# frankcholula/sapr

Hardware: AMD Instinct MI355X
Metric: frames/sec MFCC+Viterbi (16kHz, 13-MFCC, 8-state HMM) (higher is better)
Workload: dtype f32 (MFCC) + f64 (trellis); 1 GPU; configs[1]+[2]: 16 kHz 1 s utterances -> 13 MFCC (25 ms/10 ms, n_fft 512, 40 mels) -> Viterbi vs 11 word models x 8 emitting states (decoder.py API), features materialised in HBM; utterances_per_gpu=100000, frames_per_utterance=101, word_models=11, states=10, parallelism=utterance-shard x1, decoder=pruned

## Files before the change

### include/sapr_hip.h

```cpp
#ifndef SAPR_HIP_H
#define SAPR_HIP_H

#include <stddef.h>
#include <stdint.h>

#ifdef __cplusplus
extern "C" {
#endif

#define SAPR_ABI_VERSION 2

#define SAPR_TOPO_DENSE 0
#define SAPR_TOPO_BIDIAG 1

#define SAPR_TIE_LOW 0
#define SAPR_TIE_HIGH 1

#define SAPR_SUM_PAIRWISE 0
#define SAPR_SUM_TVIEW 1
#define SAPR_SUM_SEQ 2

#define SAPR_PACK_FAST_DIV 1
#define SAPR_PACK_BOUND_OK 2
#define SAPR_ESTEP_STAGED 256
#define SAPR_PACK_GEMM_OK 4
#define SAPR_PACK_BIDIAG 8

#define SAPR_PACK_EXACT_ONLY 16

#define SAPR_ERR_ARG (-1)
#define SAPR_ERR_UNSUPPORTED (-2)
#define SAPR_ERR_WORKSPACE (-3)

int sapr_abi_version(void);
const char *sapr_last_error(void);
int sapr_device_info(int dev, int *cu_count, int *wave_size, char *arch, size_t arch_len);
int sapr_selftest_lse(const double *d, int64_t n, double *out, void *stream);

int sapr_viterbi_workspace_bytes(int64_t n_utts, int32_t W, int32_t S, int32_t max_T,
                                 int32_t topology, size_t *bytes);

int sapr_diag_pack_bytes(int32_t W, int32_t S, int32_t D, size_t *bytes);
int sapr_diag_pack(const double *means, const double *vars, const double *gconst,
                   const double *log_start, const double *log_trans, int32_t W, int32_t S, int32_t D,
                   void *pack, size_t pack_bytes, int32_t *pack_flags , void *stream);

int sapr_viterbi_diag_scores(const float *feats, const int64_t *offsets, const int32_t *order,
                             int64_t n_utts, int32_t D, int32_t max_T, const void *pack,
                             int32_t W, int32_t S, int32_t topology, int32_t tie, int32_t sum_order,
                             int32_t fast_div, void *workspace, size_t workspace_bytes,
                             double *scores, int32_t *last_state, void *stream);

int sapr_viterbi_backtrace(const int64_t *offsets, const int32_t *order, int64_t n_utts,
                           int32_t max_T, int32_t W, int32_t S, int32_t topology,
                           const void *workspace, size_t workspace_bytes,
                           const double *scores, const int32_t *last_state,
                           const int32_t *word_sel,
                           int32_t *best_word, double *best_score,
                           int32_t *path , void *stream);

int sapr_viterbi_pruned_workspace_bytes(int64_t n_utts, int32_t W, int32_t S, int32_t max_T, size_t *bytes);
int sapr_viterbi_decode_pruned(const float *feats, const int64_t *offsets, const int32_t *order, int64_t n_utts,
                               int32_t D, int32_t max_T, const void *pack, int32_t W, int32_t S, int32_t tie,
                               int32_t sum_order, int32_t pack_flags, void *workspace, size_t workspace_bytes,
                               int32_t *best_word, double *best_score, int32_t *path ,
                               void *stream);
int sapr_viterbi_pruned_views(int64_t n_utts, int32_t W, int32_t max_T, void *workspace, double **approx_score,
                              double **approx_eps, double **exact_score, int32_t **cand_slot,
                              int32_t **cand_count);

int sapr_fb_workspace_bytes(int64_t n_utts, int64_t n_tiles, int32_t S, int32_t D, int32_t max_T,
                            size_t *bytes);
int sapr_stats_width(int32_t S, int32_t D, int32_t *width);
int sapr_forward_diag(const float *feats, const int64_t *offsets, const int32_t *slot_utt,
                      const int32_t *tile_model, int64_t n_tiles, int32_t D, const void *pack,
                      int32_t W, int32_t S, int32_t topology, int32_t fast_div, double *loglik,
                      void *stream);
int sapr_estep_diag(const float *feats, const int64_t *offsets, const int32_t *slot_utt,
                    const int32_t *tile_model, const int32_t *model_tile_off, int64_t n_utts,
                    int64_t n_tiles, int32_t D, int32_t max_T, const void *pack, int32_t W, int32_t S,
                    int32_t topology, int32_t fast_div, void *workspace, size_t workspace_bytes,
                    double *loglik, double *stats, void *stream);

int sapr_colsum_f32(const float *x, int64_t n_rows, int32_t D, const float *center , float *out,
                    void *stream);

int sapr_custom_estep(const float *feats, const int64_t *offsets, const int32_t *utt_model, int64_t n_utts,
                      int32_t D, int32_t S, int32_t W, const double *means, const double *inv,
                      const double *cterm, const double *A, const double *logA, int64_t lane_slots, double *E,
                      double *alpha, double *beta, double *gamma, double *xi_dense ,
                      double *utt_out, void *stream);
int sapr_custom_stage_features(const float *feats, const int64_t *offsets, int64_t n_utts, int32_t D, int32_t max_T,
                               int64_t lane_slots, float *feat_t, double *frame_sums , void *stream);
int sapr_custom_estep_staged(const float *feats, const int64_t *offsets, const int32_t *utt_model, int64_t n_utts,
                             int32_t D, int32_t S, int32_t W, const double *means, const double *inv,
                             const double *cterm, const double *A, const double *logA, int64_t lane_slots, double *E,
                             double *alpha, double *beta, double *gamma, double *xi ,
                             double *utt_out, const float *feat_t ,
                             const double *frame_sums , void *stream);
int sapr_custom_piece(int32_t op, const float *x, int32_t T, int32_t D, int32_t S, const double *means,
                      const double *inv, const double *cterm, const double *A, const double *logA, double *E,
                      double *alpha, double *beta, double *gamma, double *xi, double *scalar, void *stream);
int sapr_custom_emission_exact(const float *feats, const int64_t *offsets, int64_t n_utts, int32_t W, int32_t D,
                               int32_t S, int32_t n_rows, int32_t max_T ,
                               const double *means, const double *inv, const double *cterm, double *E, void *stream);
int sapr_custom_decode(const float *feats, const int64_t *offsets, int64_t n_utts, int32_t W, int32_t D,
                       int32_t S, int32_t num_states, int32_t Tq, const double *means, const double *inv,
                       const double *cterm, const double *A, const double *logA, double *e_rows, double *scores,
                       int32_t *paths, int32_t *best_word, double *best_score, int32_t *best_path, void *stream);
int sapr_custom_update_b_workspace_bytes(int64_t n_utts, int32_t W, int32_t D, int32_t S, size_t *bytes);
int sapr_custom_update_b(const float *feats, const int64_t *offsets, const int32_t *utt_model, int64_t n_utts,
                         int32_t W, int32_t D, int32_t S, const double *gamma, int64_t lane_slots,
                         double *means_out, double *occ_out, double *covs_out, void *workspace,
                         size_t workspace_bytes, void *stream);
int sapr_custom_update_b_sums(const float *feats, const int64_t *offsets, const int32_t *utt_model, int64_t n_utts,
                              int32_t W, int32_t D, int32_t S, const double *gamma, int64_t lane_slots,
                              double *sum_x_out, double *occ_out, void *workspace, size_t workspace_bytes,
                              void *stream);
int sapr_custom_update_b_scatter(const float *feats, const int64_t *offsets, const int32_t *utt_model,
                                 int64_t n_utts, int32_t W, int32_t D, int32_t S, const double *gamma,
                                 int64_t lane_slots, const double *means, double *scatter_out, void *workspace,
                                 size_t workspace_bytes, void *stream);
int sapr_custom_update_b_moments(const float *feats, const int64_t *offsets, int64_t n_utts, int32_t D, int32_t S,
                                 const double *gamma, int64_t lane_slots, const double *center, double *out,
                                 void *workspace, size_t workspace_bytes, void *stream);
int sapr_custom_normalise(double *x, const double *occ, int64_t n_states, int32_t per, void *stream);
int sapr_custom_fold_rows(const double *part, int64_t n_rows, int64_t K, double *out, void *stream);
int sapr_custom_global_workspace_bytes(int64_t n_utts, int64_t total_frames, int32_t D, size_t *bytes);
int sapr_custom_global_sum(const float *feats, const int64_t *offsets, int64_t n_utts, int32_t D,
                           double *sum_out, void *workspace, size_t workspace_bytes, void *stream);
int sapr_custom_global_cov(const float *feats, int64_t total_frames, int32_t D, const double *mean,
                           double *cov_out, void *workspace, size_t workspace_bytes, void *stream);

int sapr_mfcc_plan_create(double sr, int32_t n_fft, int32_t win_length, int32_t hop,
                          int32_t n_mels, int32_t n_mfcc, double fmin, double fmax ,
                          double top_db, double preemph , int32_t deltas,
                          int32_t max_frames, void **plan_out);
int sapr_mfcc_plan_destroy(void *plan);
int sapr_mfcc_plan_info(const void *plan, int32_t *d_out, int32_t *max_frames, int64_t *lds_bytes,
                        int32_t *mel_ksteps);
int sapr_mfcc_workspace_bytes(const void *plan, int64_t total_frames, int64_t n_utts, size_t *bytes);
int sapr_mfcc_batch(const void *plan, const float *pcm, const int64_t *sample_offsets,
                    const int64_t *frame_offsets, int64_t n_utts, int64_t total_frames, float *out,
                    int32_t grid_blocks , void *workspace ,
                    size_t workspace_bytes, void *stream);

int sapr_resample_poly(const float *x, const int64_t *in_offsets, const int64_t *out_offsets, int64_t n_utts,
                       int64_t max_out, int32_t up, int32_t down, const float *taps, int32_t n_taps,
                       int32_t n_pre_remove, float *y, void *stream);

int sapr_pcm16_to_f32(const int16_t *pcm16, int64_t n_samples, float *out, void *stream);

int sapr_mfcc_batch_stamped(const void *plan, const float *pcm, const int64_t *sample_offsets,
                            const int64_t *frame_offsets, int64_t n_utts, float *out,
                            int32_t grid_blocks, uint64_t *stamps, void *stream);

#ifdef __cplusplus
}
#endif
#endif
```

### sapr_amd/_lib.py

```python
from __future__ import annotations

import ctypes as C
import os

HERE = os.path.dirname(os.path.abspath(__file__))
LIB_PATH = os.environ.get("SAPR_LIB") or os.path.join(HERE, "libsapr_hip.so")

c_void_p, c_int, c_int32, c_int64, c_size_t, c_double, c_float = (
    C.c_void_p, C.c_int, C.c_int32, C.c_int64, C.c_size_t, C.c_double, C.c_float)

SIGNATURES = {
    "sapr_abi_version": (c_int, []),
    "sapr_last_error": (C.c_char_p, []),
    "sapr_device_info": (c_int, [c_int, C.POINTER(c_int), C.POINTER(c_int), C.c_char_p, c_size_t]),
    "sapr_selftest_lse": (c_int, [c_void_p, c_int64, c_void_p, c_void_p]),
    "sapr_viterbi_workspace_bytes": (c_int, [c_int64, c_int32, c_int32, c_int32, c_int32,
                                             C.POINTER(c_size_t)]),
    "sapr_diag_pack_bytes": (c_int, [c_int32, c_int32, c_int32, C.POINTER(c_size_t)]),
    "sapr_diag_pack": (c_int, [c_void_p, c_void_p, c_void_p, c_void_p, c_void_p, c_int32, c_int32, c_int32,
                               c_void_p, c_size_t, C.POINTER(c_int32), c_void_p]),
    "sapr_viterbi_diag_scores": (c_int, [c_void_p, c_void_p, c_void_p, c_int64, c_int32, c_int32,
                                         c_void_p, c_int32, c_int32, c_int32, c_int32, c_int32, c_int32,
                                         c_void_p, c_size_t, c_void_p, c_void_p, c_void_p]),
    "sapr_viterbi_backtrace": (c_int, [c_void_p, c_void_p, c_int64, c_int32, c_int32, c_int32, c_int32,
                                       c_void_p, c_size_t, c_void_p, c_void_p, c_void_p,
                                       c_void_p, c_void_p, c_void_p, c_void_p]),
    "sapr_viterbi_pruned_workspace_bytes": (c_int, [c_int64, c_int32, c_int32, c_int32, C.POINTER(c_size_t)]),
    "sapr_viterbi_decode_pruned": (c_int, [c_void_p, c_void_p, c_void_p, c_int64, c_int32, c_int32, c_void_p,
                                           c_int32, c_int32, c_int32, c_int32, c_int32, c_void_p, c_size_t,
                                           c_void_p, c_void_p, c_void_p, c_void_p]),
    "sapr_viterbi_pruned_views": (c_int, [c_int64, c_int32, c_int32, c_void_p] + [C.POINTER(c_void_p)] * 5),
    "sapr_fb_workspace_bytes": (c_int, [c_int64, c_int64, c_int32, c_int32, c_int32, C.POINTER(c_size_t)]),
    "sapr_stats_width": (c_int, [c_int32, c_int32, C.POINTER(c_int32)]),
    "sapr_forward_diag": (c_int, [c_void_p, c_void_p, c_void_p, c_void_p, c_int64, c_int32, c_void_p,
                                  c_int32, c_int32, c_int32, c_int32, c_void_p, c_void_p]),
    "sapr_estep_diag": (c_int, [c_void_p, c_void_p, c_void_p, c_void_p, c_void_p, c_int64, c_int64, c_int32,
                                c_int32, c_void_p, c_int32, c_int32, c_int32, c_int32, c_void_p, c_size_t,
                                c_void_p, c_void_p, c_void_p]),
    "sapr_colsum_f32": (c_int, [c_void_p, c_int64, c_int32, c_void_p, c_void_p, c_void_p]),
    "sapr_custom_estep": (c_int, [c_void_p, c_void_p, c_void_p, c_int64, c_int32, c_int32, c_int32] + [c_void_p] * 5
                          + [c_int64] + [c_void_p] * 6 + [c_void_p]),
    "sapr_custom_stage_features": (c_int, [c_void_p, c_void_p, c_int64, c_int32, c_int32, c_int64, c_void_p, c_void_p,
                                           c_void_p]),
    "sapr_custom_estep_staged": (c_int, [c_void_p, c_void_p, c_void_p, c_int64, c_int32, c_int32, c_int32] + [c_void_p] * 5
                                 + [c_int64] + [c_void_p] * 6 + [c_void_p, c_void_p, c_void_p]),
    "sapr_custom_piece": (c_int, [c_int32, c_void_p, c_int32, c_int32, c_int32] + [c_void_p] * 11 + [c_void_p]),
    "sapr_custom_emission_exact": (c_int, [c_void_p, c_void_p, c_int64, c_int32, c_int32, c_int32, c_int32, c_int32]
                                   + [c_void_p] * 4 + [c_void_p]),
    "sapr_custom_decode": (c_int, [c_void_p, c_void_p, c_int64, c_int32, c_int32, c_int32, c_int32, c_int32]
                           + [c_void_p] * 11 + [c_void_p]),
    "sapr_custom_update_b_workspace_bytes": (c_int, [c_int64, c_int32, c_int32, c_int32, C.POINTER(c_size_t)]),
    "sapr_custom_update_b": (c_int, [c_void_p, c_void_p, c_void_p, c_int64, c_int32, c_int32, c_int32, c_void_p, c_int64]
                             + [c_void_p] * 4 + [c_size_t, c_void_p]),
    "sapr_custom_update_b_sums": (c_int, [c_void_p, c_void_p, c_void_p, c_int64, c_int32, c_int32, c_int32, c_void_p,
                                          c_int64] + [c_void_p] * 3 + [c_size_t, c_void_p]),
    "sapr_custom_update_b_scatter": (c_int, [c_void_p, c_void_p, c_void_p, c_int64, c_int32, c_int32, c_int32, c_void_p,
                                             c_int64] + [c_void_p] * 3 + [c_size_t, c_void_p]),
    "sapr_custom_update_b_moments": (c_int, [c_void_p, c_void_p, c_int64, c_int32, c_int32, c_void_p, c_int64, c_void_p,
                                             c_void_p, c_void_p, c_size_t, c_void_p]),
    "sapr_custom_normalise": (c_int, [c_void_p, c_void_p, c_int64, c_int32, c_void_p]),
    "sapr_custom_fold_rows": (c_int, [c_void_p, c_int64, c_int64, c_void_p, c_void_p]),
    "sapr_custom_global_workspace_bytes": (c_int, [c_int64, c_int64, c_int32, C.POINTER(c_size_t)]),
    "sapr_custom_global_sum": (c_int, [c_void_p, c_void_p, c_int64, c_int32, c_void_p, c_void_p, c_size_t, c_void_p]),
    "sapr_custom_global_cov": (c_int, [c_void_p, c_int64, c_int32, c_void_p, c_void_p, c_void_p, c_size_t, c_void_p]),
    "sapr_pcm16_to_f32": (c_int, [c_void_p, c_int64, c_void_p, c_void_p]),
    "sapr_resample_poly": (c_int, [c_void_p, c_void_p, c_void_p, c_int64, c_int64, c_int32, c_int32, c_void_p, c_int32,
                                   c_int32, c_void_p, c_void_p]),
    "sapr_mfcc_plan_create": (c_int, [c_double, c_int32, c_int32, c_int32, c_int32, c_int32, c_double,
                                      c_double, c_double, c_double, c_int32, c_int32,
                                      C.POINTER(c_void_p)]),
    "sapr_mfcc_plan_destroy": (c_int, [c_void_p]),
    "sapr_mfcc_plan_info": (c_int, [c_void_p, C.POINTER(c_int32), C.POINTER(c_int32),
                                    C.POINTER(c_int64), C.POINTER(c_int32)]),
    "sapr_mfcc_workspace_bytes": (c_int, [c_void_p, c_int64, c_int64, C.POINTER(c_size_t)]),
    "sapr_mfcc_batch": (c_int, [c_void_p, c_void_p, c_void_p, c_void_p, c_int64, c_int64, c_void_p, c_int32,
                                c_void_p, c_size_t, c_void_p]),
    "sapr_mfcc_batch_stamped": (c_int, [c_void_p, c_void_p, c_void_p, c_void_p, c_int64, c_void_p, c_int32,
                                        c_void_p, c_void_p]),
}

TOPO_DENSE, TOPO_BIDIAG = 0, 1
TIE_LOW, TIE_HIGH = 0, 1
PACK_FAST_DIV, PACK_BOUND_OK, PACK_GEMM_OK, PACK_BIDIAG, PACK_EXACT_ONLY = 1, 2, 4, 8, 16
ESTEP_STAGED = 256
SUM_PAIRWISE, SUM_TVIEW, SUM_SEQ = 0, 1, 2

_lib = None


class SaprHipError(RuntimeError):
    pass


def load():
    global _lib
    if _lib is not None:
        return _lib
    if not os.path.exists(LIB_PATH):
        raise SaprHipError(
            f"{LIB_PATH} is missing: build it with `python -m sapr_amd.build` "
            "(hipcc --offload-arch=gfx950).  sapr_amd has no CPU fallback.")
    import torch
    lib = C.CDLL(LIB_PATH)
    for name, (res, args) in SIGNATURES.items():
        try:
            fn = getattr(lib, name)
        except AttributeError as e:
            raise SaprHipError(f"{LIB_PATH} lacks symbol {name}; rebuild it") from e
        fn.restype = res
        fn.argtypes = args
    if lib.sapr_abi_version() != 2:
        raise SaprHipError("libsapr_hip.so ABI version mismatch; rebuild it")
    _lib = lib
    return lib


def check(rc: int, what: str) -> None:
    if rc != 0:
        msg = load().sapr_last_error().decode("utf-8", "replace")
        raise SaprHipError(f"{what} failed (rc={rc}): {msg}")


def ptr(t):
    if t is None:
        return None
    return C.c_void_p(t.data_ptr())


def require_gpu():
    import torch
    if not torch.cuda.is_available():
        raise SaprHipError("no HIP device visible: sapr_amd kernels need an MI355X (gfx950); "
                           "there is no CPU fallback")
    return torch.device("cuda", torch.cuda.current_device())


def current_stream():
    import torch
    return C.c_void_p(torch.cuda.current_stream().cuda_stream)


def to_host(*tensors):
    import torch
    outs = []
    for t in tensors:
        if t.is_cuda:
            o = torch.empty(t.shape, dtype=t.dtype, pin_memory=True)
            o.copy_(t, non_blocking=True)
        else:
            o = t
        outs.append(o)
    if any(t.is_cuda for t in tensors):
        torch.cuda.current_stream().synchronize()
    return tuple(o.numpy() for o in outs)
```

### sapr_amd/csrc/mfcc.hip

```cpp
#include <cmath>
#include <algorithm>
#include <cstdlib>
#include <cstring>
#include <functional>
#include <type_traits>
#include <vector>

#include "sapr_common.h"

#pragma clang fp contract(fast)

#ifndef SAPR_ABLATE
#define SAPR_ABLATE 0
#endif

namespace sapr {
namespace {

constexpr int kThreads = 256;
constexpr int kWaves = kThreads / kWave;
constexpr double kPi = 3.14159265358979323846264338327950288;

typedef float f32x4 __attribute__((ext_vector_type(4)));

// ... 613 lines not shown
    if constexpr (TWO_PASS) {
      if (tid == 0) gmax_out[u] = enc_ordered(gmax);
      __syncthreads();
      continue;
    }
    const float floor_db = gmax - P.top_db;
    SAPR_STAMP(9)

    const int n_ks = align_up(P.n_mels, 16) / 4;
    for (int nt = wave; nt * 16 < T; nt += kWaves) {
      f32x4 acc = {0.f, 0.f, 0.f, 0.f};
      const int t = nt * 16 + j16;
      const int tc = t < T ? t : T - 1;
      const float *lrow = s_lm + tc * P.lm_stride + q;
      for (int ks = 0; ks < n_ks; ks += 4) {
        float a[4], b[4];
#pragma unroll
        for (int i = 0; i < 4; ++i) {
          a[i] = P.dct_frag[(ks + i) * kWave + lane];
          const int mel = 4 * (ks + i) + q;
          b[i] = mel < P.n_mels ? fmaxf(lrow[4 * (ks + i)], floor_db) : 0.f;
        }
#pragma unroll
        for (int i = 0; i < 4; ++i) acc = __builtin_amdgcn_mfma_f32_16x16x4f32(a[i], b[i], acc, 0, 0, 0);
      }
      if (t < T) *reinterpret_cast<f32x4 *>(&s_out[t * 16 + 4 * q]) = acc;
    }
    __syncthreads();
    SAPR_STAMP(10)

    {
      float *__restrict__ o = out + f_beg * P.d_out;
      const int total = T * P.d_out;
      for (int e = tid; e < total; e += kThreads) {
        const int t = e / P.d_out;
        const int c = e - t * P.d_out;
        float v;
        if (c < P.n_mfcc) {
          v = s_out[t * 16 + c];
        } else {
          const int order = c / P.n_mfcc;
          const int cc = c - order * P.n_mfcc;
          const float *tab = s_dtab + (order - 1) * 81;
          int row, t0;
          if (t < 4) {
            row = 1 + t;
            t0 = 0;
          } else if (t >= T - 4) {
            row = 5 + (t - (T - 4));
            t0 = T - 9;
          } else {
            row = 0;
            t0 = t - 4;
          }
          v = 0.f;
#pragma unroll
          for (int k = 0; k < 9; ++k) v += tab[row * 9 + k] * s_out[(t0 + k) * 16 + cc];
        }
        o[e] = v;
      }
    }
    __syncthreads();
    SAPR_STAMP(11)
  }
  if constexpr (STAMP) {
    if (lane == 0)
      for (int i = 0; i < 12; ++i) stamps[(static_cast<int64_t>(blockIdx.x) * kWaves + wave) * 12 + i] = st_acc[i];
  }
}
#undef SAPR_STAMP

constexpr int kFinChunk = 96, kFinHalo = 8, kFinRows = kFinChunk + 2 * kFinHalo;

__global__ __launch_bounds__(kThreads) void mfcc_finish_kernel(const float *__restrict__ lm,
                                                               const unsigned *__restrict__ gmax,
                                                               const int64_t *__restrict__ frame_offsets,
                                                               int64_t n_utts, MfccDev P, float *__restrict__ out) {
  extern __shared__ __attribute__((aligned(16))) unsigned char smem[];
  float *s_dtab = reinterpret_cast<float *>(smem);
  float *s_c = s_dtab + align_up(2 * 81, 4);
  float *s_l = s_c + kFinRows * 16;
  const int tid = threadIdx.x;
  const int wave = tid / kWave, lane = tid % kWave;
  const int q = lane >> 4, j16 = lane & 15;
  for (int i = tid; i < 2 * 81; i += kThreads) s_dtab[i] = P.delta_tab[i];
  __syncthreads();
  const int n_ks = align_up(P.n_mels, 16) / 4;
  for (int64_t u = blockIdx.x; u < n_utts; u += gridDim.x) {
    const int64_t f_beg = frame_offsets[u];
    const int T = static_cast<int>(frame_offsets[u + 1] - f_beg);
    const float floor_db = dec_ordered(gmax[u]) - P.top_db;
    const int chunk = T <= kFinRows ? T : kFinChunk;
    for (int c0 = 0; c0 < T; c0 += chunk) {
      const int c1 = c0 + chunk < T ? c0 + chunk : T;
      const int r0 = c0 - kFinHalo > 0 ? c0 - kFinHalo : 0;
      const int r1 = c1 + kFinHalo < T ? c1 + kFinHalo : T;
      const int rows = r1 - r0;
      const float *src = lm + (f_beg + r0) * P.n_mels;
      for (int i = tid; i < rows * P.n_mels; i += kThreads) {
        const int r = i / P.n_mels, m = i - r * P.n_mels;
        s_l[r * P.lm_stride + m] = fmaxf(src[i], floor_db);
      }
      __syncthreads();
      for (int nt = wave; nt * 16 < rows; nt += kWaves) {
        f32x4 acc = {0.f, 0.f, 0.f, 0.f};
        const int r = nt * 16 + j16;
        const int rc = r < rows ? r : rows - 1;
        const float *lrow = s_l + rc * P.lm_stride + q;
        for (int ks = 0; ks < n_ks; ks += 4) {
          float a[4], bb[4];
#pragma unroll
          for (int i = 0; i < 4; ++i) {
            a[i] = P.dct_frag[(ks + i) * kWave + lane];
            const int mel = 4 * (ks + i) + q;
            bb[i] = mel < P.n_mels ? lrow[4 * (ks + i)] : 0.f;
          }
#pragma unroll
          for (int i = 0; i < 4; ++i) acc = __builtin_amdgcn_mfma_f32_16x16x4f32(a[i], bb[i], acc, 0, 0, 0);
        }
        if (r < rows) *reinterpret_cast<f32x4 *>(&s_c[r * 16 + 4 * q]) = acc;
      }
      __syncthreads();
      float *__restrict__ o = out + (f_beg + c0) * P.d_out;
      const int total = (c1 - c0) * P.d_out;
      for (int e = tid; e < total; e += kThreads) {
        const int tl = e / P.d_out, c = e - tl * P.d_out;
        const int t = c0 + tl;
        float v;
        if (c < P.n_mfcc) {
          v = s_c[(t - r0) * 16 + c];
        } else {
          const int order = c / P.n_mfcc, cc = c - order * P.n_mfcc;
          const float *tab = s_dtab + (order - 1) * 81;
          int row, t0;
          if (t < 4) {
            row = 1 + t;
            t0 = 0;
          } else if (t >= T - 4) {
            row = 5 + (t - (T - 4));
            t0 = T - 9;
          } else {
            row = 0;
            t0 = t - 4;
          }
          v = 0.f;
#pragma unroll
          for (int k = 0; k < 9; ++k) v += tab[row * 9 + k] * s_c[(t0 + k - r0) * 16 + cc];
        }
        o[e] = v;
      }
      __syncthreads();
    }
  }
}

double hz_to_mel(double f) {
  const double f_sp = 200.0 / 3, min_log_hz = 1000.0, min_log_mel = min_log_hz / f_sp;
  const double logstep = std::log(6.4) / 27.0;
  return f >= min_log_hz ? min_log_mel + std::log(f / min_log_hz) / logstep : f / f_sp;
}
double mel_to_hz(double m) {
  const double f_sp = 200.0 / 3, min_log_hz = 1000.0, min_log_mel = min_log_hz / f_sp;
  const double logstep = std::log(6.4) / 27.0;
  return m >= min_log_mel ? min_log_hz * std::exp(logstep * (m - min_log_mel)) : f_sp * m;
}

std::vector<float> mel_filterbank(double sr, int n_fft, int n_mels, double fmin, double fmax) {
  const int nb = 1 + n_fft / 2;
  std::vector<double> mel_f(n_mels + 2);
  const double m0 = hz_to_mel(fmin), m1 = hz_to_mel(fmax);
  for (int i = 0; i < n_mels + 2; ++i) mel_f[i] = mel_to_hz(m0 + (m1 - m0) * i / (n_mels + 1));
  std::vector<float> w(static_cast<size_t>(n_mels) * nb, 0.f);
  for (int i = 0; i < n_mels; ++i) {
    const double fd0 = mel_f[i + 1] - mel_f[i], fd1 = mel_f[i + 2] - mel_f[i + 1];
    const double enorm = 2.0 / (mel_f[i + 2] - mel_f[i]);
    for (int b = 0; b < nb; ++b) {
      const double f = b * sr / n_fft;
      const double lower = -(mel_f[i] - f) / fd0, upper = (mel_f[i + 2] - f) / fd1;
      const double v = std::fmax(0.0, std::fmin(lower, upper));
      const float v32 = static_cast<float>(v);
      w[static_cast<size_t>(i) * nb + b] = static_cast<float>(static_cast<double>(v32) * enorm);
    }
  }
  return w;
}

void savgol_row(int order, double pos, double *out9) {
  const int n = 9, m = order + 1;
  double AtA[3][3] = {{0}}, inv[3][3];
  for (int i = 0; i < n; ++i) {
    double pw[3] = {1.0, i - pos, (i - pos) * (i - pos)};
    for (int a = 0; a < m; ++a)
      for (int b = 0; b < m; ++b) AtA[a][b] += pw[a] * pw[b];
  }
  double aug[3][6];
  for (int a = 0; a < m; ++a)
    for (int b = 0; b < m; ++b) {
      aug[a][b] = AtA[a][b];
      aug[a][m + b] = a == b ? 1.0 : 0.0;
    }
  for (int c = 0; c < m; ++c) {
    int piv = c;
    for (int r2 = c + 1; r2 < m; ++r2)
      if (std::fabs(aug[r2][c]) > std::fabs(aug[piv][c])) piv = r2;
    for (int b = 0; b < 2 * m; ++b) std::swap(aug[c][b], aug[piv][b]);
    const double d = aug[c][c];
    for (int b = 0; b < 2 * m; ++b) aug[c][b] /= d;
    for (int r2 = 0; r2 < m; ++r2)
      if (r2 != c) {
        const double f = aug[r2][c];
        for (int b = 0; b < 2 * m; ++b) aug[r2][b] -= f * aug[c][b];
      }
  }
  for (int a = 0; a < m; ++a)
    for (int b = 0; b < m; ++b) inv[a][b] = aug[a][m + b];
  const double fact = order == 2 ? 2.0 : 1.0;
  for (int i = 0; i < n; ++i) {
    double pw[3] = {1.0, i - pos, (i - pos) * (i - pos)};
    double c = 0.0;
    for (int b = 0; b < m; ++b) c += inv[order][b] * pw[b];
    out9[i] = fact * c;
  }
}

constexpr int kKsr = 24;

template <int R, bool PRE, bool MLDS, int KSR, bool TWO, bool BMEL = false>
hipError_t launch_one(const MfccPlan &pl, const float *pcm, const int64_t *so, const int64_t *fo,
                      int64_t n_utts, float *out, int grid, hipStream_t st, float *lm, unsigned *gmax) {
  if (pl.lds_bytes > 64 * 1024) {
    hipError_t e = hipFuncSetAttribute(reinterpret_cast<const void *>(&mfcc_kernel<R, PRE, MLDS, KSR, false, TWO, BMEL>),
                                       hipFuncAttributeMaxDynamicSharedMemorySize,
                                       static_cast<int>(pl.lds_bytes));
    if (e != hipSuccess) return e;
  }
  SAPR_LAUNCH((mfcc_kernel<R, PRE, MLDS, KSR, false, TWO, BMEL>), dim3(grid), dim3(kThreads), pl.lds_bytes, st, pcm, so,
              fo, n_utts, pl.dev, out, static_cast<unsigned long long *>(nullptr), lm, gmax);
  return hipGetLastError();
}

template <int R, bool TWO>
hipError_t launch(const MfccPlan &pl, const float *pcm, const int64_t *so, const int64_t *fo,
                  int64_t n_utts, float *out, int grid, hipStream_t st, float *lm, unsigned *gmax) {
  const bool pre = pl.dev.preemph != 0.f, ml = pl.dev.mel_in_lds != 0;
  if constexpr (R == 16) {
    if (pl.dev.ksr == kKsr) {
      if (pl.dev.mel_bf16) {
        if (pre) return launch_one<R, true, false, kKsr, TWO, true>(pl, pcm, so, fo, n_utts, out, grid, st, lm, gmax);
        return launch_one<R, false, false, kKsr, TWO, true>(pl, pcm, so, fo, n_utts, out, grid, st, lm, gmax);
      }
      if (pre) return launch_one<R, true, false, kKsr, TWO>(pl, pcm, so, fo, n_utts, out, grid, st, lm, gmax);
      return launch_one<R, false, false, kKsr, TWO>(pl, pcm, so, fo, n_utts, out, grid, st, lm, gmax);
    }
  }
  if (pre && ml) return launch_one<R, true, true, 0, TWO>(pl, pcm, so, fo, n_utts, out, grid, st, lm, gmax);
  if (pre) return launch_one<R, true, false, 0, TWO>(pl, pcm, so, fo, n_utts, out, grid, st, lm, gmax);
  if (ml) return launch_one<R, false, true, 0, TWO>(pl, pcm, so, fo, n_utts, out, grid, st, lm, gmax);
  return launch_one<R, false, false, 0, TWO>(pl, pcm, so, fo, n_utts, out, grid, st, lm, gmax);
}

template <bool PRE, int RLO, int RHI, int S4>
hipError_t wave_prepare(size_t lds, int *blocks_per_cu) {
  const void *fn = reinterpret_cast<const void *>(&mfcc_wave_kernel<PRE, RLO, RHI, S4>);
  if (lds > 64 * 1024) {
    hipError_t e = hipFuncSetAttribute(fn, hipFuncAttributeMaxDynamicSharedMemorySize, static_cast<int>(lds));
    if (e != hipSuccess) return e;
  }
  return hipOccupancyMaxActiveBlocksPerMultiprocessor(blocks_per_cu, fn, kThreads, lds);
}
template <bool PRE, int RLO, int RHI, int S4>
hipError_t wave_launch_one(const MfccPlan &pl, const float *pcm, const int64_t *so, const int64_t *fo, int64_t n_utts,
                           int grid, int64_t span, hipStream_t st, float *lm, unsigned *gmax, int64_t total_cap) {
  SAPR_LAUNCH((mfcc_wave_kernel<PRE, RLO, RHI, S4>), dim3(grid), dim3(kThreads), pl.wave_lds, st, pcm, so, fo, n_utts,
              pl.dev, lm, gmax, span, total_cap);
  return hipGetLastError();
}
template <bool PRE, int RLO, int RHI>
hipError_t wave_dispatch_s4(const MfccPlan &pl, int *prepare, const float *pcm, const int64_t *so, const int64_t *fo,
                            int64_t n_utts, int grid, int64_t span, hipStream_t st, float *lm, unsigned *gmax,
                            int64_t total_cap) {
  switch (pl.dev.wave_s4) {
#define SAPR_WAVE_CASE(S4)                                                                                        \
  case S4:                                                                                                        \
    return prepare ? wave_prepare<PRE, RLO, RHI, S4>(pl.wave_lds, prepare)                                        \
                   : wave_launch_one<PRE, RLO, RHI, S4>(pl, pcm, so, fo, n_utts, grid, span, st, lm, gmax, total_cap);
    SAPR_WAVE_CASE(6)
    SAPR_WAVE_CASE(7)
    SAPR_WAVE_CASE(8)
#undef SAPR_WAVE_CASE
    default:
      return hipErrorInvalidValue;
  }
}
hipError_t wave_dispatch(const MfccPlan &pl, int *prepare, const float *pcm, const int64_t *so, const int64_t *fo,
                         int64_t n_utts, int grid, int64_t span, hipStream_t st, float *lm, unsigned *gmax,
                         int64_t total_cap) {
  const bool pre = pl.dev.preemph != 0.f, tight = pl.wave_rlo == 1 && pl.wave_rhi == 15;
  if (pre && tight) return wave_dispatch_s4<true, 1, 15>(pl, prepare, pcm, so, fo, n_utts, grid, span, st, lm, gmax, total_cap);
  if (pre) return wave_dispatch_s4<true, 0, 16>(pl, prepare, pcm, so, fo, n_utts, grid, span, st, lm, gmax, total_cap);
  if (tight) return wave_dispatch_s4<false, 1, 15>(pl, prepare, pcm, so, fo, n_utts, grid, span, st, lm, gmax, total_cap);
  return wave_dispatch_s4<false, 0, 16>(pl, prepare, pcm, so, fo, n_utts, grid, span, st, lm, gmax, total_cap);
}

size_t finish_lds_bytes(const MfccDev &d) {
  return static_cast<size_t>(align_up(2 * 81, 4) + kFinRows * 16 + kFinRows * d.lm_stride) * 4;
}

}
}

using namespace sapr;

extern "C" int sapr_mfcc_plan_create(double sr, int32_t n_fft, int32_t win_length, int32_t hop,
                                     int32_t n_mels, int32_t n_mfcc, double fmin, double fmax,
                                     double top_db, double preemph, int32_t deltas,
                                     int32_t max_frames, void **plan_out) {
  SAPR_REQUIRE(plan_out != nullptr, "plan_out is NULL");
  SAPR_REQUIRE(n_fft == 512 || n_fft == 2048, "n_fft must be 512 or 2048 (got %d)", n_fft);
  SAPR_REQUIRE(win_length > 0 && win_length <= n_fft && hop > 0, "bad window/hop");
  SAPR_REQUIRE(n_mels > 0 && n_mels <= 128 && n_mfcc > 0 && n_mfcc <= 16 && n_mfcc <= n_mels,
               "need 0 < n_mfcc <= 16, n_mfcc <= n_mels <= 128");
  SAPR_REQUIRE(max_frames >= 0, "max_frames must be >= 0 (0 = two-pass, any utterance length)");
  SAPR_REQUIRE(!deltas || max_frames == 0 || max_frames >= 9, "deltas need at least 9 frames");
  if (fmax <= 0) fmax = sr / 2;
  const int R = n_fft == 512 ? 16 : 32;
  const int Nc = R * R, nb = Nc + 1;
  MfccPlan *pl = new MfccPlan();
  pl->R = R;
  MfccDev &d = pl->dev;
  d.n_fft = n_fft;
  d.win_length = win_length;
  d.hop = hop;
  d.n_mels = n_mels;
  d.n_mfcc = n_mfcc;
  d.deltas = deltas ? 1 : 0;
  d.d_out = n_mfcc * (deltas ? 3 : 1);
  d.n_bins = nb;
  d.lm_stride = n_mels | 1;
  d.t_pad = max_frames;
  d.two_pass = max_frames == 0 ? 1 : 0;
  d.preemph = static_cast<float>(preemph);
  d.top_db = static_cast<float>(top_db);
  d.amin = 1e-10f;

  std::vector<float> win(n_fft, 0.f);
  const int lpad = (n_fft - win_length) / 2;
  for (int i = 0; i < win_length; ++i)
    win[lpad + i] = static_cast<float>(0.5 * (0.54 - 0.46 * std::cos(2.0 * kPi * i / win_length)));
  d.r_lo = lpad / (2 * R);
  d.r_hi = (lpad + win_length - 1) / (2 * R) + 1;
  if (d.r_hi > R) d.r_hi = R;

  std::vector<float> twab(2 * R * R), twu(2 * Nc);
  for (int k1 = 0; k1 < R; ++k1)
    for (int l = 0; l < R; ++l) {
      const double a = -2.0 * kPi * k1 * l / Nc;
      twab[2 * (k1 * R + l)] = static_cast<float>(std::cos(a));
      twab[2 * (k1 * R + l) + 1] = static_cast<float>(std::sin(a));
    }
  for (int k = 0; k < Nc; ++k) {
    const double a = -kPi * k / Nc;
    twu[2 * k] = static_cast<float>(std::cos(a));
    twu[2 * k + 1] = static_cast<float>(std::sin(a));
  }

  std::vector<float> mel = mel_filterbank(sr, n_fft, n_mels, fmin, fmax);
  std::vector<int> mlo(n_mels), mhi(n_mels);
  for (int m = 0; m < n_mels; ++m) {
    int lo = nb, hi = -1;
    for (int b = 0; b < nb; ++b)
      if (mel[static_cast<size_t>(m) * nb + b] != 0.f) {
        lo = b < lo ? b : lo;
        hi = b > hi ? b : hi;
      }
    if (hi < 0) lo = hi = 0;
    mlo[m] = lo;
    mhi[m] = hi;
  }
  auto tile_ks = [&](int m0, int m1) {
    int lo = nb, hi = 0;
    for (int m = m0; m < m1; ++m) {
      lo = mlo[m] < lo ? mlo[m] : lo;
      hi = mhi[m] > hi ? mhi[m] : hi;
    }
    lo = lo / 4 * 4;
    return align_up((hi - lo) / 4 + 1, 4);
  };
  const int want_tiles = align_up((n_mels + 15) / 16, kWaves);
  auto cut = [&](int limit, std::vector<int> *starts) {
    int m0 = 0, n = 0;
    if (starts) starts->clear();
    while (m0 < n_mels) {
      int m1 = m0 + 1;
      if (tile_ks(m0, m1) > limit) return 1 << 30;
      while (m1 < n_mels && m1 - m0 < 16 && tile_ks(m0, m1 + 1) <= limit) ++m1;
      if (starts) starts->push_back(m0);
      m0 = m1;
      ++n;
    }
    return n;
  };
  int lim_lo = 4, lim_hi = align_up(nb / 4 + 1, 4);
  while (lim_lo < lim_hi) {
    const int mid = (lim_lo + lim_hi) / 8 * 4;
    if (cut(mid, nullptr) <= want_tiles)
      lim_hi = mid;
    else
      lim_lo = mid + 4;
  }
  std::vector<int> starts;
  cut(lim_lo, &starts);
  d.n_mtiles = static_cast<int>(starts.size());
  if (d.n_mtiles > 15) {
    delete pl;
    return fail(SAPR_ERR_UNSUPPORTED, "mel filterbank needs %d tiles (> 15)", d.n_mtiles);
  }
  std::vector<int> tiles(4 * (d.n_mtiles + 1), 0);
  std::vector<float> frag;
  int ks_total = 0;
  for (int mt = 0; mt < d.n_mtiles; ++mt) {
    const int m0 = starts[mt], m1 = mt + 1 < d.n_mtiles ? starts[mt + 1] : n_mels;
    int lo = nb;
    for (int m = m0; m < m1; ++m) lo = mlo[m] < lo ? mlo[m] : lo;
    lo = lo / 4 * 4;
    const int nks = tile_ks(m0, m1);
    tiles[4 * mt + 0] = m0;
    tiles[4 * mt + 1] = m1 - m0;
    tiles[4 * mt + 2] = lo;
    tiles[4 * mt + 3] = ks_total;
    for (int ks = 0; ks < nks; ++ks)
      for (int ln = 0; ln < 64; ++ln) {
        const int mi = ln & 15, b = lo + 4 * ks + (ln >> 4);
        frag.push_back((mi < m1 - m0 && b < nb) ? mel[static_cast<size_t>(m0 + mi) * nb + b] : 0.f);
      }
    ks_total += nks;
  }
  tiles[4 * d.n_mtiles + 3] = ks_total;
  d.total_ks = ks_total;
  auto bf16_rn = [](float v) {
    unsigned b;
    std::memcpy(&b, &v, 4);
    b = (b + 0x7FFFu + ((b >> 16) & 1u)) >> 16;
    return b;
  };
  auto bf16_val = [](unsigned h) {
    const unsigned b = h << 16;
    float v;
    std::memcpy(&v, &b, 4);
    return v;
  };
  std::vector<unsigned> frag16;
  if (d.n_mtiles <= kWaves) {
    frag16.assign(static_cast<size_t>(d.n_mtiles) * 24 * 64, 0u);
    for (int mt = 0; mt < d.n_mtiles; ++mt) {
      const int m0 = tiles[4 * mt + 0], cnt = tiles[4 * mt + 1], lo = tiles[4 * mt + 2];
      for (int c = 0; c < 3; ++c)
        for (int i = 0; i < 4; ++i)
          for (int ln = 0; ln < 64; ++ln) {
            unsigned hi_w = 0, lo_w = 0;
            for (int h = 0; h < 2; ++h) {
              const int mi = ln & 15, b = lo + 32 * c + 8 * i + 2 * (ln >> 4) + h;
              const float v = (mi < cnt && b < nb) ? mel[static_cast<size_t>(m0 + mi) * nb + b] : 0.f;
              const unsigned vh = bf16_rn(v), vl = bf16_rn(v - bf16_val(vh));
              hi_w |= vh << (16 * h);
              lo_w |= vl << (16 * h);
            }
            frag16[(static_cast<size_t>(mt) * 24 + 8 * c + i) * 64 + ln] = hi_w;
            frag16[(static_cast<size_t>(mt) * 24 + 8 * c + 4 + i) * 64 + ln] = lo_w;
          }
    }
  }
  const int nks_d = align_up(n_mels, 16) / 4;
  std::vector<float> dfrag(static_cast<size_t>(std::max(nks_d, 16)) * 64, 0.f);
  for (int ks = 0; ks < nks_d; ++ks)
    for (int ln = 0; ln < 64; ++ln) {
      const int c = ln & 15, m = 4 * ks + (ln >> 4);
      if (c < n_mfcc && m < n_mels) {
        const double sc = c == 0 ? std::sqrt(1.0 / (4.0 * n_mels)) : std::sqrt(1.0 / (2.0 * n_mels));
        dfrag[ks * 64 + ln] = static_cast<float>(2.0 * std::cos(kPi * c * (2 * m + 1) / (2.0 * n_mels)) * sc);
      }
    }
  WavePack wp;
  {
    const char *core = std::getenv("SAPR_MFCC_CORE");
    const bool want = !(core && std::strcmp(core, "tile") == 0);
    if (want && R == 16 && hop % 2 == 0) wp = wave_pack(mel, n_mels, nb);
  }
  std::vector<float> dtab(2 * 81, 0.f);
  for (int order = 1; order <= 2; ++order) {
    double row[9];
    savgol_row(order, 4.0, row);
    for (int k = 0; k < 9; ++k) dtab[(order - 1) * 81 + k] = static_cast<float>(row[k]);
    for (int p = 0; p < 4; ++p) {
      savgol_row(order, p, row);
      for (int k = 0; k < 9; ++k) dtab[(order - 1) * 81 + (1 + p) * 9 + k] = static_cast<float>(row[k]);
      savgol_row(order, 5 + p, row);
      for (int k = 0; k < 9; ++k) dtab[(order - 1) * 81 + (5 + p) * 9 + k] = static_cast<float>(row[k]);
    }
  }

  auto pad = [](size_t b) { return (b + 255) / 256 * 256; };
  const size_t b_win = pad(win.size() * 4), b_ab = pad(twab.size() * 4), b_u = pad(twu.size() * 4),
               b_fr = pad(frag.size() * 4), b_ti = pad(tiles.size() * 4),
               b_df = pad(dfrag.size() * 4), b_dt = pad(dtab.size() * 4), b_f16 = pad(frag16.size() * 4 + 4),
               b_wa = pad(wp.a.size() * 4 + 4), b_wb = pad(wp.blk.size() * 4 + 4);
  const size_t total = b_win + b_ab + b_u + b_fr + b_ti + b_df + b_dt + b_f16 + b_wa + b_wb;
  std::vector<unsigned char> host(total, 0);
  size_t o = 0;
  auto put = [&](const void *src, size_t bytes, size_t padded) {
    std::copy(static_cast<const unsigned char *>(src), static_cast<const unsigned char *>(src) + bytes,
              host.begin() + o);
    const size_t at = o;
    o += padded;
    return at;
  };
  const size_t o_win = put(win.data(), win.size() * 4, b_win);
  const size_t o_ab = put(twab.data(), twab.size() * 4, b_ab);
  const size_t o_u = put(twu.data(), twu.size() * 4, b_u);
  const size_t o_fr = put(frag.data(), frag.size() * 4, b_fr);
  const size_t o_ti = put(tiles.data(), tiles.size() * 4, b_ti);
  const size_t o_df = put(dfrag.data(), dfrag.size() * 4, b_df);
  const size_t o_dt = put(dtab.data(), dtab.size() * 4, b_dt);
  const size_t o_f16 = put(frag16.data(), frag16.size() * 4, b_f16);
  const size_t o_wa = put(wp.a.data(), wp.a.size() * 4, b_wa);
  const size_t o_wb = put(wp.blk.data(), wp.blk.size() * 4, b_wb);
  unsigned char *devbuf = nullptr;
  hipError_t e = hipMalloc(reinterpret_cast<void **>(&devbuf), total);
  if (e != hipSuccess) {
    delete pl;
    return hip_fail(e, "hipMalloc(mfcc tables)");
  }
  e = hipMemcpy(devbuf, host.data(), total, hipMemcpyHostToDevice);
  if (e != hipSuccess) {
    (void)hipFree(devbuf);
    delete pl;
    return hip_fail(e, "hipMemcpy(mfcc tables)");
  }
  pl->buffer = devbuf;
  d.window = reinterpret_cast<const float *>(devbuf + o_win);
  d.tw_ab = reinterpret_cast<const float2 *>(devbuf + o_ab);
  d.tw_u = reinterpret_cast<const float2 *>(devbuf + o_u);
  d.mel_frag = reinterpret_cast<const float *>(devbuf + o_fr);
  d.mel_tiles = reinterpret_cast<const int *>(devbuf + o_ti);
  d.dct_frag = reinterpret_cast<const float *>(devbuf + o_df);
  d.delta_tab = reinterpret_cast<const float *>(devbuf + o_dt);
  d.mel_frag_bf16 = reinterpret_cast<const unsigned *>(devbuf + o_f16);
  d.wave_s4 = wp.s4;
  d.wave_a = reinterpret_cast<const float *>(devbuf + o_wa);
  d.wave_blk = reinterpret_cast<const int *>(devbuf + o_wb);

  {
    const int tile = R == 16 ? 16 : 8;
    d.span0 = 2 * R * d.r_lo - n_fft / 2;
    d.span_len = (tile - 1) * hop + 2 * R * (d.r_hi - d.r_lo);
    d.stage_floats = align_up(d.span_len, 4);
    if (d.span_len > kStagePasses * kThreads * 4 || hop % 2 != 0) {
      (void)hipFree(devbuf);
      delete pl;
      return fail(SAPR_ERR_UNSUPPORTED, "hop %d / window %d: staged span of %d samples unsupported (max %d, even hop)",
                  hop, win_length, d.span_len, kStagePasses * kThreads * 4);
    }
  }
  int max_nks = 0;
  for (int mt = 0; mt < d.n_mtiles; ++mt) {
    const int nks = tiles[4 * (mt + 1) + 3] - tiles[4 * mt + 3];
    max_nks = nks > max_nks ? nks : max_nks;
  }
  d.ksr = (R == 16 && d.n_mtiles <= kWaves && max_nks <= kKsr) ? kKsr : 0;
  {
    const char *sel = std::getenv("SAPR_MFCC_MEL");
    d.mel_bf16 = (d.ksr && sel && std::strcmp(sel, "bf16") == 0) ? 1 : 0;
  }
  auto lds_total = [&](int ml) {
    const int tp = d.two_pass ? 0 : d.t_pad;
    return R == 16 ? lds_layout<16>(tp, d.lm_stride, d.total_ks, ml, d.n_mels, d.stage_floats).total
                   : lds_layout<32>(tp, d.lm_stride, d.total_ks, ml, d.n_mels, d.stage_floats).total;
  };
  auto pick_mel = [&]() {
    if (d.ksr) return 0;
    return lds_total(1) <= 80 * 1024 || (lds_total(0) > 80 * 1024 && lds_total(1) <= 160 * 1024) ? 1 : 0;
  };
  d.mel_in_lds = pick_mel();
  if (!d.two_pass && lds_total(d.mel_in_lds) > 160 * 1024) {
    d.two_pass = 1;
    d.mel_in_lds = pick_mel();
  }
  if (!d.two_pass && lds_total(d.mel_in_lds) > 80 * 1024) {
    const char *keep = std::getenv("SAPR_MFCC_FUSED");
    MfccDev t = d;
    t.two_pass = 1;
    auto total_of = [&](const MfccDev &x, int ml) {
      return R == 16 ? lds_layout<16>(0, x.lm_stride, x.total_ks, ml, x.n_mels, x.stage_floats).total
                     : lds_layout<32>(0, x.lm_stride, x.total_ks, ml, x.n_mels, x.stage_floats).total;
    };
    const int ml2 = t.ksr ? 0 : ((total_of(t, 1) <= 80 * 1024 || (total_of(t, 0) > 80 * 1024 && total_of(t, 1) <= 160 * 1024)) ? 1 : 0);
    if (!(keep && keep[0] == '1') && total_of(t, ml2) <= 80 * 1024) {
      d.two_pass = 1;
      d.mel_in_lds = ml2;
    }
  }
  pl->lds_bytes = static_cast<size_t>(lds_total(d.mel_in_lds));
  if (pl->lds_bytes > 160 * 1024) {
    (void)hipFree(devbuf);
    const size_t need = pl->lds_bytes;
    delete pl;
    return fail(SAPR_ERR_UNSUPPORTED, "configuration needs %zu bytes of LDS (> 160 KiB)", need);
  }
  if (d.wave_s4) {
    d.two_pass = 1;
    pl->wave_rlo = (d.r_lo >= 1 && d.r_hi <= 15) ? 1 : 0;
    pl->wave_rhi = (d.r_lo >= 1 && d.r_hi <= 15) ? 15 : 16;
    pl->wave_lds = static_cast<size_t>(wave_lds(d.wave_s4, wave_region_floats(d.n_mels, d.deltas)).total);
    pl->lds_bytes = pl->wave_lds;
    hipError_t oe = wave_dispatch(*pl, &pl->wave_blocks_per_cu, nullptr, nullptr, nullptr, 0, 0, 1, nullptr, nullptr,
                                  nullptr, 0);
    if (oe != hipSuccess || pl->wave_blocks_per_cu < 1) {
      (void)hipFree(devbuf);
      delete pl;
      return hip_fail(oe, "occupancy query (mfcc_wave_kernel)");
    }
  }
  *plan_out = pl;
  return 0;
}

extern "C" int sapr_mfcc_plan_destroy(void *plan) {
  if (!plan) return 0;
  MfccPlan *pl = static_cast<MfccPlan *>(plan);
  if (pl->buffer) (void)hipFree(pl->buffer);
  delete pl;
  return 0;
}

extern "C" int sapr_mfcc_plan_info(const void *plan, int32_t *d_out, int32_t *max_frames,
                                   int64_t *lds_bytes, int32_t *mel_ksteps) {
  SAPR_REQUIRE(plan != nullptr, "plan is NULL");
  const MfccPlan *pl = static_cast<const MfccPlan *>(plan);
  if (d_out) *d_out = pl->dev.d_out;
  if (max_frames) *max_frames = pl->dev.two_pass ? 0 : pl->dev.t_pad;
  if (lds_bytes) *lds_bytes = static_cast<int64_t>(pl->lds_bytes);
  if (mel_ksteps) *mel_ksteps = pl->dev.total_ks;
  return 0;
}

extern "C" int sapr_mfcc_batch_stamped(const void *plan, const float *pcm, const int64_t *sample_offsets,
                                       const int64_t *frame_offsets, int64_t n_utts, float *out,
                                       int32_t grid_blocks, uint64_t *stamps, void *stream) {
  SAPR_REQUIRE(plan && pcm && sample_offsets && frame_offsets && out && stamps, "NULL pointer argument");
  const MfccPlan *pl = static_cast<const MfccPlan *>(plan);
  SAPR_REQUIRE(pl->R == 16 && pl->dev.preemph == 0.f && pl->dev.ksr == kKsr, "stamped build: bench preset only");
  SAPR_REQUIRE(grid_blocks > 0 && grid_blocks <= n_utts, "bad grid");
  if (pl->dev.mel_bf16) {
    if (pl->lds_bytes > 64 * 1024)
      SAPR_HIP_TRY(hipFuncSetAttribute(reinterpret_cast<const void *>(&mfcc_kernel<16, false, false, kKsr, true, false, true>),
                                       hipFuncAttributeMaxDynamicSharedMemorySize, static_cast<int>(pl->lds_bytes)));
    SAPR_LAUNCH((mfcc_kernel<16, false, false, kKsr, true, false, true>), dim3(grid_blocks), dim3(kThreads),
                pl->lds_bytes, as_stream(stream), pcm, sample_offsets, frame_offsets, n_utts, pl->dev, out,
                reinterpret_cast<unsigned long long *>(stamps));
  } else {
    if (pl->lds_bytes > 64 * 1024)
      SAPR_HIP_TRY(hipFuncSetAttribute(reinterpret_cast<const void *>(&mfcc_kernel<16, false, false, kKsr, true>),
                                       hipFuncAttributeMaxDynamicSharedMemorySize, static_cast<int>(pl->lds_bytes)));
    SAPR_LAUNCH((mfcc_kernel<16, false, false, kKsr, true>), dim3(grid_blocks), dim3(kThreads), pl->lds_bytes,
                as_stream(stream), pcm, sample_offsets, frame_offsets, n_utts, pl->dev, out,
                reinterpret_cast<unsigned long long *>(stamps));
  }
  SAPR_HIP_TRY(hipGetLastError());
  return 0;
}

extern "C" int sapr_mfcc_workspace_bytes(const void *plan, int64_t total_frames, int64_t n_utts, size_t *bytes) {
  SAPR_REQUIRE(plan && bytes && total_frames >= 0 && n_utts >= 0, "bad arguments");
  const MfccPlan *pl = static_cast<const MfccPlan *>(plan);
  *bytes = pl->dev.two_pass
               ? (static_cast<size_t>(total_frames) * pl->dev.n_mels + static_cast<size_t>(n_utts)) * sizeof(float) + 256
               : 0;
  return 0;
}

extern "C" int sapr_mfcc_batch(const void *plan, const float *pcm, const int64_t *sample_offsets,
                               const int64_t *frame_offsets, int64_t n_utts, int64_t total_frames, float *out,
                               int32_t grid_blocks, void *workspace, size_t workspace_size, void *stream) {
  SAPR_REQUIRE(plan != nullptr, "plan is NULL");
  SAPR_REQUIRE(n_utts >= 0 && total_frames >= 0, "bad sizes");
  if (n_utts == 0) return 0;
  SAPR_REQUIRE(pcm && sample_offsets && frame_offsets && out, "NULL pointer argument");
  const MfccPlan *pl = static_cast<const MfccPlan *>(plan);
  int dev = 0, cus = 256;
  SAPR_HIP_TRY(hipGetDevice(&dev));
  SAPR_HIP_TRY(hipDeviceGetAttribute(&cus, hipDeviceAttributeMultiprocessorCount, dev));
  int grid = grid_blocks;
  if (grid <= 0) {
    const int per_cu = static_cast<int>((160 * 1024) / pl->lds_bytes);
    const int cap = 3;
    grid = cus * (per_cu < 1 ? 1 : (per_cu > cap ? cap : per_cu));
  }
  if (grid > n_utts) grid = static_cast<int>(n_utts);
  hipStream_t st = as_stream(stream);
  if (!pl->dev.two_pass) {
    if (pl->R == 16)
      SAPR_HIP_TRY((launch<16, false>(*pl, pcm, sample_offsets, frame_offsets, n_utts, out, grid, st, nullptr, nullptr)));
    else
      SAPR_HIP_TRY((launch<32, false>(*pl, pcm, sample_offsets, frame_offsets, n_utts, out, grid, st, nullptr, nullptr)));
    return 0;
  }
  const size_t need = (static_cast<size_t>(total_frames) * pl->dev.n_mels + static_cast<size_t>(n_utts)) * sizeof(float) + 256;
  if (!workspace || workspace_size < need)
    return fail(SAPR_ERR_WORKSPACE, "two-pass MFCC plan needs a %zu-byte workspace (sapr_mfcc_workspace_bytes)", need);
  float *lm = static_cast<float *>(workspace);
  unsigned *gmax = reinterpret_cast<unsigned *>(lm + static_cast<size_t>(total_frames) * pl->dev.n_mels);
  if (pl->dev.wave_s4) {
    int wgrid = grid_blocks > 0 ? grid_blocks : cus * pl->wave_blocks_per_cu;
    const int64_t n_waves = static_cast<int64_t>(wgrid) * kWaves;
    int64_t span = (total_frames + n_waves - 1) / n_waves;
    span = span < 4 ? 4 : (span + 3) / 4 * 4;
    const int64_t need_blocks = ((total_frames + span - 1) / span + kWaves - 1) / kWaves;
    if (need_blocks < wgrid) wgrid = static_cast<int>(need_blocks < 1 ? 1 : need_blocks);
    SAPR_HIP_TRY(hipMemsetAsync(gmax, 0, static_cast<size_t>(n_utts) * sizeof(unsigned), st));
    SAPR_HIP_TRY(wave_dispatch(*pl, nullptr, pcm, sample_offsets, frame_offsets, n_utts, wgrid, span, st, lm, gmax,
                               total_frames));
    int fgrid = cus * SAPR_FINISH_OCC;
    const int64_t fwaves = static_cast<int64_t>(fgrid) * kWaves;
    int fsplit = 1;
    if (n_utts < fwaves) {
      fsplit = static_cast<int>(std::min<int64_t>(8, fwaves / n_utts));
      const int64_t need_blocks = (n_utts * fsplit + kWaves - 1) / kWaves;
      if (need_blocks < fgrid) fgrid = static_cast<int>(need_blocks);
    }
    SAPR_LAUNCH(mfcc_wave_finish_kernel, dim3(fgrid), dim3(kThreads), wave_finish_lds(pl->dev.n_mels, pl->dev.deltas), st,
                lm, gmax, frame_offsets, n_utts, pl->dev, out, fsplit, total_frames);
    SAPR_HIP_TRY(hipGetLastError());
    return 0;
  } else if (pl->R == 16)
    SAPR_HIP_TRY((launch<16, true>(*pl, pcm, sample_offsets, frame_offsets, n_utts, out, grid, st, lm, gmax)));
  else
    SAPR_HIP_TRY((launch<32, true>(*pl, pcm, sample_offsets, frame_offsets, n_utts, out, grid, st, lm, gmax)));
  int fgrid = cus * 6;
  if (fgrid > n_utts) fgrid = static_cast<int>(n_utts);
  SAPR_LAUNCH(mfcc_finish_kernel, dim3(fgrid), dim3(kThreads), finish_lds_bytes(pl->dev), st, lm, gmax, frame_offsets,
              n_utts, pl->dev, out);
  SAPR_HIP_TRY(hipGetLastError());
  return 0;
}
```

### sapr_amd/csrc/mfcc_wave.h

```cpp
#pragma once

constexpr int kWRowPad = 18;
constexpr int kWGroup = 16 * kWRowPad;
constexpr int kWRegion = 4 * kWGroup;
#include "mfcc_wave_pack.h"

struct WaveLds {
  int win, twab, twu, mela, dtab, scr, total;
};
__host__ __device__ inline int wave_region_floats(int, int) { return kWRegion; }
__host__ __device__ inline WaveLds wave_lds(int s4, int region_floats) {
  WaveLds L;
  int o = 0;
  L.win = o;
  o += 512 * 4;
  L.twab = o;
  o += 256 * 8;
  L.twu = o;
  o += 128 * 8;
  L.mela = o;
  o += s4 * kWave * 16;
  L.dtab = o;
  o += 2 * 81 * 4 + 8;
  L.scr = o;
  o += kWaves * region_floats * 4;
  L.total = o;
  return L;
}

__host__ __device__ inline unsigned enc_ordered(float v) {
  const unsigned u = __builtin_bit_cast(unsigned, v);
  return (u & 0x80000000u) ? ~u : (u | 0x80000000u);
}
__host__ __device__ inline float dec_ordered(unsigned e) {
  const unsigned u = (e & 0x80000000u) ? (e & 0x7FFFFFFFu) : ~e;
  return __builtin_bit_cast(float, u);
}

struct __attribute__((packed, aligned(4))) f2u {
  float x, y;
};

template <bool PREEMPH, int NR>
struct WaveSet {
  f2u y[NR];
  float m0;
};

typedef float v2f __attribute__((ext_vector_type(2)));
__device__ __forceinline__ unsigned lds_addr(const void *p) {
  return static_cast<unsigned>(reinterpret_cast<uintptr_t>((__attribute__((address_space(3))) const void *)p));
}
template <int OFF>
__device__ __forceinline__ v2f ds_rd64(unsigned addr) {
  v2f v;
  asm volatile("ds_read_b64 %0, %1 offset:%2" : "=v"(v) : "v"(addr), "n"(OFF));
  return v;
}
template <int OFF>
__device__ __forceinline__ v2f ds_rd64_mem(unsigned addr) {
  v2f v;
  asm volatile("ds_read_b64 %0, %1 offset:%2" : "=v"(v) : "v"(addr), "n"(OFF) : "memory");
  return v;
}
__device__ __forceinline__ void lds_wait() { asm volatile("s_waitcnt lgkmcnt(0)" ::: "memory"); }
template <int N>
__device__ __forceinline__ void lds_dep(v2f (&v)[N]) {
#pragma unroll
  for (int i = 0; i < N; ++i) asm volatile("" : "+v"(v[i]));
}

template <int CTRL>
__device__ __forceinline__ float dpp_mov(float v) {
  return __int_as_float(__builtin_amdgcn_mov_dpp(__float_as_int(v), CTRL, 0xf, 0xf, true));
}

#ifndef SAPR_WAVE_CNDDPP
#define SAPR_WAVE_CNDDPP 1
#endif
#ifndef SAPR_WAVE_FRAG64
#define SAPR_WAVE_FRAG64 0
#endif
__device__ __forceinline__ void mirror_unless2(float a, float b, unsigned long long keep, float &ma, float &mb) {
  asm("s_mov_b64 vcc, %4\n\ts_nop 0\n\t"
      "v_cndmask_b32_dpp %0, %2, %2, vcc row_mirror row_mask:0xf bank_mask:0xf\n\t"
      "v_cndmask_b32_dpp %1, %3, %3, vcc row_mirror row_mask:0xf bank_mask:0xf"
      : "=&v"(ma), "=v"(mb)
      : "v"(a), "v"(b), "s"(keep)
      : "vcc");
}

__device__ __forceinline__ void mirror_unless2_e64(float a, float b, unsigned long long keep, float &ma, float &mb) {
  asm("s_nop 1\n\t"
      "v_mov_b32_dpp %0, %2 row_mirror row_mask:0xf bank_mask:0xf\n\t"
      "v_mov_b32_dpp %1, %3 row_mirror row_mask:0xf bank_mask:0xf\n\t"
      "v_cndmask_b32_e64 %0, %0, %2, %4\n\t"
      "v_cndmask_b32_e64 %1, %1, %3, %4"
      : "=&v"(ma), "=&v"(mb)
      : "v"(a), "v"(b), "s"(keep));
}

__device__ __forceinline__ void wave_fence() {
  __builtin_amdgcn_fence(__ATOMIC_RELEASE, "wavefront");
  __builtin_amdgcn_wave_barrier();
  __builtin_amdgcn_fence(__ATOMIC_ACQUIRE, "wavefront");
}
__device__ __forceinline__ void wave_finish(const float *__restrict__ lm, int T, float floor_db, float *__restrict__ out,
                                            const MfccDev &P, float *s_tile, float *s_ceps, const float *s_dtab,
                                            int lane, int tile_lo, int tile_hi) {
  const int q = lane >> 4, j16 = lane & 15;
  const int NQ = P.n_mels >> 2, LS = P.n_mels + 4, per_tile = 16 * NQ;
  const float inv_nm = 1.0f / static_cast<float>(P.n_mfcc);
  const int n_tiles = (T + 15) >> 4;
  const bool deltas = P.deltas != 0;
  float dc1[9], dc2[9];
#pragma unroll
  for (int k = 0; k < 9; ++k) {
    dc1[k] = deltas ? s_dtab[k] : 0.f;
    dc2[k] = deltas ? s_dtab[81 + k] : 0.f;
  }
  const int first = deltas && tile_lo > 0 ? tile_lo - 1 : tile_lo;
  const int last = deltas && tile_hi < n_tiles ? tile_hi + 1 : tile_hi;
  float afr[16];
#pragma unroll
  for (int ks = 0; ks < 16; ++ks) afr[ks] = P.dct_frag[ks * kWave + lane];
  int prow_[4], pcg_[4];
  {
    const float inv_nq = 1.0f / static_cast<float>(NQ);
#pragma unroll
    for (int c = 0; c < 4; ++c) {
      const int idx = lane + kWave * c;
      prow_[c] = static_cast<int>((static_cast<float>(idx) + 0.5f) * inv_nq);
      pcg_[c] = idx - prow_[c] * NQ;
    }
  }
  auto fetch = [&](int nt, float4 (&v)[4]) {
#pragma unroll
    for (int c = 0; c < 4; ++c)
      if (lane + kWave * c < per_tile) {
        const int t = 16 * nt + prow_[c] < T ? 16 * nt + prow_[c] : T - 1;
        v[c] = reinterpret_cast<const float4 *>(lm + static_cast<int64_t>(t) * P.n_mels)[pcg_[c]];
      }
  };
  auto tile = [&](int nt, float4 (&cur)[4]) {
    if (nt < last) {
#pragma unroll
      for (int c = 0; c < 4; ++c)
        if (lane + kWave * c < per_tile) {
          float4 v = cur[c];
          v.x = fmaxf(v.x, floor_db);
          v.y = fmaxf(v.y, floor_db);
          v.z = fmaxf(v.z, floor_db);
          v.w = fmaxf(v.w, floor_db);
          *reinterpret_cast<float4 *>(s_tile + prow_[c] * LS + 4 * pcg_[c]) = v;
        }
      if (nt + 3 < last) fetch(nt + 3, cur);
      wave_fence();
      f32x4 acc0 = {0.f, 0.f, 0.f, 0.f}, acc1 = {0.f, 0.f, 0.f, 0.f};
      const float *lrow = s_tile + j16 * LS + q;
      float bv[16];
#pragma unroll
      for (int ks = 0; ks < 16; ++ks) bv[ks] = lrow[4 * ks];
#pragma unroll
      for (int ks = 0; ks < 16; ks += 2) {
        acc0 = __builtin_amdgcn_mfma_f32_16x16x4f32(afr[ks], bv[ks], acc0, 0, 0, 0);
        acc1 = __builtin_amdgcn_mfma_f32_16x16x4f32(afr[ks + 1], bv[ks + 1], acc1, 0, 0, 0);
      }
      *reinterpret_cast<f32x4 *>(s_ceps + (deltas ? (nt % 3) * 256 : 0) + j16 * 16 + 4 * q) = acc0 + acc1;
      wave_fence();
    }
    const int e = deltas ? nt - 1 : nt;
    if (e >= tile_lo && e < tile_hi) {
      const int rows = T - 16 * e < 16 ? T - 16 * e : 16;
      float *__restrict__ o = out + static_cast<int64_t>(16 * e) * P.d_out;
      if (!deltas) {
#pragma unroll
        for (int c4 = 0; c4 < 4; ++c4) {
          const int idx = lane + kWave * c4;
          if (idx < rows * P.n_mfcc) {
            const int tl = static_cast<int>((static_cast<float>(idx) + 0.5f) * inv_nm), c = idx - tl * P.n_mfcc;
            o[idx] = s_ceps[tl * 16 + c];
          }
        }
      } else {
        auto ceps = [&](int t, int c) { return s_ceps[((t >> 4) % 3) * 256 + (t & 15) * 16 + c]; };
#pragma unroll
        for (int c4 = 0; c4 < 4; ++c4) {
          const int idx = lane + kWave * c4;
          if (idx < rows * P.n_mfcc) {
            const int tl = static_cast<int>((static_cast<float>(idx) + 0.5f) * inv_nm), c = idx - tl * P.n_mfcc;
            const int t = 16 * e + tl;
            float d1 = 0.f, d2 = 0.f;
            if (t >= 4 && t < T - 4) {
#pragma unroll
              for (int k = 0; k < 9; ++k) {
                const float x = ceps(t - 4 + k, c);
                d1 += dc1[k] * x;
                d2 += dc2[k] * x;
              }
            } else {
              const int row = t < 4 ? 1 + t : 5 + (t - (T - 4)), t0 = t < 4 ? 0 : T - 9;
#pragma unroll
              for (int k = 0; k < 9; ++k) {
                const float x = ceps(t0 + k, c);
                d1 += s_dtab[row * 9 + k] * x;
                d2 += s_dtab[81 + row * 9 + k] * x;
              }
            }
            float *ot = o + tl * P.d_out + c;
            ot[0] = ceps(t, c);
            ot[P.n_mfcc] = d1;
            ot[2 * P.n_mfcc] = d2;
          }
        }
      }
      wave_fence();
    }
  };
  float4 t0[4], t1[4], t2[4];
  if (first < last) fetch(first, t0);
  if (first + 1 < last) fetch(first + 1, t1);
  if (first + 2 < last) fetch(first + 2, t2);
  const int end = last + (deltas ? 1 : 0);
  for (int base = first; base < end; base += 3) {
    tile(base, t0);
    if (base + 1 < end) tile(base + 1, t1);
    if (base + 2 < end) tile(base + 2, t2);
  }
}

#ifndef SAPR_FINISH_OCC
#define SAPR_FINISH_OCC 3
#endif
__global__ __launch_bounds__(kThreads, SAPR_FINISH_OCC) void mfcc_wave_finish_kernel(const float *__restrict__ lm,
                                                                       const unsigned *__restrict__ gmax_enc,
                                                                       const int64_t *__restrict__ frame_offsets,
                                                                       int64_t n_utts, MfccDev P, float *__restrict__ out,
                                                                       int split, int64_t total_cap) {
  extern __shared__ __attribute__((aligned(16))) unsigned char smem[];
  float *s_dtab = reinterpret_cast<float *>(smem);
  const int per_wave = 16 * (P.n_mels + 4) + (P.deltas ? 3 : 1) * 256;
  const int tid = threadIdx.x;
  const int wave = __builtin_amdgcn_readfirstlane(tid / kWave), lane = tid % kWave;
  for (int i = tid; i < 2 * 81; i += kThreads) s_dtab[i] = P.delta_tab[i];
  for (int i = tid; i < kWaves * per_wave; i += kThreads) s_dtab[168 + i] = 0.f;
  __syncthreads();
  float *s_tile = s_dtab + 168 + wave * per_wave;
  const int n_waves = gridDim.x * kWaves;
  const int wid = blockIdx.x * kWaves + wave;
  if (frame_offsets[n_utts] > total_cap) {
    const int64_t n = total_cap * P.d_out;
    for (int64_t i = static_cast<int64_t>(blockIdx.x) * kThreads + tid; i < n; i += static_cast<int64_t>(gridDim.x) * kThreads)
      out[i] = __builtin_nanf("");
    return;
  }
  const int n_teams = n_waves / split, part = wid % split;
  if (wid >= n_teams * split) return;
  for (int64_t u = wid / split; u < n_utts; u += n_teams) {
    const int64_t f_beg = frame_offsets[u];
    const int T = static_cast<int>(frame_offsets[u + 1] - f_beg);
    const int n_tiles = (T + 15) >> 4, per = (n_tiles + split - 1) / split;
    const int lo = part * per, hi = lo + per < n_tiles ? lo + per : n_tiles;
    if (lo >= hi) continue;
    wave_finish(lm + f_beg * P.n_mels, T, dec_ordered(gmax_enc[u]) - P.top_db, out + f_beg * P.d_out, P, s_tile,
                s_tile + 16 * (P.n_mels + 4), s_dtab, lane, lo, hi);
  }
}
inline size_t wave_finish_lds(int n_mels, int deltas) {
  return static_cast<size_t>(168 + kWaves * (16 * (n_mels + 4) + (deltas ? 3 : 1) * 256)) * 4;
}

#ifndef SAPR_WAVE_OCC
#define SAPR_WAVE_OCC 4
#endif

template <bool PREEMPH, int RLO, int RHI, int S4>
__global__ __launch_bounds__(kThreads, SAPR_WAVE_OCC) void mfcc_wave_kernel(
    const float *__restrict__ pcm, const int64_t *__restrict__ sample_offsets,
    const int64_t *__restrict__ frame_offsets, int64_t n_utts, MfccDev P, float *__restrict__ lm_out,
    unsigned *__restrict__ gmax_enc, int64_t span, int64_t total_cap) {
  constexpr int R = 16, kNc = 256, kBits = 4, NR = RHI - RLO;
  extern __shared__ __attribute__((aligned(16))) unsigned char smem[];
  const int region_floats = wave_region_floats(P.n_mels, P.deltas);
  const WaveLds L = wave_lds(S4, region_floats);
  float *s_win = reinterpret_cast<float *>(smem + L.win);
  float2 *s_twab = reinterpret_cast<float2 *>(smem + L.twab);
  float2 *s_twu = reinterpret_cast<float2 *>(smem + L.twu);
  float4 *s_a = reinterpret_cast<float4 *>(smem + L.mela);
  float *s_dtab = reinterpret_cast<float *>(smem + L.dtab);
  float *s_scr = reinterpret_cast<float *>(smem + L.scr);

  const int tid = threadIdx.x;
  const int wave = __builtin_amdgcn_readfirstlane(tid / kWave);
  const int lane = tid % kWave;

  for (int i = tid; i < 512; i += kThreads) s_win[i] = P.window[i];
  for (int i = tid; i < 256; i += kThreads) s_twab[i] = P.tw_ab[i];
  for (int i = tid; i < 128; i += kThreads) s_twu[i] = P.tw_u[i];
  for (int i = tid; i < S4 * kWave; i += kThreads) s_a[i] = reinterpret_cast<const float4 *>(P.wave_a)[i];
  for (int i = tid; i < 2 * 81; i += kThreads) s_dtab[i] = P.delta_tab[i];
  for (int i = tid; i < kWaves * region_floats; i += kThreads) s_scr[i] = 0.f;
  __syncthreads();

  const int grp = lane >> 4;
  const int l = lane & 15;
  const int sigma = l < 8 ? l : (l == 15 ? 8 : l + 1);
  const bool is0 = l == 0;
  [[maybe_unused]] const bool special = l == 0 || l == 15;
  const unsigned long long special_mask = 0x8001800180018001ull;
  float *region = s_scr + wave * region_floats;
  float *scr = region + grp * kWGroup;
  float *prow = region + grp * kWPRow;
  const int rot = (grp & 1) * 8;
  float *wlo = scr + rot * kWRowPad + l;
  float *whi = scr + (rot ? -8 : 0) * kWRowPad + l;
  const unsigned a_rrow = lds_addr(scr + ((sigma + rot) & 15) * kWRowPad);
  const unsigned a_twu = lds_addr(s_twu + sigma);
  const unsigned a_twab = lds_addr(s_twab + l);
  const unsigned a_win = lds_addr(reinterpret_cast<const float2 *>(s_win) + l);

  const int j4 = lane & 3;
  const int4 bi = reinterpret_cast<const int4 *>(P.wave_blk)[lane >> 2];
  const float4 *bq = reinterpret_cast<const float4 *>(region + j4 * kWPRow + bi.x);
  const float4 *aq = s_a + lane;
  const int mel0 = bi.y;
  const float f1 = bi.z ? 1.f : 0.f, f2 = bi.w ? 1.f : 0.f;

  const int64_t total = frame_offsets[n_utts];
  const int64_t wid = static_cast<int64_t>(blockIdx.x) * kWaves + wave;
  if (total > total_cap) return;
  const int64_t run_lo = wid * span;
  if (run_lo >= total) return;
  const int64_t run_hi = run_lo + span < total ? run_lo + span : total;
  int64_t u_first = 0;
  {
    int64_t hi = n_utts;
    while (hi - u_first > 1) {
      const int64_t mid = (u_first + hi) >> 1;
      if (frame_offsets[mid] <= run_lo)
// ... 240 lines not shown
```

### sapr_amd/csrc/sapr_common.h

```cpp
#pragma once

#include <hip/hip_runtime.h>

#include <cstdarg>
#include <cstdint>
#include <cstdio>
#include <limits>
#include <string>

#include "../../include/sapr_hip.h"

namespace sapr {

constexpr int kWave = 64;

std::string &last_error();
int fail(int code, const char *fmt, ...);
int hip_fail(hipError_t e, const char *what);

#define SAPR_HIP_TRY(expr)                                      \
  do {                                                          \
    hipError_t _e = (expr);                                     \
    if (_e != hipSuccess) return ::sapr::hip_fail(_e, #expr);   \
  } while (0)

#define SAPR_REQUIRE(cond, ...)                                         \
  do {                                                                  \
    if (!(cond)) return ::sapr::fail(SAPR_ERR_ARG, __VA_ARGS__);        \
  } while (0)

inline hipStream_t as_stream(void *s) { return reinterpret_cast<hipStream_t>(s); }

#define SAPR_LAUNCH(...)             \
  do {                               \
    (void)hipGetLastError();         \
    hipLaunchKernelGGL(__VA_ARGS__); \
  } while (0)

__device__ __forceinline__ constexpr double neg_inf() { return -__builtin_huge_val(); }

template <int N>
__device__ __forceinline__ double np_pairwise_sum(const double (&a)[N]) {
  static_assert(N >= 1 && N <= 128, "numpy switches to recursive halving above 128 terms");
  if constexpr (N < 8) {
    double r = 0.0;
#pragma unroll
    for (int i = 0; i < N; ++i) r += a[i];
    return r;
  } else {
    double r[8];
#pragma unroll
    for (int j = 0; j < 8; ++j) r[j] = a[j];
    constexpr int kFull = N - (N % 8);
#pragma unroll
    for (int i = 8; i < kFull; i += 8) {
#pragma unroll
      for (int j = 0; j < 8; ++j) r[j] += a[i + j];
    }
    double res = ((r[0] + r[1]) + (r[2] + r[3])) + ((r[4] + r[5]) + (r[6] + r[7]));
#pragma unroll
    for (int i = kFull; i < N; ++i) res += a[i];
    return res;
  }
}

__device__ __forceinline__ int wave_max_i32(int v) {
#pragma unroll
  for (int o = 32; o > 0; o >>= 1) {
    int other = __shfl_xor(v, o, 64);
    v = other > v ? other : v;
  }
  return v;
}

}
```

### sapr_amd/csrc/viterbi.hip

```cpp
#include "emission.h"
#include "viterbi_shared.h"

namespace sapr {
namespace {

using namespace emission;

__global__ __launch_bounds__(kBlock) void viterbi_select_kernel(
    const int32_t *__restrict__ order, int64_t n_utts, int64_t n_slots, int32_t W,
    const double *__restrict__ ascore, const double *__restrict__ aeps, int32_t *__restrict__ cand_cnt,
    int32_t *__restrict__ cand_utt, int32_t *__restrict__ cand_slot) {
  constexpr int kMaxW = 64;
  __shared__ int wave_cnt[kMaxW][kBlock / kWave];
  __shared__ int block_base[kMaxW];
  const int64_t p = static_cast<int64_t>(blockIdx.x) * kBlock + threadIdx.x;
  const bool live = p < n_utts;
  const int64_t u = live ? (order ? static_cast<int64_t>(order[p]) : p) : 0;
  const int lane = threadIdx.x & 63, wave = threadIdx.x >> 6;
  double thr = neg_inf();
  if (live)
    for (int w = 0; w < W; ++w) {
      const double lo = ascore[u * W + w] - aeps[u * W + w];
      if (lo > thr) thr = lo;
    }
// ... 257 lines not shown
      e = e < -40 ? -40 : (e > 40 ? 40 : e);
      return static_cast<float>(ldexp(1.0, e));
    };
    a_sq = pow2_below(128.0 / r);
    a_lin = pow2_below(16384.0 / r);
  }
  out[d] = c;
  out[G8 + d] = a_sq;
  out[2 * G8 + d] = a_lin;
}

__device__ int unreachable_tail(const double *__restrict__ log_start, const double *__restrict__ log_trans, int S,
                                int w) {
  int j0 = S;
  for (int j = S - 1; j >= 1; --j) {
    if (log_start[static_cast<int64_t>(w) * S + j] != neg_inf()) break;
    if (log_trans[(static_cast<int64_t>(w) * S + (j - 1)) * S + j] == neg_inf()) j0 = j;
  }
  return j0;
}

__device__ double gemm_entry(const double *__restrict__ means, const double *__restrict__ vars,
                             const double *__restrict__ gconst, const double *__restrict__ log_trans,
                             const PackView &pv, int W, int S, int D, int w, int j, int g, int i, bool *noself_elsewhere,
                             int tail ) {
  const int G = gemm_groups(D), G8 = 8 * G;
  if (j >= S || j >= tail) return 0.0;
  const int64_t row = (static_cast<int64_t>(w) * S + j) * D;
  if (g < G) {
    const int f = 8 * g + i;
    if (f < D) {
      const double a = static_cast<double>(pv.gctr[G8 + f]);
      return -0.5 * (1.0 / vars[row + f]) / (a * a);
    }
    if (f == D) {
      double c0 = 0.0;
      for (int d = 0; d < D; ++d) {
        const double mu = means[row + d] - static_cast<double>(pv.gctr[d]);
        c0 += mu * mu / vars[row + d];
      }
      double sg = log_trans[(static_cast<int64_t>(w) * S + j) * S + j];
      if (sg == neg_inf()) {
        if (j % 4 != 0) *noself_elsewhere = true;
        sg = 0.0;
      }
      return (-0.5 * (c0 + gconst[static_cast<int64_t>(w) * S + j]) + sg) * (1.0 / 1024.0);
    }
  } else if (g < 2 * G) {
    const int f = 8 * (g - G) + i;
    if (f < D)
      return (means[row + f] - static_cast<double>(pv.gctr[f])) / vars[row + f] /
             static_cast<double>(pv.gctr[2 * G8 + f]);
  }
  return 0.0;
}

__global__ void diag_pack_gemm_max_kernel(const double *__restrict__ means, const double *__restrict__ vars,
                                          const double *__restrict__ gconst, const double *__restrict__ log_trans,
                                          int W, int S, int D, double *__restrict__ blob, int *__restrict__ bad) {
  const PackView pv = pack_view(blob, W, S, D);
  const int G = gemm_groups(D);
  const int64_t idx = blockIdx.x * static_cast<int64_t>(blockDim.x) + threadIdx.x;
  if (idx >= static_cast<int64_t>(W) * S * 2 * G) return;
  const int g = static_cast<int>(idx % (2 * G));
  const int j = static_cast<int>((idx / (2 * G)) % S);
  const int w = static_cast<int>(idx / (2 * G) / S);
  bool elsewhere = false;
  double m = 0.0;
  const int tail = unreachable_tail(pv.log_start, log_trans, S, w);
  for (int i = 0; i < 8; ++i) {
    const double v = fabs(gemm_entry(means, vars, gconst, log_trans, pv, W, S, D, w, j, g, i, &elsewhere, tail));
    if (!(v <= 1e300)) atomicOr(bad, 4);
    else if (v > m) m = v;
  }
  if (elsewhere) atomicOr(bad, 4);
  atomicMax(reinterpret_cast<unsigned long long *>(const_cast<double *>(pv.gkw) + 2 * W + 2),
            static_cast<unsigned long long>(__double_as_longlong(m)));
}

__global__ void diag_pack_gemm_kernel(const double *__restrict__ means, const double *__restrict__ vars,
                                      const double *__restrict__ gconst, const double *__restrict__ log_trans,
                                      int W, int S, int D, double *__restrict__ blob, int *__restrict__ bad) {
  const PackView pv = pack_view(blob, W, S, D);
  const int KC = gemm_kchunks(D), RT = gemm_rtiles(S);
  const int64_t idx = blockIdx.x * static_cast<int64_t>(blockDim.x) + threadIdx.x;
  if (idx >= static_cast<int64_t>(W) * RT * KC * 64) return;
  const double pmax = pv.gkw[2 * W + 2];
  int ge = (pmax > 0.0) ? static_cast<int>(floor(log2(16384.0 / pmax))) : 0;
  ge = ge < -60 ? -60 : (ge > 60 ? 60 : ge);
  const double scale = ldexp(1.0, ge);
  if (idx == 0) {
    const_cast<double *>(pv.gkw)[2 * W] = scale;
    const_cast<double *>(pv.gkw)[2 * W + 1] = ldexp(1.0, -ge);
    if (!(pmax > 0.0) || pmax * scale >= 32768.0) atomicOr(bad, 4);
  }
  const int lane = static_cast<int>(idx & 63);
  int64_t rest = idx >> 6;
  const int c = static_cast<int>(rest % KC);
  rest /= KC;
  const int rt = static_cast<int>(rest % RT);
  const int w = static_cast<int>(rest / RT);
  const int j = 16 * rt + (lane & 15), g = 4 * c + (lane >> 4);
  unsigned pc[2][4] = {{0u, 0u, 0u, 0u}, {0u, 0u, 0u, 0u}};
  bool elsewhere = false;
  const int tail = unreachable_tail(pv.log_start, log_trans, S, w);
  for (int i = 0; i < 8; ++i) {
    const float v32 = static_cast<float>(gemm_entry(means, vars, gconst, log_trans, pv, W, S, D, w, j, g, i, &elsewhere, tail) * scale);
    const _Float16 hi = static_cast<_Float16>(v32);
    const _Float16 lo = static_cast<_Float16>(v32 - static_cast<float>(hi));
    const int sh = 16 * (i & 1);
    pc[0][i >> 1] |= static_cast<unsigned>(__builtin_bit_cast(unsigned short, hi)) << sh;
    pc[1][i >> 1] |= static_cast<unsigned>(__builtin_bit_cast(unsigned short, lo)) << sh;
  }
  uint4 *out = const_cast<uint4 *>(pv.gfrag);
  for (int p = 0; p < 2; ++p)
    out[(((static_cast<int64_t>(w) * RT + rt) * KC + c) * 2 + p) * 64 + lane] =
        make_uint4(pc[p][0], pc[p][1], pc[p][2], pc[p][3]);
}

__global__ void diag_pack_gemm_consts_kernel(const double *__restrict__ means, const double *__restrict__ vars,
                                             const double *__restrict__ gconst, const double *__restrict__ log_trans,
                                             int W, int S, int D, double *__restrict__ blob, int *__restrict__ bad) {
  const int w = blockIdx.x * blockDim.x + threadIdx.x;
  if (w >= W) return;
  const PackView pv = pack_view(blob, W, S, D);
  const double scale = pv.gkw[2 * W];
  const int j0 = unreachable_tail(pv.log_start, log_trans, S, w);
  {
    double *R = const_cast<double *>(pv.gR) + static_cast<int64_t>(w) * S;
    double *Rf = R + static_cast<int64_t>(W) * S;
    double acc = 0.0;
    for (int j = 0; j < S; ++j) {
      if (j >= 1 && j < j0) {
        double sg = log_trans[(static_cast<int64_t>(w) * S + (j - 1)) * S + (j - 1)];
        if (sg == neg_inf()) sg = 0.0;
        const double r = log_trans[(static_cast<int64_t>(w) * S + (j - 1)) * S + j] - sg;
        if (!(fabs(r) <= 1e300)) atomicOr(bad, 4);
        acc += r;
      }
      R[j] = acc;
      Rf[j] = j < j0 ? acc : neg_inf();
    }
  }
  double k = 0.0, psum = 0.0;
  for (int s = 0; s < S; ++s) {
    double c0 = 0.0;
    for (int d = 0; d < D; ++d) {
      const int64_t i = (static_cast<int64_t>(w) * S + s) * D + d;
      const double mu = means[i] - static_cast<double>(pv.gctr[d]);
      c0 += mu * mu / vars[i];
    }
    double sg = log_trans[(static_cast<int64_t>(w) * S + s) * S + s];
    if (sg == neg_inf()) sg = 0.0;
    k = nan_max(k, 3.0 * c0 + 2.0 * fabs(gconst[w * S + s]) + 4.0 * fabs(sg));
    double row = 0.0;
    bool unused = false;
    for (int g = 0; g < 2 * gemm_groups(D); ++g)
      for (int i = 0; i < 8; ++i)
        row += fabs(gemm_entry(means, vars, gconst, log_trans, pv, W, S, D, w, s, g, i, &unused, j0)) * scale;
    psum = nan_max(psum, row);
  }
  const_cast<double *>(pv.gkw)[w] = k;
  const_cast<double *>(pv.gkw)[W + w] = psum;
}


}
}

using namespace sapr;

extern "C" int sapr_viterbi_workspace_bytes(int64_t n_utts, int32_t W, int32_t S, int32_t max_T,
                                            int32_t topology, size_t *bytes) {
  SAPR_REQUIRE(bytes != nullptr, "bytes is NULL");
  SAPR_REQUIRE(n_utts >= 0 && W > 0 && S > 0 && max_T >= 0, "bad sizes");
  SAPR_REQUIRE(topology == SAPR_TOPO_DENSE || topology == SAPR_TOPO_BIDIAG, "bad topology");
  *bytes = workspace_bytes(n_utts, W, S, max_T, topology);
  return 0;
}

extern "C" int sapr_diag_pack_bytes(int32_t W, int32_t S, int32_t D, size_t *bytes) {
  SAPR_REQUIRE(bytes != nullptr && W > 0 && S > 0 && D > 0, "bad arguments");
  *bytes = pack_doubles(W, S, D) * sizeof(double) + 64;
  return 0;
}

extern "C" int sapr_diag_pack(const double *means, const double *vars, const double *gconst,
                              const double *log_start, const double *log_trans, int32_t W, int32_t S,
                              int32_t D, void *pack, size_t pack_bytes, int32_t *fast_div_ok,
                              void *stream) {
  SAPR_REQUIRE(W > 0 && S > 0 && D > 0, "bad sizes");
  SAPR_REQUIRE(means && vars && gconst && log_start && log_trans && pack, "NULL pointer argument");
  SAPR_REQUIRE(pack_bytes >= pack_doubles(W, S, D) * sizeof(double) + 64, "pack buffer too small");
  hipStream_t st = as_stream(stream);
  const bool exact_only = fast_div_ok && (*fast_div_ok & SAPR_PACK_EXACT_ONLY);
  int *flag = reinterpret_cast<int *>(static_cast<double *>(pack) + pack_doubles(W, S, D));
  SAPR_HIP_TRY(hipMemsetAsync(flag, 0, sizeof(int), st));
  SAPR_LAUNCH(diag_pack_kernel, dim3(64), dim3(256), 0, st, means, vars, gconst, log_start, log_trans,
                     W, S, D, static_cast<double *>(pack), flag);
  SAPR_LAUNCH(diag_pack_consts_kernel, dim3((W + 63) / 64), dim3(64), 0, st, means, vars, gconst, log_start,
              log_trans, W, S, D, static_cast<double *>(pack), flag);
  if (!exact_only) {
  SAPR_LAUNCH(diag_pack_center_kernel, dim3(1), dim3(64 * ((8 * gemm_groups(D) + 63) / 64)), 0, st, means, vars, W, S,
              D, static_cast<double *>(pack));
  const int64_t n_ent = static_cast<int64_t>(W) * S * 2 * gemm_groups(D);
  SAPR_LAUNCH(diag_pack_gemm_max_kernel, dim3(static_cast<unsigned>((n_ent + 255) / 256)), dim3(256), 0, st, means,
              vars, gconst, log_trans, W, S, D, static_cast<double *>(pack), flag);
  const int64_t n_gemm = static_cast<int64_t>(W) * gemm_rtiles(S) * gemm_kchunks(D) * 64;
  SAPR_LAUNCH(diag_pack_gemm_kernel, dim3(static_cast<unsigned>((n_gemm + 255) / 256)), dim3(256), 0, st, means, vars,
              gconst, log_trans, W, S, D, static_cast<double *>(pack), flag);
  SAPR_LAUNCH(diag_pack_gemm_consts_kernel, dim3((W + 63) / 64), dim3(64), 0, st, means, vars, gconst, log_trans, W, S,
              D, static_cast<double *>(pack), flag);
  }
  SAPR_HIP_TRY(hipGetLastError());
  int bad = 0;
  SAPR_HIP_TRY(hipMemcpyAsync(&bad, flag, sizeof(int), hipMemcpyDeviceToHost, st));
  SAPR_HIP_TRY(hipStreamSynchronize(st));
  if (fast_div_ok) {
    *fast_div_ok = ((bad & 1) ? 0 : SAPR_PACK_FAST_DIV) | ((bad & 2) ? 0 : SAPR_PACK_BOUND_OK) |
                   ((bad & 6) ? 0 : SAPR_PACK_GEMM_OK) | ((bad & 8) ? 0 : SAPR_PACK_BIDIAG);
    if (exact_only) *fast_div_ok = (*fast_div_ok & ~(SAPR_PACK_BOUND_OK | SAPR_PACK_GEMM_OK)) | SAPR_PACK_EXACT_ONLY;
  }
  return 0;
}

extern "C" int sapr_viterbi_diag_scores(const float *feats, const int64_t *offsets,
                                        const int32_t *order, int64_t n_utts, int32_t D,
                                        int32_t max_T, const void *pack, int32_t W, int32_t S,
                                        int32_t topology, int32_t tie, int32_t sum_order,
                                        int32_t fast_div, void *workspace, size_t workspace_size,
                                        double *scores, int32_t *last_state, void *stream) {
  SAPR_REQUIRE(n_utts >= 0 && W > 0 && S > 0 && D > 0 && max_T >= 0, "bad sizes");
  SAPR_REQUIRE(topology == SAPR_TOPO_DENSE || topology == SAPR_TOPO_BIDIAG, "bad topology");
  SAPR_REQUIRE(tie == SAPR_TIE_LOW || tie == SAPR_TIE_HIGH, "bad tie-break");
  SAPR_REQUIRE(sum_order == SAPR_SUM_PAIRWISE || sum_order == SAPR_SUM_TVIEW || sum_order == SAPR_SUM_SEQ, "bad sum_order");
  if (n_utts == 0) return 0;
  SAPR_REQUIRE(feats && offsets && pack && scores && last_state && workspace, "NULL pointer argument");
  if (workspace_size < workspace_bytes(n_utts, W, S, max_T, topology))
    return fail(SAPR_ERR_WORKSPACE, "workspace too small: %zu < %zu", workspace_size,
                workspace_bytes(n_utts, W, S, max_T, topology));
  const PackView pv = pack_view(pack, W, S, D);
  ScoreArgs a;
  a.feats = feats;
  a.offsets = offsets;
  a.order = order;
  a.n_utts = n_utts;
  a.n_tiles = (n_utts + kBlock - 1) / kBlock;
  a.n_slots = round_up(n_utts, kBlock);
  a.max_T = max_T > 0 ? max_T : 1;
  a.W = W;
  a.prm = pv.prm;
  a.gconst = pv.gconst;
  a.log_start = pv.log_start;
  a.log_trans = pv.log_trans;
  a.bp = workspace;
  a.scores = scores;
  a.last_state = last_state;
  a.stream = as_stream(stream);
  a.seq_all = sum_order == SAPR_SUM_SEQ ? 1 : 0;
  const int fast = (fast_div & SAPR_PACK_FAST_DIV) ? 1 : 0;
  if (D == 13 && S == 10) return launch_scores_13_10(a, topology, tie, sum_order, fast);
  if (D == 13 && S == 18) return launch_scores_13_18(a, topology, tie, sum_order, fast);
  if (D == 39 && S == 10) return launch_scores_39_10(a, topology, tie, sum_order, fast);
  if (D == 39 && S == 18) return launch_scores_39_18(a, topology, tie, sum_order, fast);
  return fail(SAPR_ERR_UNSUPPORTED,
              "viterbi kernels are instantiated for (D,S) in {13,39}x{10,18}; got D=%d S=%d", D, S);
}

extern "C" int sapr_viterbi_backtrace(const int64_t *offsets, const int32_t *order, int64_t n_utts,
                                      int32_t max_T, int32_t W, int32_t S, int32_t topology,
                                      const void *workspace, size_t workspace_size,
                                      const double *scores, const int32_t *last_state,
                                      const int32_t *word_sel, int32_t *best_word,
                                      double *best_score, int32_t *path, void *stream) {
  SAPR_REQUIRE(n_utts >= 0 && W > 0 && S > 0 && max_T >= 0, "bad sizes");
  SAPR_REQUIRE(topology == SAPR_TOPO_DENSE || topology == SAPR_TOPO_BIDIAG, "bad topology");
  if (n_utts == 0) return 0;
  SAPR_REQUIRE(offsets && scores && last_state && workspace, "NULL pointer argument");
  if (workspace_size < workspace_bytes(n_utts, W, S, max_T, topology))
    return fail(SAPR_ERR_WORKSPACE, "workspace too small");
  const int64_t n_slots = round_up(n_utts, kBlock);
  const int mt = max_T > 0 ? max_T : 1;
  dim3 grid(static_cast<unsigned>((n_utts + kBlock - 1) / kBlock)), block(kBlock);
  if (topology == SAPR_TOPO_BIDIAG)
    SAPR_LAUNCH(viterbi_backtrace_kernel<true>, grid, block, 0, as_stream(stream), offsets,
                       order, n_utts, n_slots, mt, W, S, workspace, scores, last_state, word_sel,
                       best_word, best_score, path);
  else
    SAPR_LAUNCH(viterbi_backtrace_kernel<false>, grid, block, 0, as_stream(stream), offsets,
                       order, n_utts, n_slots, mt, W, S, workspace, scores, last_state, word_sel,
                       best_word, best_score, path);
  SAPR_HIP_TRY(hipGetLastError());
  return 0;
}

extern "C" int sapr_viterbi_pruned_workspace_bytes(int64_t n_utts, int32_t W, int32_t S, int32_t max_T,
                                                   size_t *bytes) {
  SAPR_REQUIRE(bytes != nullptr, "bytes is NULL");
  SAPR_REQUIRE(n_utts >= 0 && W > 0 && S > 0 && S <= 32 && max_T >= 0, "bad sizes");
  *bytes = pruned_layout(n_utts, W, max_T).total;
  return 0;
}

extern "C" int sapr_viterbi_decode_pruned(const float *feats, const int64_t *offsets, const int32_t *order,
                                          int64_t n_utts, int32_t D, int32_t max_T, const void *pack, int32_t W,
                                          int32_t S, int32_t tie, int32_t sum_order, int32_t pack_flags,
                                          void *workspace, size_t workspace_size, int32_t *best_word,
                                          double *best_score, int32_t *path, void *stream) {
  SAPR_REQUIRE(n_utts >= 0 && W > 0 && S > 0 && D > 0 && max_T >= 0, "bad sizes");
  SAPR_REQUIRE(tie == SAPR_TIE_LOW || tie == SAPR_TIE_HIGH, "bad tie-break");
  SAPR_REQUIRE(sum_order == SAPR_SUM_PAIRWISE || sum_order == SAPR_SUM_TVIEW || sum_order == SAPR_SUM_SEQ, "bad sum_order");
  if (!(pack_flags & SAPR_PACK_BOUND_OK))
    return fail(SAPR_ERR_UNSUPPORTED, "model pack is outside the bounding pass's domain (variances in "
                                      "[1e-20, 1e20]): use sapr_viterbi_diag_scores + sapr_viterbi_backtrace");
  if (S > 32 || !(pack_flags & SAPR_PACK_BIDIAG))
    return fail(SAPR_ERR_UNSUPPORTED, "the pruned decoder covers the bidiagonal topology only (transitions i -> i and "
                                      "i -> i + 1, S <= 32; sapr_diag_pack reports SAPR_PACK_BIDIAG): use "
                                      "sapr_viterbi_diag_scores + sapr_viterbi_backtrace");
  if (n_utts == 0) return 0;
  SAPR_REQUIRE(feats && offsets && pack && workspace && best_word && best_score, "NULL pointer argument");
  const PrunedLayout L = pruned_layout(n_utts, W, max_T);
  if (workspace_size < L.total)
    return fail(SAPR_ERR_WORKSPACE, "workspace too small: %zu < %zu", workspace_size, L.total);
  char *ws = static_cast<char *>(workspace);
  auto *cand_utt = reinterpret_cast<int32_t *>(ws + L.cand_utt);
  auto *cand_slot = reinterpret_cast<int32_t *>(ws + L.cand_slot);
  auto *ascore = reinterpret_cast<double *>(ws + L.ascore);
  auto *aeps = reinterpret_cast<double *>(ws + L.aeps);
  auto *scores = reinterpret_cast<double *>(ws + L.scores);
  auto *last = reinterpret_cast<int32_t *>(ws + L.last);
  auto *cnt = reinterpret_cast<int32_t *>(ws + L.cnt);
  const PackView pv = pack_view(pack, W, S, D);
  ScoreArgs a;
  a.feats = feats;
  a.offsets = offsets;
  a.order = order;
  a.n_utts = n_utts;
  a.n_tiles = (n_utts + kBlock - 1) / kBlock;
  a.n_slots = round_up(n_utts, kBlock);
  a.max_T = max_T > 0 ? max_T : 1;
  a.W = W;
  a.prm = pv.prm;
  a.gconst = pv.gconst;
  a.log_start = pv.log_start;
  a.log_trans = pv.log_trans;
  a.bp = ws + L.bp;
  a.scores = scores;
  a.last_state = last;
  a.stream = as_stream(stream);
  a.seq_all = sum_order == SAPR_SUM_SEQ ? 1 : 0;
  int rc;
  if (D == 13 && S == 10) rc = launch_approx_13_10(a, pv, ascore, aeps, pack_flags);
  else if (D == 13 && S == 18) rc = launch_approx_13_18(a, pv, ascore, aeps, pack_flags);
  else if (D == 39 && S == 10) rc = launch_approx_39_10(a, pv, ascore, aeps, pack_flags);
  else if (D == 39 && S == 18) rc = launch_approx_39_18(a, pv, ascore, aeps, pack_flags);
  else
    return fail(SAPR_ERR_UNSUPPORTED,
                "viterbi kernels are instantiated for (D,S) in {13,39}x{10,18}; got D=%d S=%d", D, S);
  if (rc) return rc;
  SAPR_HIP_TRY(hipMemsetAsync(cnt, 0, static_cast<size_t>(W) * sizeof(int32_t), a.stream));
  dim3 ugrid(static_cast<unsigned>(a.n_tiles)), block(kBlock);
  SAPR_LAUNCH(viterbi_select_kernel, ugrid, block, 0, a.stream, order, n_utts, a.n_slots, W, ascore, aeps, cnt,
              cand_utt, cand_slot);
  SAPR_HIP_TRY(hipGetLastError());
  a.cand_utt = cand_utt;
  a.cand_cnt = cnt;
  const int fast = (pack_flags & SAPR_PACK_FAST_DIV) ? 1 : 0;
  if (D == 13 && S == 10) rc = launch_scores_13_10(a, SAPR_TOPO_BIDIAG, tie, sum_order, fast);
  else if (D == 13 && S == 18) rc = launch_scores_13_18(a, SAPR_TOPO_BIDIAG, tie, sum_order, fast);
  else if (D == 39 && S == 10) rc = launch_scores_39_10(a, SAPR_TOPO_BIDIAG, tie, sum_order, fast);
  else rc = launch_scores_39_18(a, SAPR_TOPO_BIDIAG, tie, sum_order, fast);
  if (rc) return rc;
  SAPR_LAUNCH(viterbi_backtrace_pruned_kernel, ugrid, block, 0, a.stream, offsets, order, n_utts, a.n_slots, a.max_T,
              W, reinterpret_cast<const uint32_t *>(ws + L.bp), scores, last, cand_slot, best_word, best_score, path);
  SAPR_HIP_TRY(hipGetLastError());
  return 0;
}

extern "C" int sapr_viterbi_pruned_views(int64_t n_utts, int32_t W, int32_t max_T, void *workspace,
                                         double **approx_score, double **approx_eps, double **exact_score,
                                         int32_t **cand_slot, int32_t **cand_count) {
  SAPR_REQUIRE(workspace != nullptr && n_utts >= 0 && W > 0, "bad arguments");
  const PrunedLayout L = pruned_layout(n_utts, W, max_T);
  char *ws = static_cast<char *>(workspace);
  if (approx_score) *approx_score = reinterpret_cast<double *>(ws + L.ascore);
  if (approx_eps) *approx_eps = reinterpret_cast<double *>(ws + L.aeps);
  if (exact_score) *exact_score = reinterpret_cast<double *>(ws + L.scores);
  if (cand_slot) *cand_slot = reinterpret_cast<int32_t *>(ws + L.cand_slot);
  if (cand_count) *cand_count = reinterpret_cast<int32_t *>(ws + L.cnt);
  return 0;
}
```

### sapr_amd/csrc/viterbi_bound.hip

```cpp
#include <algorithm>
#include <cstdlib>

#include "viterbi_shared.h"

namespace sapr {
namespace {

using namespace emission;

template <int D, int S>
__global__ __launch_bounds__(kBlock) void viterbi_approx_kernel(
    const float *__restrict__ feats, const int64_t *__restrict__ offsets, const int32_t *__restrict__ order,
    int64_t n_utts, int64_t n_tiles, int32_t W, const double *__restrict__ prm32_all,
    const double *__restrict__ hgc_all, const double *__restrict__ log_start,
    const double *__restrict__ log_trans, const double *__restrict__ wconst, double *__restrict__ ascore,
    double *__restrict__ aeps) {
  int64_t tile;
  int w;
  decode_block(W, n_tiles, tile, w);
  if (tile >= n_tiles) return;
  const int64_t slot = tile * kBlock + threadIdx.x;
  const bool live = slot < n_utts;
  const int64_t u = live ? (order ? static_cast<int64_t>(order[slot]) : slot) : 0;
  const int64_t beg = live ? offsets[u] : 0;
  const int T = live ? static_cast<int>(offsets[u + 1] - beg) : 0;
  const int Tw = wave_max_i32(T);

  const double *__restrict__ prm32 = prm32_all + static_cast<int64_t>(w) * pack_p32(S, D);
  const double *__restrict__ hg = hgc_all + static_cast<int64_t>(w) * S;
  const double *__restrict__ ls = log_start + static_cast<int64_t>(w) * S;
  const double *__restrict__ lt = log_trans + static_cast<int64_t>(w) * S * S;
  const float *__restrict__ xp = feats + beg * D;

  double delta[S];
  float x[D];
  double mag = 0.0;
#pragma unroll
  for (int s = 0; s < S; ++s) delta[s] = ls[s];
  for (int t = 0; t < Tw; ++t) {
    if (t < T) {
      load_frame_f32<D>(xp + static_cast<int64_t>(t) * D, x);
      const bool first = (t == 0);
      double carry = 0.0;
      float magf = 0.0f;
      frame_quads_f32_each<D, S>(x, prm32, [&](auto jc, float qf) {
        constexpr int j = decltype(jc)::value;
        magf += qf;
        const double bj = __builtin_fma(static_cast<double>(qf), -0.5, hg[j]);
        const double old = delta[j];
        if constexpr (j == 0) {
          delta[0] = (old + (first ? 0.0 : lt[0])) + bj;
        } else {
          const double cp = carry + (first ? neg_inf() : lt[(j - 1) * S + j]);
          const double cs = old + (first ? 0.0 : lt[j * S + j]);
          delta[j] = fmax(cp, cs) + bj;
        }
        carry = old;
      });
      mag += static_cast<double>(magf);
    }
  }
  if (live) {
    double best = delta[0];
#pragma unroll
    for (int s = 1; s < S; ++s) best = (delta[s] > best || delta[s] != delta[s]) ? delta[s] : best;
    const double *wc = wconst + static_cast<int64_t>(w) * 4;
    const double cmax = wc[0], gcs = wc[1], lts = wc[2], lss = wc[3];
    constexpr double u32 = 5.9604644775390625e-08, u64 = 1.1102230246251565e-16;
    const double Td = static_cast<double>(T);
    const double e32 = u32 * (0.5 * (D + 7) * mag + 0.6 * Td * cmax);
    const double e64 = (8.0 * Td + 16.0) * u64 * (0.5 * mag + Td * (0.5 * gcs + lts) + lss);
    ascore[u * W + w] = T > 0 ? best : neg_inf();
    aeps[u * W + w] = T > 0 ? 2.0 * (e32 + e64) + Td * 1e-14 + 1e-30 : 0.0;
  }
}

typedef _Float16 f16x8 __attribute__((ext_vector_type(8)));
typedef float f32x4 __attribute__((ext_vector_type(4)));
typedef unsigned u32x4 __attribute__((ext_vector_type(4)));

__device__ __forceinline__ double nan_where(double v, unsigned long long mask) {
  const unsigned long long b = __builtin_bit_cast(unsigned long long, v);
  unsigned hi = static_cast<unsigned>(b >> 32);
  asm("v_cndmask_b32 %0, %1, %2, %3" : "=v"(hi) : "v"(hi), "v"(0x7FF80000u), "s"(mask));
  return __builtin_bit_cast(double, (static_cast<unsigned long long>(hi) << 32) | (b & 0xFFFFFFFFull));
}

__device__ __forceinline__ float nan_where(float v, unsigned long long mask) {
  unsigned b = __builtin_bit_cast(unsigned, v);
  asm("v_cndmask_b32 %0, %1, %2, %3" : "=v"(b) : "v"(b), "v"(0x7FC00000u), "s"(mask));
  return __builtin_bit_cast(float, b);
}
__device__ __forceinline__ float max_drop_nan(float a, float b) {
  float r;
  asm("v_max_f32 %0, %1, %2" : "=v"(r) : "v"(a), "v"(b));
  return r;
}

__device__ __forceinline__ double max_drop_nan(double a, double b) {
  double r;
  asm("v_max_f64 %0, %1, %2" : "=v"(r) : "v"(a), "v"(b));
  return r;
}

#ifndef SAPR_MFMA_ABL
#define SAPR_MFMA_ABL 0
#endif
__device__ __forceinline__ f32x4 mfma_f16(const u32x4 &a, const u32x4 &b, const f32x4 &c) {
  if constexpr (SAPR_MFMA_ABL & 1) {
    f32x4 r = c;
    r[0] += __uint_as_float(a[0] ^ b[1]);
    return r;
  }
  return __builtin_amdgcn_mfma_f32_16x16x32_f16(__builtin_bit_cast(f16x8, a), __builtin_bit_cast(f16x8, b), c, 0, 0,
                                                0);
}

__host__ __device__ constexpr unsigned long long dense_first_mask(int S, int tau) {
  unsigned long long m = 0;
  for (int r = 1; r < 16; ++r)
    if ((16 * tau + r) % S == 0) m |= 1ull << r;
  return m * 0x0001000100010001ull;
}
__host__ __device__ constexpr int dense_tiles(int S, int WP) { return (WP * S + 15) / 16; }
__device__ __forceinline__ float cnd_f32(float a, float b, unsigned long long mask) {
  float r;
  asm("v_cndmask_b32 %0, %1, %2, %3" : "=v"(r) : "v"(a), "v"(b), "s"(mask));
  return r;
}

template <int B, int E, class F>
__device__ __forceinline__ void sfor(F &&f) {
  if constexpr (B < E) {
    f(std::integral_constant<int, B>{});
    sfor<B + 1, E>(f);
  }
}
__device__ __forceinline__ void wave_fence_lds() {
  __builtin_amdgcn_fence(__ATOMIC_RELEASE, "wavefront");
  __builtin_amdgcn_wave_barrier();
  __builtin_amdgcn_fence(__ATOMIC_ACQUIRE, "wavefront");
}
template <int D, int S, int WP, int NW>
struct BoundLds {
  static constexpr int KC = gemm_kchunks(D), NT = dense_tiles(S, WP), NG = 16 * NT;
  static constexpr size_t frag = static_cast<size_t>(NT) * KC * 2 * 64 * 16;
  static constexpr size_t tab = frag, tab_bytes = 2 * 4 * KC * 8 * 4;
  static constexpr size_t start = tab + tab_bytes, start_bytes = NG * 4;
  static constexpr size_t fin = start + start_bytes, fin_bytes = static_cast<size_t>(NW) * 4 * NG * 4;
  static constexpr bool kDma = NT * (8 * KC + 4) > 256;
  static constexpr size_t stage = (fin + fin_bytes + 15) / 16 * 16, stage_bytes = kDma ? static_cast<size_t>(NW) * KC * 2 * 1024 : 0;
  static constexpr size_t total = stage + stage_bytes;
};

template <int D, int S, int WP, int NW, int WPE>
__global__ __launch_bounds__(NW *kWave) __attribute__((amdgpu_waves_per_eu(WPE))) void viterbi_bound_lds_kernel(
    const float *__restrict__ feats, const int64_t *__restrict__ offsets, const int32_t *__restrict__ order,
    int64_t n_utts, int32_t W, const uint4 *__restrict__ gfrag, const float *__restrict__ gctr,
    const double *__restrict__ gkw, const double *__restrict__ gR, const double *__restrict__ log_start,
    const double *__restrict__ log_trans, const double *__restrict__ wconst, const double *__restrict__ hgc,
    double *__restrict__ ascore, double *__restrict__ aeps) {
  using L = BoundLds<D, S, WP, NW>;
  constexpr int G = gemm_groups(D), KC = L::KC, RT = gemm_rtiles(S), NT = L::NT, NG = L::NG, iC = D % 8, G8 = 8 * G;
  extern __shared__ __attribute__((aligned(16))) unsigned char smem[];
  uint4 *s_frag = reinterpret_cast<uint4 *>(smem);
  float *s_fa = reinterpret_cast<float *>(smem + L::tab);
  float *s_ctra = s_fa + 4 * KC * 8;
  float *s_start = reinterpret_cast<float *>(smem + L::start);
  const int tid = threadIdx.x;
  const int wave = __builtin_amdgcn_readfirstlane(tid / kWave), lane = tid % kWave, col = lane & 15, q = lane >> 4;
  float *s_fin = reinterpret_cast<float *>(smem + L::fin) + static_cast<size_t>(wave) * 4 * NG;
  unsigned char *s_stage = smem + L::stage + static_cast<size_t>(wave) * KC * 2 * 1024;
  constexpr bool kDma = L::kDma;
  const int w0 = static_cast<int>(blockIdx.y) * WP;
  const int nw = W - w0 < WP ? W - w0 : WP;
  const int nt_valid = (nw * S + 15) / 16;
  const double up = gkw[2 * W], down = gkw[2 * W + 1];

  for (int idx = tid; idx < NT * KC * 2 * 64; idx += NW * kWave) {
    const int l = idx & 63, p = (idx >> 6) & 1, c = (idx >> 7) % KC, tau = (idx >> 7) / KC;
    const int g = 16 * tau + (l & 15), wl = g / S, j = g - wl * S;
    uint4 x = make_uint4(0u, 0u, 0u, 0u);
    if (wl < nw) x = gfrag[(((static_cast<int64_t>(w0 + wl) * RT + j / 16) * KC + c) * 2 + p) * kWave + (j % 16) + 16 * (l >> 4)];
    s_frag[idx] = x;
  }
  for (int idx = tid; idx < 4 * KC * 8; idx += NW * kWave) {
    const int i = idx & 7, c = (idx >> 3) % KC, qq = (idx >> 3) / KC;
    const int g = 4 * c + qq;
    const int half = g < G ? 0 : (g < 2 * G ? 1 : 2);
    const int gg = half == 2 ? 0 : g - (half == 1 ? G : 0);
    const int f = 8 * gg + i;
    const bool ok = half < 2 && f < D;
    const float a = ok ? gctr[(half == 0 ? G8 : 2 * G8) + f] : 0.0f;
    s_fa[idx] = a;
    s_ctra[idx] = ok ? gctr[f] * a : 0.0f;
  }
  for (int g = tid; g < NG; g += NW * kWave) {
    const int wl = g / S, j = g - wl * S;
    s_start[g] = wl < nw ? static_cast<float>((log_start[static_cast<int64_t>(w0 + wl) * S + j] - gR[static_cast<int64_t>(w0 + wl) * S + j]) * up)
                         : -__builtin_huge_valf();
  }
  int fbase[KC];
  float onev[KC];
  bool sq[KC];
#pragma unroll
  for (int c = 0; c < KC; ++c) {
    const int g = 4 * c + q;
    const int half = g < G ? 0 : (g < 2 * G ? 1 : 2);
    const int gg = half == 2 ? 0 : g - (half == 1 ? G : 0);
    sq[c] = half == 0;
    onev[c] = (half == 0 && gg == D / 8) ? 1024.0f : 0.0f;
    fbase[c] = 8 * gg;
  }
  unsigned nsbits = 0u;
  bool inner_noself = false;
#pragma unroll
  for (int tau = 0; tau < NT; ++tau) {
    const int g = 16 * tau + col, wl = g / S, j = g - wl * S;
    const bool ns = wl < nw && log_trans[(static_cast<int64_t>(w0 + (wl < nw ? wl : 0)) * S + j) * S + j] == neg_inf();
    nsbits |= ns ? 1u << tau : 0u;
    inner_noself = inner_noself || __ballot(ns && j != 0) != 0ull;
  }
  __syncthreads();

  const float ninf = -__builtin_huge_valf(), qnan = __builtin_nanf("");
  const int64_t n_floats = offsets[n_utts] * D;
  const int64_t n_tiles = (n_utts + 15) / 16;
  const uint4 *fr_lane = s_frag + lane;
  const float4 *fa_q = reinterpret_cast<const float4 *>(s_fa + q * KC * 8);
  const float4 *ctra_q = reinterpret_cast<const float4 *>(s_ctra + q * KC * 8);

  for (int64_t tile = static_cast<int64_t>(blockIdx.x) * NW + wave; tile < n_tiles; tile += static_cast<int64_t>(gridDim.x) * NW) {
    const int64_t slot = tile * 16 + col;
    const bool live = slot < n_utts;
    const int u = live ? (order ? order[slot] : static_cast<int>(slot)) : 0;
    const int64_t beg = live ? offsets[u] : 0;
    const int T = live ? static_cast<int>(offsets[u + 1] - beg) : 0;
    const int Tw = wave_max_i32(T);
    const int Tmin = -wave_max_i32(-T);
    int Ti[4];
#pragma unroll
    for (int i = 0; i < 4; ++i) Ti[i] = __shfl(T, 4 * q + i);
    float v[NT][4];
#pragma unroll
    for (int tau = 0; tau < NT; ++tau) {
      const float sv = s_start[16 * tau + col];
#pragma unroll
      for (int i = 0; i < 4; ++i) v[tau][i] = sv;
    }
    float bigsum = 0.0f;

    float xr[KC][8];
    const float *pc[KC];
    bool tile_safe = true;
#pragma unroll
    for (int c = 0; c < KC; ++c) {
      pc[c] = feats + beg * D + fbase[c];
      tile_safe = tile_safe && (beg + (T > 0 ? T - 1 : 0)) * D + fbase[c] + 8 <= n_floats;
    }
    tile_safe = __all(tile_safe);
    auto load = [&](int t) {
      const int tt = t < T ? t : (T > 0 ? T - 1 : 0);
      if (tile_safe) {
#pragma unroll
        for (int c = 0; c < KC; ++c) {
          const float *p = pc[c] + tt * D;
          const FeatQuad v0 = *reinterpret_cast<const FeatQuad *>(p);
          const FeatQuad v1 = *reinterpret_cast<const FeatQuad *>(p + 4);
          xr[c][0] = v0.a, xr[c][1] = v0.b, xr[c][2] = v0.c, xr[c][3] = v0.d;
          xr[c][4] = v1.a, xr[c][5] = v1.b, xr[c][6] = v1.c, xr[c][7] = v1.d;
        }
      } else {
#pragma unroll
        for (int c = 0; c < KC; ++c) {
          const float *p = pc[c] + tt * D;
#pragma unroll
          for (int i = 0; i < 8; ++i) xr[c][i] = (T > 0 && fbase[c] + i < D) ? p[i] : 0.0f;
        }
      }
    };
    auto prefetch = [&](int t) {
      const int tt = t < T ? t : (T > 0 ? T - 1 : 0);
      if (tile_safe) {
        if (T > 0) {
#pragma unroll
        for (int c = 0; c < KC; ++c) {
          const float *p = pc[c] + tt * D;
          __builtin_amdgcn_global_load_lds(p, (__attribute__((address_space(3))) void *)(s_stage + (2 * c) * 1024), 16, 0, 0);
          __builtin_amdgcn_global_load_lds(p + 4, (__attribute__((address_space(3))) void *)(s_stage + (2 * c + 1) * 1024), 16, 0, 0);
        }
        }
      } else {
#pragma unroll
        for (int c = 0; c < KC; ++c) {
          const float *p = pc[c] + tt * D;
          float4 lo4, hi4;
          lo4.x = (T > 0 && fbase[c] + 0 < D) ? p[0] : 0.0f;
          lo4.y = (T > 0 && fbase[c] + 1 < D) ? p[1] : 0.0f;
          lo4.z = (T > 0 && fbase[c] + 2 < D) ? p[2] : 0.0f;
          lo4.w = (T > 0 && fbase[c] + 3 < D) ? p[3] : 0.0f;
          hi4.x = (T > 0 && fbase[c] + 4 < D) ? p[4] : 0.0f;
          hi4.y = (T > 0 && fbase[c] + 5 < D) ? p[5] : 0.0f;
          hi4.z = (T > 0 && fbase[c] + 6 < D) ? p[6] : 0.0f;
          hi4.w = (T > 0 && fbase[c] + 7 < D) ? p[7] : 0.0f;
          reinterpret_cast<float4 *>(s_stage + (2 * c) * 1024)[lane] = lo4;
          reinterpret_cast<float4 *>(s_stage + (2 * c + 1) * 1024)[lane] = hi4;
        }
      }
    };
    auto step = [&](auto first_c, auto generic_c, auto uniform_c, int t) {
      constexpr bool first = decltype(first_c)::value, generic = decltype(generic_c)::value,
                     uniform = decltype(uniform_c)::value;
      if constexpr (kDma) {
        asm volatile("s_waitcnt vmcnt(0)" ::: "memory");
        wave_fence_lds();
#pragma unroll
        for (int c = 0; c < KC; ++c) {
          const float4 a4 = reinterpret_cast<const float4 *>(s_stage + (2 * c) * 1024)[lane];
          const float4 b4 = reinterpret_cast<const float4 *>(s_stage + (2 * c + 1) * 1024)[lane];
          xr[c][0] = a4.x, xr[c][1] = a4.y, xr[c][2] = a4.z, xr[c][3] = a4.w;
          xr[c][4] = b4.x, xr[c][5] = b4.y, xr[c][6] = b4.z, xr[c][7] = b4.w;
        }
        asm volatile("s_waitcnt lgkmcnt(0)" ::: "memory");
        wave_fence_lds();
        if (t + 1 < Tw) prefetch(t + 1);
      }
      u32x4 fr[2][KC][2];
      auto fetch = [&](auto tau_c, auto buf_c) {
        constexpr int tau = decltype(tau_c)::value, buf = decltype(buf_c)::value;
#pragma unroll
        for (int c = 0; c < KC; ++c)
#pragma unroll
          for (int p = 0; p < 2; ++p) {
            const uint4 x = fr_lane[((tau * KC + c) * 2 + p) * 64];
            fr[buf][c][p] = u32x4{x.x, x.y, x.z, x.w};
          }
      };
      u32x4 bh[KC], bl[KC];
#pragma unroll
      for (int c = 0; c < KC; ++c) {
        const float4 fa0 = fa_q[2 * c], fa1 = fa_q[2 * c + 1], ct0 = ctra_q[2 * c], ct1 = ctra_q[2 * c + 1];
        const float fa[8] = {fa0.x, fa0.y, fa0.z, fa0.w, fa1.x, fa1.y, fa1.z, fa1.w};
        const float ct[8] = {ct0.x, ct0.y, ct0.z, ct0.w, ct1.x, ct1.y, ct1.z, ct1.w};
        float ph[8];
#pragma unroll
        for (int i = 0; i < 8; ++i) {
          const float xv = __builtin_fmaf(xr[c][i], fa[i], -ct[i]);
          const float m = sq[c] ? xv : 1.0f;
          ph[i] = __builtin_fmaf(xv, m, i == iC ? onev[c] : 0.0f);
        }
        const float big = fmaxf(fmaxf(fmaxf(fabsf(ph[0]), fabsf(ph[1])), fmaxf(fabsf(ph[2]), fabsf(ph[3]))),
                                fmaxf(fmaxf(fabsf(ph[4]), fabsf(ph[5])), fmaxf(fabsf(ph[6]), fabsf(ph[7]))));
        bigsum += big > 65504.0f ? __builtin_nanf("") : big;
#pragma unroll
        for (int e = 0; e < 4; ++e) {
          float a = ph[2 * e], b = ph[2 * e + 1];
          const unsigned h2 = __builtin_bit_cast(unsigned, __builtin_amdgcn_cvt_pkrtz(a, b));
          asm("v_fma_mix_f32 %0, %1, -1.0, %0 op_sel_hi:[1,0,0]" : "+v"(a) : "v"(h2));
          asm("v_fma_mix_f32 %0, %1, -1.0, %0 op_sel:[1,0,0] op_sel_hi:[1,0,0]" : "+v"(b) : "v"(h2));
          bh[c][e] = h2;
          bl[c][e] = __builtin_bit_cast(unsigned, __builtin_amdgcn_cvt_pkrtz(a, b));
        }
      }
      __builtin_amdgcn_sched_barrier(0);
      fetch(std::integral_constant<int, NT - 1>{}, std::integral_constant<int, (NT - 1) & 1>{});
      if constexpr (NT > 1) fetch(std::integral_constant<int, NT - 2>{}, std::integral_constant<int, (NT - 2) & 1>{});
      if constexpr (!kDma) {
        if (t + 1 < Tw) load(t + 1);
      }
      __builtin_amdgcn_sched_barrier(0);
      f32x4 accs[2];
      auto chain = [&](auto tau_c) {
        constexpr int tau = decltype(tau_c)::value, buf = tau & 1;
        if (tau < nt_valid) {
          f32x4 acc = {0.f, 0.f, 0.f, 0.f};
#pragma unroll
          for (int c = 0; c < KC; ++c) {
            acc = mfma_f16(bl[c], fr[buf][c][0], acc);
            acc = mfma_f16(bh[c], fr[buf][c][1], acc);
          }
#pragma unroll
          for (int c = 0; c < KC; ++c) acc = mfma_f16(bh[c], fr[buf][c][0], acc);
          accs[buf] = acc;
        }
      };
      chain(std::integral_constant<int, NT - 1>{});
      sfor<0, NT>([&](auto k_c) {
        constexpr int tau = NT - 1 - decltype(k_c)::value, buf = tau & 1;
        if constexpr (tau > 0) chain(std::integral_constant<int, tau - 1>{});
        if constexpr (tau > 1 && !(SAPR_MFMA_ABL & 8)) fetch(std::integral_constant<int, tau - 2>{}, std::integral_constant<int, tau & 1>{});
        if (tau < nt_valid) {
          const f32x4 acc = accs[buf];
          if constexpr (SAPR_MFMA_ABL & 2) {
#pragma unroll
            for (int i = 0; i < 4; ++i) v[tau][i] += acc[i];
          } else {
          constexpr unsigned long long fm = dense_first_mask(S, tau);
          constexpr bool head0 = (16 * tau) % S == 0;
          float nv[4];
          if constexpr (first) {
#pragma unroll
            for (int i = 0; i < 4; ++i) nv[i] = v[tau][i] + acc[i];
          } else {
            int wrap[4];
            float pred[4], self[4];
#pragma unroll
            for (int i = 0; i < 4; ++i) {
              wrap[i] = __float_as_int(ninf);
              if constexpr (tau > 0 && !head0)
                wrap[i] = __builtin_amdgcn_mov_dpp(__float_as_int(v[tau > 0 ? tau - 1 : 0][i]), 0x121, 0xf, 0xf, true);
            }
#pragma unroll
            for (int i = 0; i < 4; ++i)
              pred[i] = __int_as_float(__builtin_amdgcn_update_dpp(wrap[i], __float_as_int(v[tau][i]), 0x111, 0xf, 0xf, false));
            if constexpr (fm != 0ull) {
#pragma unroll
              for (int i = 0; i < 4; ++i) pred[i] = cnd_f32(pred[i], ninf, fm);
            }
#pragma unroll
            for (int i = 0; i < 4; ++i) {
              self[i] = v[tau][i];
              if constexpr (generic) self[i] = (nsbits >> tau) & 1u ? qnan : self[i];
            }
#pragma unroll
            for (int i = 0; i < 4; ++i) pred[i] = max_drop_nan(pred[i], self[i]);
#pragma unroll
            for (int i = 0; i < 4; ++i) nv[i] = pred[i] + acc[i];
          }
#pragma unroll
          for (int i = 0; i < 4; ++i) {
            if constexpr (uniform)
              v[tau][i] = nv[i];
            else
              v[tau][i] = t < Ti[i] ? nv[i] : v[tau][i];
          }
          }
        }
        __builtin_amdgcn_sched_barrier(0);
      });
    };

    if constexpr (kDma) {
      if (Tw > 0) prefetch(0);
    } else {
      load(0);
    }
    if (Tw > 0) step(std::true_type{}, std::false_type{}, std::false_type{}, 0);
    int t = 1;
    if (Tw > 1) {
      step(std::false_type{}, std::true_type{}, std::false_type{}, 1);
      t = 2;
    }
    if (inner_noself) {
      for (; t < Tw; ++t) step(std::false_type{}, std::true_type{}, std::false_type{}, t);
    } else {
      for (; t < Tmin; ++t) step(std::false_type{}, std::false_type{}, std::true_type{}, t);
      for (; t < Tw; ++t) step(std::false_type{}, std::false_type{}, std::false_type{}, t);
    }

    double phi_sum = static_cast<double>(bigsum);
#pragma unroll
    for (int off = 16; off < 64; off <<= 1) phi_sum += __shfl_xor(phi_sum, off);
    constexpr double u32 = 5.9604644775390625e-08, u64 = 1.1102230246251565e-16;
    constexpr double cacc = 36.0 + 68.0 * KC;
    const int wl = col;
    const bool mine = wl < nw;
    const int w = w0 + (mine ? wl : 0);
#pragma unroll
    for (int i = 0; i < 4; ++i) {
      const double phik = __shfl(phi_sum, 4 * q + i);
      const int ui = __shfl(u, 4 * q + i);
      const bool livei = __shfl(live ? 1 : 0, 4 * q + i) != 0;
      wave_fence_lds();
#pragma unroll
      for (int tau = 0; tau < NT; ++tau) s_fin[q * NG + 16 * tau + col] = v[tau][i];
      wave_fence_lds();
      if (mine && livei) {
        double best = neg_inf(), tau_l = 0.0;
        for (int j = 0; j < S; ++j) {
          double sg = log_trans[(static_cast<int64_t>(w) * S + j) * S + j];
          if (sg == neg_inf()) sg = 0.0;
          const double top = hgc[static_cast<int64_t>(w) * S + j] + sg;
          tau_l = (top > tau_l || top != top) ? top : tau_l;
          const double d = static_cast<double>(s_fin[q * NG + wl * S + j]) * down + gR[(static_cast<int64_t>(W) + w) * S + j] - sg;
          best = (d > best || d != d) ? d : best;
        }
        const double *wc4 = wconst + static_cast<int64_t>(w) * 4;
        const double lts = wc4[2], lss = wc4[3], Td = static_cast<double>(Ti[i]);
        const double m_raw = 2.0 * Td * tau_l - best + lss + 7.0 * lts;
        const double m0 = (m_raw > 0.0 || m_raw != m_raw) ? m_raw : 0.0;
        auto interval = [&](double mm) {
          const double span = 3.0 * mm + Td * gkw[w];
          const double e32 = cacc * u32 * 1.001 * span + 0x1p-14 * 1.01 * (Td * gkw[W + w] + 8.0 * phik) * down;
          const double e_lat = u32 * 1.01 * (Td + 1.0) * (mm + 2.0 * lts + lss);
          const double e64 = (8.0 * Td + 16.0) * u64 * (span + Td * lts + lss);
          return 2.0 * (e32 + e_lat + e64) + Td * 1e-14 + 1e-30;
        };
        const double eps0 = interval(m0);
        const double eps = interval(m0 + 2.0 * eps0);
        ascore[static_cast<int64_t>(ui) * W + w] = Ti[i] > 0 ? best : neg_inf();
        aeps[static_cast<int64_t>(ui) * W + w] = Ti[i] > 0 ? eps : 0.0;
      }
    }
    wave_fence_lds();
  }
}

template <int D, int S, int WP, int NW, int WPE>
int launch_bound_lds(const ScoreArgs &a, const PackView &pv, double *ascore, double *aeps) {
  using L = BoundLds<D, S, WP, NW>;
  static_assert(WP <= 16, "one finishing lane per word of a pass");
  const auto kern = viterbi_bound_lds_kernel<D, S, WP, NW, WPE>;
  SAPR_HIP_TRY(hipFuncSetAttribute(reinterpret_cast<const void *>(kern), hipFuncAttributeMaxDynamicSharedMemorySize,
                                   static_cast<int>(L::total)));
  int dev = 0, cus = 256;
  SAPR_HIP_TRY(hipGetDevice(&dev));
  SAPR_HIP_TRY(hipDeviceGetAttribute(&cus, hipDeviceAttributeMultiprocessorCount, dev));
  const int64_t n_tiles = (a.n_utts + 15) / 16;
  const int per_cu = std::max(1, std::min(static_cast<int>((160 * 1024) / L::total), (4 * WPE) / NW));
  int64_t gx = std::min<int64_t>((n_tiles + NW - 1) / NW, static_cast<int64_t>(cus) * per_cu);
  if (gx < 1) gx = 1;
  const int n_pass = (a.W + WP - 1) / WP;
  SAPR_LAUNCH((viterbi_bound_lds_kernel<D, S, WP, NW, WPE>), dim3(static_cast<unsigned>(gx), static_cast<unsigned>(n_pass)),
              dim3(NW * kWave), L::total, a.stream, a.feats, a.offsets, a.order, a.n_utts, a.W, pv.gfrag, pv.gctr,
              pv.gkw, pv.gR, pv.log_start, pv.log_trans, pv.wconst, pv.hgc, ascore, aeps);
  SAPR_HIP_TRY(hipGetLastError());
  return 0;
}

template <int D, int S>
int launch_approx(const ScoreArgs &a, const PackView &pv, double *ascore, double *aeps, int pack_flags) {
  if constexpr (S <= 32) {
    if (pack_flags & SAPR_PACK_GEMM_OK) {
      const char *env = std::getenv("SAPR_BOUND_WC");
      const int want = env ? std::atoi(env) : 0;
      if constexpr (D <= 16 && S <= 16) return launch_bound_lds<D, S, 11, 4, 3>(a, pv, ascore, aeps);
      else if constexpr (D <= 16) return launch_bound_lds<D, S, 11, 4, 2>(a, pv, ascore, aeps);
      else if constexpr (S <= 16) return launch_bound_lds<D, S, 11, 8, 2>(a, pv, ascore, aeps);
      else {
        if (want == 6) return launch_bound_lds<D, S, 6, 8, 2>(a, pv, ascore, aeps);
        return launch_bound_lds<D, S, 11, 8, 2>(a, pv, ascore, aeps);
      }
    }
  }
  const int64_t blocks = round_up(a.n_tiles, kXcd) * a.W;
  if (blocks > 0x7fffffffLL) return fail(SAPR_ERR_ARG, "grid too large (%lld blocks)", (long long)blocks);
  SAPR_LAUNCH((viterbi_approx_kernel<D, S>), dim3(static_cast<unsigned>(blocks)), dim3(kBlock), 0, a.stream, a.feats,
              a.offsets, a.order, a.n_utts, a.n_tiles, a.W, pv.prm32, pv.hgc, pv.log_start, pv.log_trans, pv.wconst,
              ascore, aeps);
  SAPR_HIP_TRY(hipGetLastError());
  return 0;
}

}

int launch_approx_13_10(const ScoreArgs &a, const emission::PackView &pv, double *ascore, double *aeps, int pack_flags) {
  return launch_approx<13, 10>(a, pv, ascore, aeps, pack_flags);
}
int launch_approx_13_18(const ScoreArgs &a, const emission::PackView &pv, double *ascore, double *aeps, int pack_flags) {
  return launch_approx<13, 18>(a, pv, ascore, aeps, pack_flags);
}
int launch_approx_39_10(const ScoreArgs &a, const emission::PackView &pv, double *ascore, double *aeps, int pack_flags) {
  return launch_approx<39, 10>(a, pv, ascore, aeps, pack_flags);
}
int launch_approx_39_18(const ScoreArgs &a, const emission::PackView &pv, double *ascore, double *aeps, int pack_flags) {
  return launch_approx<39, 18>(a, pv, ascore, aeps, pack_flags);
}
}
```

### sapr_amd/csrc/viterbi_shared.h

```cpp
#pragma once

#include "emission.h"

namespace sapr {

constexpr int kBlock = 256;
constexpr int kXcd = 8;
#ifndef SAPR_EXACT_NF
#define SAPR_EXACT_NF 4
#endif
#ifndef SAPR_EXACT_NF39
#define SAPR_EXACT_NF39 4
#endif

__host__ __device__ inline int64_t round_up(int64_t a, int64_t b) { return (a + b - 1) / b * b; }

__device__ __forceinline__ void decode_block(int W, int64_t n_tiles, int64_t &tile, int &w) {
  const int64_t id = blockIdx.x;
  const int xcd = static_cast<int>(id % kXcd);
  const int64_t k = id / kXcd;
  tile = (k / W) * kXcd + xcd;
  w = static_cast<int>(k % W);
  (void)n_tiles;
}

struct ScoreArgs {
  const float *feats;
  const int64_t *offsets;
  const int32_t *order;
  int64_t n_utts, n_tiles, n_slots;
  int32_t max_T, W;
  const double4 *prm;
  const double *gconst, *log_start, *log_trans;
  void *bp;
  double *scores;
  int32_t *last_state;
  hipStream_t stream;
  const int32_t *cand_utt = nullptr;
  const int32_t *cand_cnt = nullptr;
  int32_t seq_all = 0;
};

struct PrunedLayout {
  size_t bp, cand_utt, cand_slot, ascore, aeps, scores, last, cnt, total;
};
__host__ inline PrunedLayout pruned_layout(int64_t n_utts, int W, int max_T) {
  const int64_t n_slots = round_up(n_utts > 0 ? n_utts : 1, kBlock);
  const size_t nw = static_cast<size_t>(n_utts > 0 ? n_utts : 1) * W;
  auto al = [](size_t x) { return (x + 255) / 256 * 256; };
  PrunedLayout L;
  size_t o = 0;
  L.bp = o;
  o += al(static_cast<size_t>(W) * static_cast<size_t>(max_T > 0 ? max_T : 1) * n_slots * sizeof(uint32_t));
  L.cand_utt = o;
  o += al(static_cast<size_t>(W) * n_slots * sizeof(int32_t));
  L.cand_slot = o;
  o += al(nw * sizeof(int32_t));
  L.ascore = o;
  o += al(nw * sizeof(double));
  L.aeps = o;
  o += al(nw * sizeof(double));
  L.scores = o;
  o += al(nw * sizeof(double));
  L.last = o;
  o += al(nw * sizeof(int32_t));
  L.cnt = o;
  o += al(static_cast<size_t>(W) * sizeof(int32_t));
  L.total = o;
  return L;
}

inline size_t workspace_bytes(int64_t n_utts, int W, int S, int max_T, int topology) {
  const int64_t n_slots = round_up(n_utts > 0 ? n_utts : 1, kBlock);
  const size_t per = topology == SAPR_TOPO_BIDIAG ? sizeof(uint32_t) : static_cast<size_t>(S);
  return static_cast<size_t>(W) * static_cast<size_t>(max_T > 0 ? max_T : 1) * n_slots * per;
}

int launch_scores_13_10(const ScoreArgs &a, int topology, int tie, int sum_order, int fast);
int launch_scores_13_18(const ScoreArgs &a, int topology, int tie, int sum_order, int fast);
int launch_scores_39_18_t1s1(const ScoreArgs &a, int topology, int fast);
int launch_scores_39_18_t1s0(const ScoreArgs &a, int topology, int fast);
int launch_scores_39_18_t0s1(const ScoreArgs &a, int topology, int fast);
int launch_scores_39_18_t0s0(const ScoreArgs &a, int topology, int fast);
inline int launch_scores_39_18(const ScoreArgs &a, int topology, int tie, int sum_order, int fast) {
  if (tie == SAPR_TIE_HIGH) return sum_order ? launch_scores_39_18_t1s1(a, topology, fast) : launch_scores_39_18_t1s0(a, topology, fast);
  return sum_order ? launch_scores_39_18_t0s1(a, topology, fast) : launch_scores_39_18_t0s0(a, topology, fast);
}
int launch_scores_39_10_t1s1(const ScoreArgs &a, int topology, int fast);
int launch_scores_39_10_t1s0(const ScoreArgs &a, int topology, int fast);
int launch_scores_39_10_t0s1(const ScoreArgs &a, int topology, int fast);
int launch_scores_39_10_t0s0(const ScoreArgs &a, int topology, int fast);
inline int launch_scores_39_10(const ScoreArgs &a, int topology, int tie, int sum_order, int fast) {
  if (tie == SAPR_TIE_HIGH) return sum_order ? launch_scores_39_10_t1s1(a, topology, fast) : launch_scores_39_10_t1s0(a, topology, fast);
  return sum_order ? launch_scores_39_10_t0s1(a, topology, fast) : launch_scores_39_10_t0s0(a, topology, fast);
}
int launch_approx_13_10(const ScoreArgs &a, const emission::PackView &pv, double *ascore, double *aeps, int pack_flags);
int launch_approx_13_18(const ScoreArgs &a, const emission::PackView &pv, double *ascore, double *aeps, int pack_flags);
int launch_approx_39_10(const ScoreArgs &a, const emission::PackView &pv, double *ascore, double *aeps, int pack_flags);
int launch_approx_39_18(const ScoreArgs &a, const emission::PackView &pv, double *ascore, double *aeps, int pack_flags);

}
```

### sapr_amd/pipeline.py

```python
from __future__ import annotations

import ctypes as C

import numpy as np

from . import _lib
from .frontend import MfccPlan, num_frames
from .trellis import DiagModelPack, PrunedDecoder


class RecognizerPipeline:
    def __init__(self, plan: MfccPlan, pack: DiagModelPack, sample_lengths, tie=_lib.TIE_HIGH,
                 sum_order=_lib.SUM_TVIEW, device=None, mode: str = "auto", pieces: int = 1):
        import torch
        self.torch = torch
        self.lib = _lib.load()
        dev = device or _lib.require_gpu()
        if plan.d_out != pack.D:
            raise ValueError(f"front-end emits {plan.d_out}-dim features, models expect {pack.D}")
        self.plan, self.pack, self.tie, self.sum_order = plan, pack, tie, sum_order
        sl = np.asarray(sample_lengths, dtype=np.int64)
        self.n_utts = int(sl.shape[0])
        fr = num_frames(sl, plan.hop_length).astype(np.int64)
        if not plan.two_pass and fr.max() > plan.max_frames:
            raise ValueError("utterance longer than the plan's max_frames")
        self.frames = fr
        self.total_frames = int(fr.sum())
        self.total_samples = int(sl.sum())
        self.max_T = int(fr.max())
        so = np.zeros(self.n_utts + 1, dtype=np.int64)
        np.cumsum(sl, out=so[1:])
        fo = np.zeros(self.n_utts + 1, dtype=np.int64)
        np.cumsum(fr, out=fo[1:])
        order = np.argsort(-fr, kind="stable").astype(np.int32)
        t = torch.from_numpy
        self.sample_offsets = t(so).to(dev)
        self.frame_offsets = t(fo).to(dev)
        self.order = t(order).to(dev)
        if mode not in ("auto", "pruned", "full"):
            raise ValueError("mode must be 'auto', 'pruned' or 'full'")
        if mode == "pruned" and not pack.prunable:
            raise _lib.SaprHipError("mode='pruned' needs a bidiagonal model pack inside the bound's domain")
        self.mode = "pruned" if (mode != "full" and pack.prunable) else "full"
        self.feats = torch.empty((self.total_frames, plan.d_out), dtype=torch.float32, device=dev)
        self.mfcc_ws, self.mfcc_ws_bytes = plan.workspace(self.total_frames, self.n_utts, dev)
        if self.mode == "pruned":
            self.best_word = torch.empty(self.n_utts, dtype=torch.int32, device=dev)
            self.best_score = torch.empty(self.n_utts, dtype=torch.float64, device=dev)
            self.path = torch.empty(self.total_frames, dtype=torch.int32, device=dev)
            self.scores = self.last_state = None
            n_p = max(1, min(int(pieces), self.n_utts // 4096))
            cuts = np.linspace(0, self.n_utts, n_p + 1).astype(np.int64)
            self._pieces = []
            for lo, hi in zip(cuts[:-1], cuts[1:]):
                lo, hi = int(lo), int(hi)
                dec = PrunedDecoder(hi - lo, int(fr[lo:hi].max()), 0, pack, dev)
                order_p = t(np.argsort(-fr[lo:hi], kind="stable").astype(np.int32)).to(dev)
                stream = torch.cuda.Stream(device=dev) if n_p > 1 else None
                self._pieces.append((lo, hi, dec, order_p, stream))
            self.pruned = self._pieces[0][2] if n_p == 1 else None
            self._ev_in = torch.cuda.Event()
            self._ev_out = [torch.cuda.Event() for _ in self._pieces]
            return
        nbytes = C.c_size_t(0)
        _lib.check(self.lib.sapr_viterbi_workspace_bytes(self.n_utts, pack.W, pack.S, self.max_T,
                                                         pack.topology, C.byref(nbytes)),
                   "sapr_viterbi_workspace_bytes")
        self.ws_bytes = int(nbytes.value)
        self.workspace = torch.empty(max(self.ws_bytes, 1), dtype=torch.uint8, device=dev)
        self.scores = torch.empty((self.n_utts, pack.W), dtype=torch.float64, device=dev)
        self.last_state = torch.empty((self.n_utts, pack.W), dtype=torch.int32, device=dev)
        self.best_word = torch.empty(self.n_utts, dtype=torch.int32, device=dev)
        self.best_score = torch.empty(self.n_utts, dtype=torch.float64, device=dev)
        self.path = torch.empty(self.total_frames, dtype=torch.int32, device=dev)

    def launch_decode(self, stream):
        if self.mode == "pruned":
            torch = self.torch
            if len(self._pieces) == 1:
                lo, hi, dec, order_p, _ = self._pieces[0]
                dec.launch(self.feats, self.frame_offsets, order_p, self.tie, self.sum_order, stream,
                           out=(self.best_word, self.best_score, self.path))
                return
            main = torch.cuda.ExternalStream(stream.value) if stream.value else torch.cuda.default_stream(self.feats.device)
            self._ev_in.record(main)
            for (lo, hi, dec, order_p, st), ev in zip(self._pieces, self._ev_out):
                st.wait_event(self._ev_in)
                dec.launch(self.feats, self.frame_offsets[lo:hi + 1], order_p, self.tie, self.sum_order,
                           C.c_void_p(st.cuda_stream),
                           out=(self.best_word[lo:hi], self.best_score[lo:hi], self.path))
                ev.record(st)
            for ev in self._ev_out:
                main.wait_event(ev)
        else:
            self.launch_viterbi(stream)
            self.launch_backtrace(stream)

    def launch_mfcc(self, pcm, stream):
        _lib.check(self.lib.sapr_mfcc_batch(self.plan._h, _lib.ptr(pcm), _lib.ptr(self.sample_offsets),
                                            _lib.ptr(self.frame_offsets), self.n_utts, self.total_frames,
                                            _lib.ptr(self.feats), 0, _lib.ptr(self.mfcc_ws), self.mfcc_ws_bytes,
                                            stream), "sapr_mfcc_batch")

    def launch_viterbi(self, stream):
        p = self.pack
        _lib.check(self.lib.sapr_viterbi_diag_scores(
            _lib.ptr(self.feats), _lib.ptr(self.frame_offsets), _lib.ptr(self.order), self.n_utts, p.D,
            self.max_T, _lib.ptr(p.blob), p.W, p.S, p.topology, self.tie, self.sum_order, p.fast_div,
            _lib.ptr(self.workspace), self.ws_bytes, _lib.ptr(self.scores), _lib.ptr(self.last_state),
            stream), "sapr_viterbi_diag_scores")

    def launch_backtrace(self, stream):
        p = self.pack
        _lib.check(self.lib.sapr_viterbi_backtrace(
            _lib.ptr(self.frame_offsets), _lib.ptr(self.order), self.n_utts, self.max_T, p.W, p.S,
            p.topology, _lib.ptr(self.workspace), self.ws_bytes, _lib.ptr(self.scores),
            _lib.ptr(self.last_state), None, _lib.ptr(self.best_word), _lib.ptr(self.best_score),
            _lib.ptr(self.path), stream), "sapr_viterbi_backtrace")

    def pruned_views(self):
        torch = self.torch
        v = [dec.views() for _, _, dec, _, _ in self._pieces]
        return tuple(torch.cat([x[i] for x in v], dim=0) for i in range(4)) + (sum(x[4] for x in v),)

    def run(self, pcm):
        if pcm.shape[0] != self.total_samples:
            raise ValueError("pcm length does not match the pipeline's sample_lengths")
        stream = _lib.current_stream()
        self.launch_mfcc(pcm, stream)
        self.launch_decode(stream)
        return self.best_word, self.best_score, self.path
```

### sapr_amd/trellis.py

```python
from __future__ import annotations

import os

import ctypes as C
from dataclasses import dataclass

import numpy as np

from . import _lib

_TINY = np.finfo(float).tiny


def _torch():
    import torch
    return torch


@dataclass
class FeatureBatch:
    feats: "object"
    offsets: "object"
    order: "object"
    lengths: np.ndarray
    max_T: int
    D: int
    D_model: int = 0

    def __post_init__(self):
        if not self.D_model:
            self.D_model = self.D

    @property
    def n_utts(self) -> int:
        return int(self.lengths.shape[0])

    @property
    def total_frames(self) -> int:
        return int(self.lengths.sum())

    @staticmethod
    def from_arrays(utterances, layout: str = "DT", device=None) -> "FeatureBatch":
        torch = _torch()
        device = device or _lib.require_gpu()
        if len(utterances) == 0:
            raise ValueError("empty utterance list")
        if layout == "DT":
            mats = [np.ascontiguousarray(np.asarray(f).T, dtype=np.float32) for f in utterances]
        elif layout == "TD":
            mats = [np.ascontiguousarray(np.asarray(f), dtype=np.float32) for f in utterances]
        else:
            raise ValueError(f"unknown layout {layout!r}")
        D = mats[0].shape[1]
        for m in mats:
            if m.ndim != 2 or m.shape[1] != D:
                raise ValueError("all utterances must share the feature dimension")
        lengths = np.asarray([m.shape[0] for m in mats], dtype=np.int64)
        packed = np.concatenate(mats, axis=0) if lengths.sum() else np.zeros((0, D), np.float32)
        return FeatureBatch.from_packed(torch.from_numpy(packed).to(device), lengths)

    @staticmethod
    def from_packed(feats, lengths) -> "FeatureBatch":
        torch = _torch()
        lengths = np.asarray(lengths, dtype=np.int64)
        offs = np.zeros(lengths.shape[0] + 1, dtype=np.int64)
        np.cumsum(lengths, out=offs[1:])
        if feats.dtype != torch.float32 or feats.dim() != 2 or not feats.is_contiguous():
            raise ValueError("feats must be a contiguous float32 [total_frames, D] tensor")
        if feats.shape[0] != offs[-1]:
            raise ValueError("feats rows do not match sum(lengths)")
        order = np.argsort(-lengths, kind="stable").astype(np.int32)
        dev = feats.device
        d_model = int(feats.shape[1])
        dk = kernel_dims(d_model)
        if dk != d_model and d_model > 0:
            wide = torch.zeros((feats.shape[0], dk), dtype=torch.float32, device=dev)
            wide[:, :d_model] = feats
            feats = wide
        return FeatureBatch(feats=feats, offsets=torch.from_numpy(offs).to(dev),
                            order=torch.from_numpy(order).to(dev), lengths=lengths,
                            max_T=int(lengths.max()) if lengths.size else 0, D=int(feats.shape[1]), D_model=d_model)


def is_bidiagonal(transmat: np.ndarray) -> bool:
    S = transmat.shape[-1]
    mask = np.eye(S, dtype=bool) | np.eye(S, k=1, dtype=bool)
    return bool(np.all(transmat[..., ~mask] == 0))


KERNEL_STATES = (10, 18)


def kernel_states(S: int) -> int:
    for k in KERNEL_STATES:
        if S <= k:
            return k
    return S


KERNEL_DIMS = (13, 39)


def kernel_dims(D: int) -> int:
    for k in KERNEL_DIMS:
        if D <= k:
            return k
    return D


@dataclass
class DiagModelPack:
    means: "object"
    vars: "object"
    gconst: "object"
    log_start: "object"
    log_trans: "object"
    W: int
    S: int
    D: int
    topology: int
    blob: "object" = None
    fast_div: int = 0
    flags: int = 0
    S_model: int = 0
    D_model: int = 0

    def _build_blob(self, exact_only=False):
        torch = _torch()
        lib = _lib.load()
        n = C.c_size_t(0)
        _lib.check(lib.sapr_diag_pack_bytes(self.W, self.S, self.D, C.byref(n)), "sapr_diag_pack_bytes")
        self.blob = torch.empty(int(n.value), dtype=torch.uint8, device=self.means.device)
        ok = C.c_int32(_lib.PACK_EXACT_ONLY if exact_only else 0)
        _lib.check(lib.sapr_diag_pack(_lib.ptr(self.means), _lib.ptr(self.vars), _lib.ptr(self.gconst),
                                      _lib.ptr(self.log_start), _lib.ptr(self.log_trans), self.W, self.S,
                                      self.D, _lib.ptr(self.blob), int(n.value), C.byref(ok),
                                      _lib.current_stream()), "sapr_diag_pack")
        self.flags = int(ok.value)
        self.fast_div = 1 if self.flags & _lib.PACK_FAST_DIV else 0
        return self

    @property
    def prunable(self) -> bool:
        need = _lib.PACK_BOUND_OK | _lib.PACK_BIDIAG
        return self.topology == _lib.TOPO_BIDIAG and (self.flags & need) == need

    @staticmethod
    def from_params(startprob, transmat, means, covars, device=None, exact_only=False) -> "DiagModelPack":
        torch = _torch()
        device = device or _lib.require_gpu()
        startprob = np.asarray(startprob, dtype=np.float64)
        transmat = np.asarray(transmat, dtype=np.float64)
        means = np.ascontiguousarray(means, dtype=np.float64)
        covars = np.asarray(covars, dtype=np.float64)
        W, S, D = means.shape
        if startprob.shape != (W, S) or transmat.shape != (W, S, S) or covars.shape != (W, S, D):
            raise ValueError("inconsistent model shapes")
        S_model, Sk = S, kernel_states(S)
        if Sk != S:
            pad = Sk - S
            startprob = np.concatenate([startprob, np.zeros((W, pad))], axis=1)
            tm = np.zeros((W, Sk, Sk))
            tm[:, :S, :S] = transmat
            tm[:, np.arange(S, Sk), np.arange(S, Sk)] = 1.0
            transmat = tm
            means = np.ascontiguousarray(np.concatenate([means, np.zeros((W, pad, D))], axis=1))
            covars = np.concatenate([covars, np.ones((W, pad, D))], axis=1)
            S = Sk
        var = np.maximum(covars, _TINY)
        gconst = D * np.log(2 * np.pi) + np.log(var).sum(axis=-1)
        D_model, Dk = D, kernel_dims(D)
        if Dk != D:
            means = np.ascontiguousarray(np.concatenate([means, np.zeros((W, S, Dk - D))], axis=2))
            var = np.concatenate([var, np.ones((W, S, Dk - D))], axis=2)
            D = Dk
        with np.errstate(divide="ignore"):
            log_start = np.log(startprob)
            log_trans = np.log(transmat)
        topo = _lib.TOPO_BIDIAG if (is_bidiagonal(transmat) and S <= 32) else _lib.TOPO_DENSE

        parts = [np.ascontiguousarray(a, dtype=np.float64) for a in (means, var, gconst, log_start, log_trans)]
        flat = torch.from_numpy(np.concatenate([a.ravel() for a in parts])).to(device)
        views, at = [], 0
        for a in parts:
            views.append(flat[at:at + a.size].view(a.shape))
            at += a.size
        return DiagModelPack(means=views[0], vars=views[1], gconst=views[2], log_start=views[3], log_trans=views[4],
                             W=W, S=S, D=D, topology=topo, S_model=S_model, D_model=D_model)._build_blob(exact_only)

    @staticmethod
    def from_models(models, device=None, exact_only=False) -> "DiagModelPack":
        sp = np.stack([np.asarray(m.startprob_, dtype=np.float64) for m in models])
        tm = np.stack([np.asarray(m.transmat_, dtype=np.float64) for m in models])
        mu = np.stack([np.asarray(m.means_, dtype=np.float64) for m in models])
        cv = np.stack([np.asarray(m._covars_, dtype=np.float64) for m in models])
        return DiagModelPack.from_params(sp, tm, mu, cv, device=device, exact_only=exact_only)


def _check_dims(batch: FeatureBatch, pack: "DiagModelPack"):
    if batch.D_model != (pack.D_model or pack.D) or batch.D != pack.D:
        raise ValueError(f"feature dim {batch.D_model} != model dim {pack.D_model or pack.D}")


def _exact_sum_order(batch: FeatureBatch, sum_order: int) -> int:
    if batch.D_model != batch.D and batch.D_model < 8:
        return _lib.SUM_SEQ
    return sum_order


@dataclass
class ViterbiResult:
    scores: "object"
    last_state: "object"
    best_word: "object"
    best_score: "object"
    path: "object"


class PrunedDecoder:

    def __init__(self, n_utts, max_T, total_frames, pack: DiagModelPack, device, approx: str = None):
        torch = _torch()
        self.lib = _lib.load()
        approx = approx or os.environ.get("SAPR_APPROX", "auto")
        if approx not in ("auto", "valu"):
            raise ValueError(f"approx must be 'auto' or 'valu', got {approx!r}")
        self.flag_mask = ~_lib.PACK_GEMM_OK if approx == "valu" else ~0
        if not pack.prunable:
            raise _lib.SaprHipError("model pack is not prunable (dense topology or variances outside [1e-20, 1e20])")
        self.N, self.max_T, self.pack = int(n_utts), int(max_T), pack
        n = C.c_size_t(0)
        _lib.check(self.lib.sapr_viterbi_pruned_workspace_bytes(self.N, pack.W, pack.S, self.max_T, C.byref(n)),
                   "sapr_viterbi_pruned_workspace_bytes")
        self.ws_bytes = int(n.value)
        self.workspace = torch.empty(max(self.ws_bytes, 1), dtype=torch.uint8, device=device)
        self.best_word = self.best_score = self.path = None
        if total_frames:
            self.best_word = torch.empty(self.N, dtype=torch.int32, device=device)
            self.best_score = torch.empty(self.N, dtype=torch.float64, device=device)
            self.path = torch.empty(int(total_frames), dtype=torch.int32, device=device)

    def launch(self, feats, offsets, order, tie, sum_order, stream, out=None):
        p = self.pack
        bw, bs, path = out if out is not None else (self.best_word, self.best_score, self.path)
        _lib.check(self.lib.sapr_viterbi_decode_pruned(
            _lib.ptr(feats), _lib.ptr(offsets), _lib.ptr(order), self.N, p.D, self.max_T, _lib.ptr(p.blob), p.W, p.S,
            tie, sum_order, p.flags & self.flag_mask, _lib.ptr(self.workspace), self.ws_bytes, _lib.ptr(bw),
            _lib.ptr(bs), _lib.ptr(path), stream), "sapr_viterbi_decode_pruned")

    def views(self):
        torch = _torch()
        ptrs = [C.c_void_p() for _ in range(5)]
        _lib.check(self.lib.sapr_viterbi_pruned_views(self.N, self.pack.W, self.max_T, _lib.ptr(self.workspace),
                                                      *[C.byref(q) for q in ptrs]), "sapr_viterbi_pruned_views")
        base = self.workspace.data_ptr()
        W = self.pack.W

        def view(q, dtype, shape):
            off = q.value - base
            nbytes = int(np.prod(shape)) * torch.empty((), dtype=dtype).element_size()
            return self.workspace[off:off + nbytes].view(dtype).view(*shape)
        return (view(ptrs[0], torch.float64, (self.N, W)), view(ptrs[1], torch.float64, (self.N, W)),
                view(ptrs[2], torch.float64, (self.N, W)), view(ptrs[3], torch.int32, (self.N, W)),
                view(ptrs[4], torch.int32, (W,)))


def viterbi_decode_best(batch: FeatureBatch, pack: DiagModelPack, tie: int = _lib.TIE_HIGH,
                        sum_order: int = _lib.SUM_TVIEW):
    _check_dims(batch, pack)
    sum_order = _exact_sum_order(batch, sum_order)
    if not pack.prunable or batch.n_utts == 0:
        r = viterbi_decode(batch, pack, tie=tie, sum_order=sum_order)
        return r.best_word, r.best_score, r.path
    dec = PrunedDecoder(batch.n_utts, batch.max_T, batch.total_frames, pack, batch.feats.device)
    dec.launch(batch.feats, batch.offsets, batch.order, tie, sum_order, _lib.current_stream())
    return dec.best_word, dec.best_score, dec.path


def viterbi_decode(batch: FeatureBatch, pack: DiagModelPack, tie: int = _lib.TIE_HIGH,
                   sum_order: int = _lib.SUM_TVIEW, word_sel=None,
                   want_path: bool = True, fast_div=None) -> ViterbiResult:
    torch = _torch()
    lib = _lib.load()
    _check_dims(batch, pack)
    sum_order = _exact_sum_order(batch, sum_order)
    dev = batch.feats.device
    N, W, S = batch.n_utts, pack.W, pack.S
    nbytes = C.c_size_t(0)
    _lib.check(lib.sapr_viterbi_workspace_bytes(N, W, S, batch.max_T, pack.topology, C.byref(nbytes)),
               "sapr_viterbi_workspace_bytes")
    ws = torch.empty(max(int(nbytes.value), 1), dtype=torch.uint8, device=dev)
    scores = torch.empty((N, W), dtype=torch.float64, device=dev)
    last = torch.empty((N, W), dtype=torch.int32, device=dev)
    stream = _lib.current_stream()
    _lib.check(lib.sapr_viterbi_diag_scores(
        _lib.ptr(batch.feats), _lib.ptr(batch.offsets), _lib.ptr(batch.order), N, batch.D, batch.max_T,
        _lib.ptr(pack.blob), W, S, pack.topology, tie, sum_order,
        pack.fast_div if fast_div is None else int(fast_div), _lib.ptr(ws), nbytes.value,
        _lib.ptr(scores), _lib.ptr(last), stream), "sapr_viterbi_diag_scores")
    best_word = torch.empty(N, dtype=torch.int32, device=dev)
    best_score = torch.empty(N, dtype=torch.float64, device=dev)
    path = torch.empty(batch.total_frames, dtype=torch.int32, device=dev) if want_path else None
    if word_sel is not None:
        word_sel = torch.as_tensor(word_sel, dtype=torch.int32, device=dev).contiguous()
    _lib.check(lib.sapr_viterbi_backtrace(
        _lib.ptr(batch.offsets), _lib.ptr(batch.order), N, batch.max_T, W, S, pack.topology,
        _lib.ptr(ws), nbytes.value, _lib.ptr(scores), _lib.ptr(last), _lib.ptr(word_sel),
        _lib.ptr(best_word), _lib.ptr(best_score), _lib.ptr(path), stream), "sapr_viterbi_backtrace")
    return ViterbiResult(scores, last, best_word, best_score, path)


_TILE = 256


@dataclass
class TileLayout:
    slot_utt: "object"
    tile_model: "object"
    model_tile_off: "object"
    n_tiles: int

    @staticmethod
    def build(lengths, utt_model, W, device):
        torch = _torch()
        lengths = np.asarray(lengths, dtype=np.int64)
        utt_model = np.asarray(utt_model, dtype=np.int64)
        slots, tile_model, off = [], [], [0]
        for w in range(W):
            idx = np.nonzero(utt_model == w)[0]
            idx = idx[np.argsort(-lengths[idx], kind="stable")]
            n_t = (idx.size + _TILE - 1) // _TILE
            pad = np.full(n_t * _TILE, -1, dtype=np.int32)
            pad[: idx.size] = idx
            slots.append(pad)
            tile_model += [w] * n_t
            off.append(off[-1] + n_t)
        slot_utt = np.concatenate(slots) if slots else np.zeros(0, np.int32)
        t = torch.from_numpy
        return TileLayout(t(slot_utt).to(device), t(np.asarray(tile_model, dtype=np.int32)).to(device),
                          t(np.asarray(off, dtype=np.int32)).to(device), len(tile_model))


def stats_width(S, D):
    return 2 + S + S * S + S + 2 * S * D


def split_stats(row, S, D, S_model=None, D_model=None):
    o = 0
    m = S if S_model is None else S_model
    dm = D if D_model is None else D_model

    def take(n):
        nonlocal o
        v = row[o:o + n]
        o += n
        return v
    nobs, logprob = take(1)[0], take(1)[0]
    return {"nobs": nobs, "logprob": logprob, "start": take(S)[:m].copy(),
            "trans": take(S * S).reshape(S, S)[:m, :m].copy(), "post": take(S)[:m].copy(),
            "obs": take(S * D).reshape(S, D)[:m, :dm].copy(), "obs**2": take(S * D).reshape(S, D)[:m, :dm].copy()}


def forward_loglik(batch: FeatureBatch, pack: DiagModelPack, utt_model, layout: TileLayout = None):
    torch = _torch()
    lib = _lib.load()
    dev = batch.feats.device
    layout = layout or TileLayout.build(batch.lengths, utt_model, pack.W, dev)
    loglik = torch.zeros(batch.n_utts, dtype=torch.float64, device=dev)
    _lib.check(lib.sapr_forward_diag(_lib.ptr(batch.feats), _lib.ptr(batch.offsets), _lib.ptr(layout.slot_utt),
                                     _lib.ptr(layout.tile_model), layout.n_tiles, batch.D, _lib.ptr(pack.blob),
                                     pack.W, pack.S, pack.topology, pack.fast_div, _lib.ptr(loglik),
                                     _lib.current_stream()), "sapr_forward_diag")
    return loglik


class EStep:

    def __init__(self, batch: FeatureBatch, utt_model, W, S):
        torch = _torch()
        self.lib = _lib.load()
        self.S_model, S = S, kernel_states(S)
        self.batch, self.W, self.S, self.D = batch, W, S, batch.D
        dev = batch.feats.device
        self.layout = TileLayout.build(batch.lengths, utt_model, W, dev)
        n = C.c_size_t(0)
        _lib.check(self.lib.sapr_fb_workspace_bytes(batch.n_utts, self.layout.n_tiles, S, self.D, batch.max_T,
                                                    C.byref(n)), "sapr_fb_workspace_bytes")
        self.ws_bytes = int(n.value)
        self.workspace = torch.empty(self.ws_bytes, dtype=torch.uint8, device=dev)
        self.loglik = torch.zeros(batch.n_utts, dtype=torch.float64, device=dev)
        self.stats = torch.zeros((W, stats_width(S, self.D)), dtype=torch.float64, device=dev)
        self._staged = False

    def split(self, row):
        return split_stats(row, self.S, self.D, self.S_model, self.batch.D_model)

    def run(self, pack: DiagModelPack):
        if pack.S != self.S:
            raise ValueError(f"model pack has {pack.S} kernel states, this E-step was laid out for {self.S}")
        b, lay = self.batch, self.layout
        _lib.check(self.lib.sapr_estep_diag(
            _lib.ptr(b.feats), _lib.ptr(b.offsets), _lib.ptr(lay.slot_utt), _lib.ptr(lay.tile_model),
            _lib.ptr(lay.model_tile_off), b.n_utts, lay.n_tiles, b.D, b.max_T, _lib.ptr(pack.blob), pack.W,
            pack.S, pack.topology, pack.fast_div | (_lib.ESTEP_STAGED if self._staged else 0),
            _lib.ptr(self.workspace), self.ws_bytes, _lib.ptr(self.loglik),
            _lib.ptr(self.stats), _lib.current_stream()), "sapr_estep_diag")
        self._staged = True
        return self.stats
```

Measured before the change: 2.023 billion frames/s.

## Fuse log-mel-to-MFCC finishing pass into the pruned Viterbi bounding kernel

```diff
diff --git a/include/sapr_hip.h b/include/sapr_hip.h
--- a/include/sapr_hip.h
+++ b/include/sapr_hip.h
@@ -65,6 +65,12 @@
                                int32_t sum_order, int32_t pack_flags, void *workspace, size_t workspace_bytes,
                                int32_t *best_word, double *best_score, int32_t *path ,
                                void *stream);
+int sapr_viterbi_decode_pruned_logmel(const void *mfcc_plan, const void *mfcc_workspace, int64_t total_frames,
+                                      const int64_t *offsets, const int32_t *order, int64_t n_utts, int32_t D,
+                                      int32_t max_T, const void *pack, int32_t W, int32_t S, int32_t tie,
+                                      int32_t sum_order, int32_t pack_flags, void *workspace, size_t workspace_bytes,
+                                      float *feats , int32_t *best_word, double *best_score,
+                                      int32_t *path , void *stream);
 int sapr_viterbi_pruned_views(int64_t n_utts, int32_t W, int32_t max_T, void *workspace, double **approx_score,
                               double **approx_eps, double **exact_score, int32_t **cand_slot,
                               int32_t **cand_count);
@@ -145,6 +151,10 @@
                     int32_t grid_blocks , void *workspace ,
                     size_t workspace_bytes, void *stream);
 
+int sapr_mfcc_logmel_batch(const void *plan, const float *pcm, const int64_t *sample_offsets,
+                           const int64_t *frame_offsets, int64_t n_utts, int64_t total_frames,
+                           int32_t grid_blocks , void *workspace, size_t workspace_bytes, void *stream);
+
 int sapr_resample_poly(const float *x, const int64_t *in_offsets, const int64_t *out_offsets, int64_t n_utts,
                        int64_t max_out, int32_t up, int32_t down, const float *taps, int32_t n_taps,
                        int32_t n_pre_remove, float *y, void *stream);
diff --git a/sapr_amd/_lib.py b/sapr_amd/_lib.py
--- a/sapr_amd/_lib.py
+++ b/sapr_amd/_lib.py
@@ -29,6 +29,10 @@
     "sapr_viterbi_decode_pruned": (c_int, [c_void_p, c_void_p, c_void_p, c_int64, c_int32, c_int32, c_void_p,
                                            c_int32, c_int32, c_int32, c_int32, c_int32, c_void_p, c_size_t,
                                            c_void_p, c_void_p, c_void_p, c_void_p]),
+    "sapr_viterbi_decode_pruned_logmel": (c_int, [c_void_p, c_void_p, c_int64, c_void_p, c_void_p, c_int64, c_int32,
+                                                  c_int32, c_void_p, c_int32, c_int32, c_int32, c_int32, c_int32,
+                                                  c_void_p, c_size_t, c_void_p, c_void_p, c_void_p, c_void_p,
+                                                  c_void_p]),
     "sapr_viterbi_pruned_views": (c_int, [c_int64, c_int32, c_int32, c_void_p] + [C.POINTER(c_void_p)] * 5),
     "sapr_fb_workspace_bytes": (c_int, [c_int64, c_int64, c_int32, c_int32, c_int32, C.POINTER(c_size_t)]),
     "sapr_stats_width": (c_int, [c_int32, c_int32, C.POINTER(c_int32)]),
@@ -75,6 +79,8 @@
     "sapr_mfcc_workspace_bytes": (c_int, [c_void_p, c_int64, c_int64, C.POINTER(c_size_t)]),
     "sapr_mfcc_batch": (c_int, [c_void_p, c_void_p, c_void_p, c_void_p, c_int64, c_int64, c_void_p, c_int32,
                                 c_void_p, c_size_t, c_void_p]),
+    "sapr_mfcc_logmel_batch": (c_int, [c_void_p, c_void_p, c_void_p, c_void_p, c_int64, c_int64, c_int32, c_void_p,
+                                       c_size_t, c_void_p]),
     "sapr_mfcc_batch_stamped": (c_int, [c_void_p, c_void_p, c_void_p, c_void_p, c_int64, c_void_p, c_int32,
                                         c_void_p, c_void_p]),
 }
diff --git a/sapr_amd/csrc/mfcc.hip b/sapr_amd/csrc/mfcc.hip
--- a/sapr_amd/csrc/mfcc.hip
+++ b/sapr_amd/csrc/mfcc.hip
@@ -939,6 +939,19 @@
   return wave_dispatch_s4<false, 0, 16>(pl, prepare, pcm, so, fo, n_utts, grid, span, st, lm, gmax, total_cap);
 }
 
+int wave_spectral(const MfccPlan &pl, const float *pcm, const int64_t *so, const int64_t *fo, int64_t n_utts,
+                  int64_t total_frames, int grid_blocks, int cus, hipStream_t st, float *lm, unsigned *gmax) {
+  int wgrid = grid_blocks > 0 ? grid_blocks : cus * pl.wave_blocks_per_cu;
+  const int64_t n_waves = static_cast<int64_t>(wgrid) * kWaves;
+  int64_t span = (total_frames + n_waves - 1) / n_waves;
+  span = span < 4 ? 4 : (span + 3) / 4 * 4;
+  const int64_t need_blocks = ((total_frames + span - 1) / span + kWaves - 1) / kWaves;
+  if (need_blocks < wgrid) wgrid = static_cast<int>(need_blocks < 1 ? 1 : need_blocks);
+  SAPR_HIP_TRY(hipMemsetAsync(gmax, 0, static_cast<size_t>(n_utts) * sizeof(unsigned), st));
+  SAPR_HIP_TRY(wave_dispatch(pl, nullptr, pcm, so, fo, n_utts, wgrid, span, st, lm, gmax, total_frames));
+  return 0;
+}
+
 size_t finish_lds_bytes(const MfccDev &d) {
   return static_cast<size_t>(align_up(2 * 81, 4) + kFinRows * 16 + kFinRows * d.lm_stride) * 4;
 }
@@ -1347,15 +1360,8 @@
   float *lm = static_cast<float *>(workspace);
   unsigned *gmax = reinterpret_cast<unsigned *>(lm + static_cast<size_t>(total_frames) * pl->dev.n_mels);
   if (pl->dev.wave_s4) {
-    int wgrid = grid_blocks > 0 ? grid_blocks : cus * pl->wave_blocks_per_cu;
-    const int64_t n_waves = static_cast<int64_t>(wgrid) * kWaves;
-    int64_t span = (total_frames + n_waves - 1) / n_waves;
-    span = span < 4 ? 4 : (span + 3) / 4 * 4;
-    const int64_t need_blocks = ((total_frames + span - 1) / span + kWaves - 1) / kWaves;
-    if (need_blocks < wgrid) wgrid = static_cast<int>(need_blocks < 1 ? 1 : need_blocks);
-    SAPR_HIP_TRY(hipMemsetAsync(gmax, 0, static_cast<size_t>(n_utts) * sizeof(unsigned), st));
-    SAPR_HIP_TRY(wave_dispatch(*pl, nullptr, pcm, sample_offsets, frame_offsets, n_utts, wgrid, span, st, lm, gmax,
-                               total_frames));
+    if (int rc = wave_spectral(*pl, pcm, sample_offsets, frame_offsets, n_utts, total_frames, grid_blocks, cus, st, lm, gmax))
+      return rc;
     int fgrid = cus * SAPR_FINISH_OCC;
     const int64_t fwaves = static_cast<int64_t>(fgrid) * kWaves;
     int fsplit = 1;
@@ -1379,3 +1385,38 @@
   SAPR_HIP_TRY(hipGetLastError());
   return 0;
 }
+
+namespace sapr {
+int logmel_plan_view(const void *plan, LogmelPlanView *v) {
+  SAPR_REQUIRE(plan != nullptr, "plan is NULL");
+  const MfccPlan *pl = static_cast<const MfccPlan *>(plan);
+  if (!pl->dev.wave_s4 || pl->dev.deltas)
+    return fail(SAPR_ERR_UNSUPPORTED, "log-mel-only runs need a 512-point wave-core plan without deltas");
+  v->dct_frag = pl->dev.dct_frag;
+  v->top_db = pl->dev.top_db;
+  v->n_mels = pl->dev.n_mels;
+  v->n_mfcc = pl->dev.n_mfcc;
+  return 0;
+}
+}
+
+extern "C" int sapr_mfcc_logmel_batch(const void *plan, const float *pcm, const int64_t *sample_offsets,
+                                      const int64_t *frame_offsets, int64_t n_utts, int64_t total_frames,
+                                      int32_t grid_blocks, void *workspace, size_t workspace_size, void *stream) {
+  LogmelPlanView lp;
+  if (int rc = logmel_plan_view(plan, &lp)) return rc;
+  SAPR_REQUIRE(n_utts >= 0 && total_frames >= 0, "bad sizes");
+  if (n_utts == 0) return 0;
+  SAPR_REQUIRE(pcm && sample_offsets && frame_offsets, "NULL pointer argument");
+  const MfccPlan *pl = static_cast<const MfccPlan *>(plan);
+  const size_t need = (static_cast<size_t>(total_frames) * pl->dev.n_mels + static_cast<size_t>(n_utts)) * sizeof(float) + 256;
+  if (!workspace || workspace_size < need)
+    return fail(SAPR_ERR_WORKSPACE, "log-mel-only run needs a %zu-byte workspace (sapr_mfcc_workspace_bytes)", need);
+  int dev = 0, cus = 256;
+  SAPR_HIP_TRY(hipGetDevice(&dev));
+  SAPR_HIP_TRY(hipDeviceGetAttribute(&cus, hipDeviceAttributeMultiprocessorCount, dev));
+  float *lm = static_cast<float *>(workspace);
+  unsigned *gmax = reinterpret_cast<unsigned *>(lm + static_cast<size_t>(total_frames) * pl->dev.n_mels);
+  return wave_spectral(*pl, pcm, sample_offsets, frame_offsets, n_utts, total_frames, grid_blocks, cus, as_stream(stream),
+                       lm, gmax);
+}
diff --git a/sapr_amd/csrc/mfcc_wave.h b/sapr_amd/csrc/mfcc_wave.h
--- a/sapr_amd/csrc/mfcc_wave.h
+++ b/sapr_amd/csrc/mfcc_wave.h
@@ -26,15 +26,6 @@
   o += kWaves * region_floats * 4;
   L.total = o;
   return L;
-}
-
-__host__ __device__ inline unsigned enc_ordered(float v) {
-  const unsigned u = __builtin_bit_cast(unsigned, v);
-  return (u & 0x80000000u) ? ~u : (u | 0x80000000u);
-}
-__host__ __device__ inline float dec_ordered(unsigned e) {
-  const unsigned u = (e & 0x80000000u) ? (e & 0x7FFFFFFFu) : ~e;
-  return __builtin_bit_cast(float, u);
 }
 
 struct __attribute__((packed, aligned(4))) f2u {
diff --git a/sapr_amd/csrc/sapr_common.h b/sapr_amd/csrc/sapr_common.h
--- a/sapr_amd/csrc/sapr_common.h
+++ b/sapr_amd/csrc/sapr_common.h
@@ -64,6 +64,15 @@
   }
 }
 
+__host__ __device__ inline unsigned enc_ordered(float v) {
+  const unsigned u = __builtin_bit_cast(unsigned, v);
+  return (u & 0x80000000u) ? ~u : (u | 0x80000000u);
+}
+__host__ __device__ inline float dec_ordered(unsigned e) {
+  const unsigned u = (e & 0x80000000u) ? (e & 0x7FFFFFFFu) : ~e;
+  return __builtin_bit_cast(float, u);
+}
+
 __device__ __forceinline__ int wave_max_i32(int v) {
 #pragma unroll
   for (int o = 32; o > 0; o >>= 1) {
@@ -73,4 +82,11 @@
   return v;
 }
 
+struct LogmelPlanView {
+  const float *dct_frag;
+  float top_db;
+  int n_mels, n_mfcc;
+};
+int logmel_plan_view(const void *plan, LogmelPlanView *v);
+
 }
diff --git a/sapr_amd/csrc/viterbi.hip b/sapr_amd/csrc/viterbi.hip
--- a/sapr_amd/csrc/viterbi.hip
+++ b/sapr_amd/csrc/viterbi.hip
@@ -583,11 +583,9 @@
   return 0;
 }
 
-extern "C" int sapr_viterbi_decode_pruned(const float *feats, const int64_t *offsets, const int32_t *order,
-                                          int64_t n_utts, int32_t D, int32_t max_T, const void *pack, int32_t W,
-                                          int32_t S, int32_t tie, int32_t sum_order, int32_t pack_flags,
-                                          void *workspace, size_t workspace_size, int32_t *best_word,
-                                          double *best_score, int32_t *path, void *stream) {
+namespace {
+int pruned_checks(int64_t n_utts, int32_t D, int32_t max_T, int32_t W, int32_t S, int32_t tie, int32_t sum_order,
+                  int32_t pack_flags) {
   SAPR_REQUIRE(n_utts >= 0 && W > 0 && S > 0 && D > 0 && max_T >= 0, "bad sizes");
   SAPR_REQUIRE(tie == SAPR_TIE_LOW || tie == SAPR_TIE_HIGH, "bad tie-break");
   SAPR_REQUIRE(sum_order == SAPR_SUM_PAIRWISE || sum_order == SAPR_SUM_TVIEW || sum_order == SAPR_SUM_SEQ, "bad sum_order");
@@ -598,8 +596,20 @@
     return fail(SAPR_ERR_UNSUPPORTED, "the pruned decoder covers the bidiagonal topology only (transitions i -> i and "
                                       "i -> i + 1, S <= 32; sapr_diag_pack reports SAPR_PACK_BIDIAG): use "
                                       "sapr_viterbi_diag_scores + sapr_viterbi_backtrace");
-  if (n_utts == 0) return 0;
-  SAPR_REQUIRE(feats && offsets && pack && workspace && best_word && best_score, "NULL pointer argument");
+  return 0;
+}
+
+struct FusedA {
+  LogmelPlanView lp;
+  const void *mfcc_ws;
+  int64_t total_frames;
+  float *feats;
+};
+
+int decode_pruned(const float *feats, const int64_t *offsets, const int32_t *order, int64_t n_utts, int32_t D,
+                  int32_t max_T, const void *pack, int32_t W, int32_t S, int32_t tie, int32_t sum_order,
+                  int32_t pack_flags, void *workspace, size_t workspace_size, int32_t *best_word, double *best_score,
+                  int32_t *path, void *stream, const FusedA *fused) {
   const PrunedLayout L = pruned_layout(n_utts, W, max_T);
   if (workspace_size < L.total)
     return fail(SAPR_ERR_WORKSPACE, "workspace too small: %zu < %zu", workspace_size, L.total);
@@ -631,7 +641,8 @@
   a.stream = as_stream(stream);
   a.seq_all = sum_order == SAPR_SUM_SEQ ? 1 : 0;
   int rc;
-  if (D == 13 && S == 10) rc = launch_approx_13_10(a, pv, ascore, aeps, pack_flags);
+  if (fused) rc = launch_approx_logmel_13_10(a, pv, ascore, aeps, fused->lp, fused->mfcc_ws, fused->total_frames, fused->feats);
+  else if (D == 13 && S == 10) rc = launch_approx_13_10(a, pv, ascore, aeps, pack_flags);
   else if (D == 13 && S == 18) rc = launch_approx_13_18(a, pv, ascore, aeps, pack_flags);
   else if (D == 39 && S == 10) rc = launch_approx_39_10(a, pv, ascore, aeps, pack_flags);
   else if (D == 39 && S == 18) rc = launch_approx_39_18(a, pv, ascore, aeps, pack_flags);
@@ -657,6 +668,43 @@
   SAPR_HIP_TRY(hipGetLastError());
   return 0;
 }
+}
+
+extern "C" int sapr_viterbi_decode_pruned(const float *feats, const int64_t *offsets, const int32_t *order,
+                                          int64_t n_utts, int32_t D, int32_t max_T, const void *pack, int32_t W,
+                                          int32_t S, int32_t tie, int32_t sum_order, int32_t pack_flags,
+                                          void *workspace, size_t workspace_size, int32_t *best_word,
+                                          double *best_score, int32_t *path, void *stream) {
+  if (int rc = pruned_checks(n_utts, D, max_T, W, S, tie, sum_order, pack_flags)) return rc;
+  if (n_utts == 0) return 0;
+  SAPR_REQUIRE(feats && offsets && pack && workspace && best_word && best_score, "NULL pointer argument");
+  return decode_pruned(feats, offsets, order, n_utts, D, max_T, pack, W, S, tie, sum_order, pack_flags, workspace,
+                       workspace_size, best_word, best_score, path, stream, nullptr);
+}
+
+extern "C" int sapr_viterbi_decode_pruned_logmel(const void *mfcc_plan, const void *mfcc_workspace,
+                                                 int64_t total_frames, const int64_t *offsets, const int32_t *order,
+                                                 int64_t n_utts, int32_t D, int32_t max_T, const void *pack, int32_t W,
+                                                 int32_t S, int32_t tie, int32_t sum_order, int32_t pack_flags,
+                                                 void *workspace, size_t workspace_size, float *feats,
+                                                 int32_t *best_word, double *best_score, int32_t *path, void *stream) {
+  if (int rc = pruned_checks(n_utts, D, max_T, W, S, tie, sum_order, pack_flags)) return rc;
+  FusedA f;
+  if (int rc = logmel_plan_view(mfcc_plan, &f.lp)) return rc;
+  if (!(pack_flags & SAPR_PACK_GEMM_OK) || D != 13 || S != 10 || f.lp.n_mfcc != D || f.lp.n_mels != 40)
+    return fail(SAPR_ERR_UNSUPPORTED, "the fused bounding pass covers matrix-core packs of 13 dimensions and 10 states "
+                                      "behind 40 mels x 13 coefficients (got D=%d S=%d, %d mels x %d, flags %d)",
+                D, S, f.lp.n_mels, f.lp.n_mfcc, pack_flags);
+  SAPR_REQUIRE(total_frames >= 0, "bad sizes");
+  if (n_utts == 0) return 0;
+  SAPR_REQUIRE(mfcc_workspace && feats && offsets && pack && workspace && best_word && best_score,
+               "NULL pointer argument");
+  f.mfcc_ws = mfcc_workspace;
+  f.total_frames = total_frames;
+  f.feats = feats;
+  return decode_pruned(feats, offsets, order, n_utts, D, max_T, pack, W, S, tie, sum_order, pack_flags, workspace,
+                       workspace_size, best_word, best_score, path, stream, &f);
+}
 
 extern "C" int sapr_viterbi_pruned_views(int64_t n_utts, int32_t W, int32_t max_T, void *workspace,
                                          double **approx_score, double **approx_eps, double **exact_score,
diff --git a/sapr_amd/csrc/viterbi_bound.hip b/sapr_amd/csrc/viterbi_bound.hip
--- a/sapr_amd/csrc/viterbi_bound.hip
+++ b/sapr_amd/csrc/viterbi_bound.hip
@@ -141,7 +141,7 @@
   __builtin_amdgcn_wave_barrier();
   __builtin_amdgcn_fence(__ATOMIC_ACQUIRE, "wavefront");
 }
-template <int D, int S, int WP, int NW>
+template <int D, int S, int WP, int NW, int NKS = 0>
 struct BoundLds {
   static constexpr int KC = gemm_kchunks(D), NT = dense_tiles(S, WP), NG = 16 * NT;
   static constexpr size_t frag = static_cast<size_t>(NT) * KC * 2 * 64 * 16;
@@ -150,18 +150,31 @@
   static constexpr size_t fin = start + start_bytes, fin_bytes = static_cast<size_t>(NW) * 4 * NG * 4;
   static constexpr bool kDma = NT * (8 * KC + 4) > 256;
   static constexpr size_t stage = (fin + fin_bytes + 15) / 16 * 16, stage_bytes = kDma ? static_cast<size_t>(NW) * KC * 2 * 1024 : 0;
-  static constexpr size_t total = stage + stage_bytes;
+  static constexpr size_t dct = stage + stage_bytes, dct_bytes = static_cast<size_t>(NKS) * 64 * 4;
+  static constexpr size_t lmst = dct + dct_bytes, lmst_bytes = static_cast<size_t>(NW) * NKS * 64 * 4;
+  static constexpr size_t total = lmst + lmst_bytes;
 };
 
-template <int D, int S, int WP, int NW, int WPE>
+struct LmIn {
+  const float *lm;
+  const unsigned *gmax_enc;
+  const float *dct_frag;
+  float *feats;
+  float top_db;
+  int64_t total_frames;
+};
+
+template <int D, int S, int WP, int NW, int WPE, int NKS>
 __global__ __launch_bounds__(NW *kWave) __attribute__((amdgpu_waves_per_eu(WPE))) void viterbi_bound_lds_kernel(
     const float *__restrict__ feats, const int64_t *__restrict__ offsets, const int32_t *__restrict__ order,
     int64_t n_utts, int32_t W, const uint4 *__restrict__ gfrag, const float *__restrict__ gctr,
     const double *__restrict__ gkw, const double *__restrict__ gR, const double *__restrict__ log_start,
     const double *__restrict__ log_trans, const double *__restrict__ wconst, const double *__restrict__ hgc,
-    double *__restrict__ ascore, double *__restrict__ aeps) {
-  using L = BoundLds<D, S, WP, NW>;
+    double *__restrict__ ascore, double *__restrict__ aeps, const LmIn lmi) {
+  using L = BoundLds<D, S, WP, NW, NKS>;
   constexpr int G = gemm_groups(D), KC = L::KC, RT = gemm_rtiles(S), NT = L::NT, NG = L::NG, iC = D % 8, G8 = 8 * G;
+  constexpr bool LM = NKS > 0;
+  static_assert(!LM || (!L::kDma && KC == 1 && G <= 2 && 4 * NG >= 256), "fused route: D <= 15, fragments in registers");
   extern __shared__ __attribute__((aligned(16))) unsigned char smem[];
   uint4 *s_frag = reinterpret_cast<uint4 *>(smem);
   float *s_fa = reinterpret_cast<float *>(smem + L::tab);
@@ -176,6 +189,18 @@
   const int nw = W - w0 < WP ? W - w0 : WP;
   const int nt_valid = (nw * S + 15) / 16;
   const double up = gkw[2 * W], down = gkw[2 * W + 1];
+  if constexpr (LM) {
+    if (offsets[n_utts] > lmi.total_frames) {
+      if (blockIdx.y == 0) {
+        const int64_t stride = static_cast<int64_t>(gridDim.x) * NW * kWave;
+        for (int64_t i = static_cast<int64_t>(blockIdx.x) * NW * kWave + tid; i < lmi.total_frames * D; i += stride)
+          lmi.feats[i] = __builtin_nanf("");
+        for (int64_t i = static_cast<int64_t>(blockIdx.x) * NW * kWave + tid; i < n_utts * W; i += stride)
+          ascore[i] = aeps[i] = __builtin_nan("");
+      }
+      return;
+    }
+  }
 
   for (int idx = tid; idx < NT * KC * 2 * 64; idx += NW * kWave) {
     const int l = idx & 63, p = (idx >> 6) & 1, c = (idx >> 7) % KC, tau = (idx >> 7) / KC;
@@ -195,6 +220,10 @@
     s_fa[idx] = a;
     s_ctra[idx] = ok ? gctr[f] * a : 0.0f;
   }
+  float *s_dct = reinterpret_cast<float *>(smem + L::dct);
+  for (int i = tid; i < NKS * 64; i += NW * kWave) s_dct[i] = lmi.dct_frag[i];
+  float *s_lm = reinterpret_cast<float *>(smem + L::lmst) + static_cast<size_t>(wave) * NKS * 64;
+  for (int i = lane; i < NKS * 64; i += kWave) s_lm[i] = 0.0f;
   for (int g = tid; g < NG; g += NW * kWave) {
     const int wl = g / S, j = g - wl * S;
     s_start[g] = wl < nw ? static_cast<float>((log_start[static_cast<int64_t>(w0 + wl) * S + j] - gR[static_cast<int64_t>(w0 + wl) * S + j]) * up)
@@ -259,6 +288,17 @@
       tile_safe = tile_safe && (beg + (T > 0 ? T - 1 : 0)) * D + fbase[c] + 8 <= n_floats;
     }
     tile_safe = __all(tile_safe);
+    const float *lrow = LM ? lmi.lm + beg * (4 * NKS) + q : nullptr;
+    float *frow = LM ? lmi.feats + beg * D + 4 * q : nullptr;
+    const float floor_db = LM ? dec_ordered(lmi.gmax_enc[u]) - lmi.top_db : 0.0f;
+    auto prefetch_lm = [&](int t) {
+      if (T > 0) {
+        const float *p = lrow + static_cast<int64_t>(t < T ? t : T - 1) * (4 * NKS);
+#pragma unroll
+        for (int ks = 0; ks < NKS; ++ks)
+          __builtin_amdgcn_global_load_lds(p + 4 * ks, (__attribute__((address_space(3))) void *)(s_lm + ks * 64), 4, 0, 0);
+      }
+    };
     auto load = [&](int t) {
       const int tt = t < T ? t : (T > 0 ? T - 1 : 0);
       if (tile_safe) {
@@ -311,6 +351,41 @@
     auto step = [&](auto first_c, auto generic_c, auto uniform_c, int t) {
       constexpr bool first = decltype(first_c)::value, generic = decltype(generic_c)::value,
                      uniform = decltype(uniform_c)::value;
+      if constexpr (LM) {
+        asm volatile("s_waitcnt vmcnt(0)" ::: "memory");
+        wave_fence_lds();
+        float lmr[NKS];
+#pragma unroll
+        for (int ks = 0; ks < NKS; ++ks) lmr[ks] = s_lm[ks * 64 + lane];
+        asm volatile("s_waitcnt lgkmcnt(0)" ::: "memory");
+        wave_fence_lds();
+        if (t + 1 < Tw) prefetch_lm(t + 1);
+        f32x4 acc0 = {0.f, 0.f, 0.f, 0.f}, acc1 = {0.f, 0.f, 0.f, 0.f};
+#pragma unroll
+        for (int ks = 0; ks < NKS; ++ks) {
+          const float b = fmaxf(lmr[ks], floor_db);
+          if (ks & 1)
+            acc1 = __builtin_amdgcn_mfma_f32_16x16x4f32(s_dct[ks * 64 + lane], b, acc1, 0, 0, 0);
+          else
+            acc0 = __builtin_amdgcn_mfma_f32_16x16x4f32(s_dct[ks * 64 + lane], b, acc0, 0, 0, 0);
+        }
+        const f32x4 cf = acc0 + acc1;
+        if (t < T) {
+#pragma unroll
+          for (int r = 0; r < 4; ++r)
+            if (4 * q + r < D) frow[static_cast<int64_t>(t) * D + r] = cf[r];
+        }
+        wave_fence_lds();
+        *reinterpret_cast<f32x4 *>(s_fin + col * 16 + 4 * q) = cf;
+        wave_fence_lds();
+#pragma unroll
+        for (int c = 0; c < KC; ++c) {
+          const float4 a4 = reinterpret_cast<const float4 *>(s_fin + col * 16 + fbase[c])[0];
+          const float4 b4 = reinterpret_cast<const float4 *>(s_fin + col * 16 + fbase[c])[1];
+          xr[c][0] = a4.x, xr[c][1] = a4.y, xr[c][2] = a4.z, xr[c][3] = a4.w;
+          xr[c][4] = b4.x, xr[c][5] = b4.y, xr[c][6] = b4.z, xr[c][7] = b4.w;
+        }
+      }
       if constexpr (kDma) {
         asm volatile("s_waitcnt vmcnt(0)" ::: "memory");
         wave_fence_lds();
@@ -365,7 +440,7 @@
       __builtin_amdgcn_sched_barrier(0);
       fetch(std::integral_constant<int, NT - 1>{}, std::integral_constant<int, (NT - 1) & 1>{});
       if constexpr (NT > 1) fetch(std::integral_constant<int, NT - 2>{}, std::integral_constant<int, (NT - 2) & 1>{});
-      if constexpr (!kDma) {
+      if constexpr (!LM && !kDma) {
         if (t + 1 < Tw) load(t + 1);
       }
       __builtin_amdgcn_sched_barrier(0);
@@ -440,7 +515,9 @@
       });
     };
 
-    if constexpr (kDma) {
+    if constexpr (LM) {
+      if (Tw > 0) prefetch_lm(0);
+    } else if constexpr (kDma) {
       if (Tw > 0) prefetch(0);
     } else {
       load(0);
@@ -506,11 +583,11 @@
   }
 }
 
-template <int D, int S, int WP, int NW, int WPE>
-int launch_bound_lds(const ScoreArgs &a, const PackView &pv, double *ascore, double *aeps) {
-  using L = BoundLds<D, S, WP, NW>;
+template <int D, int S, int WP, int NW, int WPE, int NKS = 0>
+int launch_bound_lds(const ScoreArgs &a, const PackView &pv, double *ascore, double *aeps, const LmIn &lmi = LmIn{}) {
+  using L = BoundLds<D, S, WP, NW, NKS>;
   static_assert(WP <= 16, "one finishing lane per word of a pass");
-  const auto kern = viterbi_bound_lds_kernel<D, S, WP, NW, WPE>;
+  const auto kern = viterbi_bound_lds_kernel<D, S, WP, NW, WPE, NKS>;
   SAPR_HIP_TRY(hipFuncSetAttribute(reinterpret_cast<const void *>(kern), hipFuncAttributeMaxDynamicSharedMemorySize,
                                    static_cast<int>(L::total)));
   int dev = 0, cus = 256;
@@ -521,9 +598,9 @@
   int64_t gx = std::min<int64_t>((n_tiles + NW - 1) / NW, static_cast<int64_t>(cus) * per_cu);
   if (gx < 1) gx = 1;
   const int n_pass = (a.W + WP - 1) / WP;
-  SAPR_LAUNCH((viterbi_bound_lds_kernel<D, S, WP, NW, WPE>), dim3(static_cast<unsigned>(gx), static_cast<unsigned>(n_pass)),
+  SAPR_LAUNCH((viterbi_bound_lds_kernel<D, S, WP, NW, WPE, NKS>), dim3(static_cast<unsigned>(gx), static_cast<unsigned>(n_pass)),
               dim3(NW * kWave), L::total, a.stream, a.feats, a.offsets, a.order, a.n_utts, a.W, pv.gfrag, pv.gctr,
-              pv.gkw, pv.gR, pv.log_start, pv.log_trans, pv.wconst, pv.hgc, ascore, aeps);
+              pv.gkw, pv.gR, pv.log_start, pv.log_trans, pv.wconst, pv.hgc, ascore, aeps, lmi);
   SAPR_HIP_TRY(hipGetLastError());
   return 0;
 }
@@ -566,4 +643,17 @@
 int launch_approx_39_18(const ScoreArgs &a, const emission::PackView &pv, double *ascore, double *aeps, int pack_flags) {
   return launch_approx<39, 18>(a, pv, ascore, aeps, pack_flags);
 }
-}
+int launch_approx_logmel_13_10(const ScoreArgs &a, const emission::PackView &pv, double *ascore, double *aeps,
+                               const LogmelPlanView &lp, const void *mfcc_ws, int64_t total_frames, float *feats) {
+  if (lp.n_mels != 40 || lp.n_mfcc != 13)
+    return fail(SAPR_ERR_UNSUPPORTED, "the fused bounding pass is instantiated for 40 mels and 13 coefficients");
+  LmIn lmi;
+  lmi.lm = static_cast<const float *>(mfcc_ws);
+  lmi.gmax_enc = reinterpret_cast<const unsigned *>(lmi.lm + total_frames * lp.n_mels);
+  lmi.dct_frag = lp.dct_frag;
+  lmi.feats = feats;
+  lmi.top_db = lp.top_db;
+  lmi.total_frames = total_frames;
+  return launch_bound_lds<13, 10, 11, 4, 3, 10>(a, pv, ascore, aeps, lmi);
+}
+}
diff --git a/sapr_amd/csrc/viterbi_shared.h b/sapr_amd/csrc/viterbi_shared.h
--- a/sapr_amd/csrc/viterbi_shared.h
+++ b/sapr_amd/csrc/viterbi_shared.h
@@ -98,5 +98,7 @@
 int launch_approx_13_18(const ScoreArgs &a, const emission::PackView &pv, double *ascore, double *aeps, int pack_flags);
 int launch_approx_39_10(const ScoreArgs &a, const emission::PackView &pv, double *ascore, double *aeps, int pack_flags);
 int launch_approx_39_18(const ScoreArgs &a, const emission::PackView &pv, double *ascore, double *aeps, int pack_flags);
+int launch_approx_logmel_13_10(const ScoreArgs &a, const emission::PackView &pv, double *ascore, double *aeps,
+                               const LogmelPlanView &lp, const void *mfcc_ws, int64_t total_frames, float *feats);
 
 }
diff --git a/sapr_amd/pipeline.py b/sapr_amd/pipeline.py
--- a/sapr_amd/pipeline.py
+++ b/sapr_amd/pipeline.py
@@ -42,6 +42,7 @@
         if mode == "pruned" and not pack.prunable:
             raise _lib.SaprHipError("mode='pruned' needs a bidiagonal model pack inside the bound's domain")
         self.mode = "pruned" if (mode != "full" and pack.prunable) else "full"
+        self.fused = False
         self.feats = torch.empty((self.total_frames, plan.d_out), dtype=torch.float32, device=dev)
         self.mfcc_ws, self.mfcc_ws_bytes = plan.workspace(self.total_frames, self.n_utts, dev)
         if self.mode == "pruned":
@@ -59,6 +60,8 @@
                 stream = torch.cuda.Stream(device=dev) if n_p > 1 else None
                 self._pieces.append((lo, hi, dec, order_p, stream))
             self.pruned = self._pieces[0][2] if n_p == 1 else None
+            self.fused = (n_p == 1 and self.mfcc_ws is not None
+                          and self.pruned.logmel_ok(plan, self.tie, self.sum_order))
             self._ev_in = torch.cuda.Event()
             self._ev_out = [torch.cuda.Event() for _ in self._pieces]
             return
@@ -77,6 +80,11 @@
     def launch_decode(self, stream):
         if self.mode == "pruned":
             torch = self.torch
+            if self.fused:
+                _, _, dec, order_p, _ = self._pieces[0]
+                dec.launch_logmel(self.plan, self.mfcc_ws, self.total_frames, self.feats, self.frame_offsets, order_p,
+                                  self.tie, self.sum_order, stream, out=(self.best_word, self.best_score, self.path))
+                return
             if len(self._pieces) == 1:
                 lo, hi, dec, order_p, _ = self._pieces[0]
                 dec.launch(self.feats, self.frame_offsets, order_p, self.tie, self.sum_order, stream,
@@ -97,6 +105,11 @@
             self.launch_backtrace(stream)
 
     def launch_mfcc(self, pcm, stream):
+        if self.fused:
+            _lib.check(self.lib.sapr_mfcc_logmel_batch(
+                self.plan._h, _lib.ptr(pcm), _lib.ptr(self.sample_offsets), _lib.ptr(self.frame_offsets), self.n_utts,
+                self.total_frames, 0, _lib.ptr(self.mfcc_ws), self.mfcc_ws_bytes, stream), "sapr_mfcc_logmel_batch")
+            return
         _lib.check(self.lib.sapr_mfcc_batch(self.plan._h, _lib.ptr(pcm), _lib.ptr(self.sample_offsets),
                                             _lib.ptr(self.frame_offsets), self.n_utts, self.total_frames,
                                             _lib.ptr(self.feats), 0, _lib.ptr(self.mfcc_ws), self.mfcc_ws_bytes,
diff --git a/sapr_amd/trellis.py b/sapr_amd/trellis.py
--- a/sapr_amd/trellis.py
+++ b/sapr_amd/trellis.py
@@ -247,6 +247,21 @@
             _lib.ptr(feats), _lib.ptr(offsets), _lib.ptr(order), self.N, p.D, self.max_T, _lib.ptr(p.blob), p.W, p.S,
             tie, sum_order, p.flags & self.flag_mask, _lib.ptr(self.workspace), self.ws_bytes, _lib.ptr(bw),
             _lib.ptr(bs), _lib.ptr(path), stream), "sapr_viterbi_decode_pruned")
+
+    def logmel_ok(self, plan, tie, sum_order) -> bool:
+        p = self.pack
+        return self.lib.sapr_viterbi_decode_pruned_logmel(
+            plan._h, None, 0, None, None, 0, p.D, self.max_T, None, p.W, p.S, tie, sum_order, p.flags & self.flag_mask,
+            None, 0, None, None, None, None, None) == 0
+
+    def launch_logmel(self, plan, mfcc_ws, total_frames, feats, offsets, order, tie, sum_order, stream, out):
+        p = self.pack
+        bw, bs, path = out
+        _lib.check(self.lib.sapr_viterbi_decode_pruned_logmel(
+            plan._h, _lib.ptr(mfcc_ws), int(total_frames), _lib.ptr(offsets), _lib.ptr(order), self.N, p.D,
+            self.max_T, _lib.ptr(p.blob), p.W, p.S, tie, sum_order, p.flags & self.flag_mask,
+            _lib.ptr(self.workspace), self.ws_bytes, _lib.ptr(feats), _lib.ptr(bw), _lib.ptr(bs), _lib.ptr(path),
+            stream), "sapr_viterbi_decode_pruned_logmel")
 
     def views(self):
         torch = _torch()
```

Result: slower. 1.849 billion frames/s (median of 2 runs) (-8.6%).
